# facebookresearch/D3GA

Measured on AMD Instinct MI355X. Metric: fwd+bwd frames/sec @500k Gaussians 1920x1080, higher is better.
Workload: dtype f32

## Files before the change

### d3ga_amd/_lib.py

```python
import ctypes
import os

_HERE = os.path.dirname(os.path.abspath(__file__))
_PATH = os.environ.get("D3GA_LIB_PATH") or os.path.join(_HERE, "libd3ga_hip.so")
_lib = None
ACC_STRIDE = 16
replay_epoch = [0]
ABI_VERSION = 111
KNOBS = ("composite_variant", "merge_slots", "tile_assign", "bwd_split", "sort_merge", "ssim_impl", "wgrad_ws", "chain_abl", "chain_grid")
CAMERA_SLOT_WINDOWED = -1.0
LOSS_PARTIALS = 2048
BLUR_PARTIALS = 6144
OPTIM_CHUNK = 8192
OPTIM_ALIGNED16 = 1


class D3GAError(RuntimeError):
    pass


def library_path():
    return _PATH


class RasterParams(ctypes.Structure):
    _fields_ = [("P", ctypes.c_int32), ("M", ctypes.c_int32), ("sh_degree", ctypes.c_int32),
                ("W", ctypes.c_int32), ("H", ctypes.c_int32),
                ("tanfovx", ctypes.c_float), ("tanfovy", ctypes.c_float), ("scale_modifier", ctypes.c_float),
                ("antialiasing", ctypes.c_int32), ("prefiltered", ctypes.c_int32), ("debug", ctypes.c_int32),
                ("opacity_activation", ctypes.c_int32), ("forward_only", ctypes.c_int32),
                ("acc_self_clearing", ctypes.c_int32), ("n_views", ctypes.c_int32), ("per_view_geometry", ctypes.c_int32),
                ("factor_rows", ctypes.c_int32), ("per_view_appearance", ctypes.c_int32), ("per_view_background", ctypes.c_int32)]


BODY_MAX_JOINTS = 64
BODY_MAX_SHAPE = 32
BODY_LD_ALIGN = 2048


def body_saved_floats(J):
    return 27 * J + 16


class BodyModel(ctypes.Structure):
    _fields_ = [("V", ctypes.c_int32), ("J", ctypes.c_int32), ("n_shape", ctypes.c_int32), ("n_expr", ctypes.c_int32),
                ("n_hand_pca", ctypes.c_int32), ("ld", ctypes.c_int32), ("n_levels", ctypes.c_int32), ("reserved", ctypes.c_int32)] + \
               [(n, ctypes.c_void_p) for n in ("v_template", "dirs", "w_ptr", "w_joint", "w_val", "wt_ptr", "wt_vert", "wt_val",
                                               "J0", "Jdirs", "parents", "level_ptr", "level_joint", "child_ptr", "child_joint",
                                               "hand_comps", "hand_mean")]


class LbsPoseGrad(ctypes.Structure):
    _fields_ = [("J", ctypes.c_int32), ("n_chunks", ctypes.c_int32), ("n_entries", ctypes.c_int64)] + \
               [(n, ctypes.c_void_p) for n in ("tmpl", "delta", "chunk_ptr", "chunk_range", "entries", "counter", "scratch", "g_joint_mats",
                                               "g_Rh", "g_Th")]


SKEL_MAX_JOINTS = 512
SKEL_SAVED_FLOATS = 12


class Skeleton(ctypes.Structure):
    _fields_ = [("J", ctypes.c_int32), ("n_params", ctypes.c_int32), ("n_levels", ctypes.c_int32), ("n_children", ctypes.c_int32)] + \
               [(n, ctypes.c_void_p) for n in ("parents", "level_ptr", "level_joint", "child_ptr", "child_joint", "joint_offset",
                                               "joint_rotation", "transform_offsets", "csr_ptr", "csr_col", "csr_val", "csc_ptr",
                                               "csc_row", "csc_val")]


_vp, _i, _i64, _f = ctypes.c_void_p, ctypes.c_int, ctypes.c_int64, ctypes.c_float
_prm = ctypes.POINTER(RasterParams)
_bm = ctypes.POINTER(BodyModel)
_lpg = ctypes.POINTER(LbsPoseGrad)
_sk = ctypes.POINTER(Skeleton)

_SIGNATURES = {
    "d3ga_version": ([], _i),
    "d3ga_status_string": ([_i], ctypes.c_char_p),
    "d3ga_debug_set": ([ctypes.c_int32, ctypes.c_int32], _i),
    "d3ga_debug_defaults": ([ctypes.POINTER(ctypes.c_int32), ctypes.c_int32], _i),
    "d3ga_lbs_cage_fwd": ([_i, _i] + [_vp] * 8 + [_vp], _i),
    "d3ga_lbs_cage_bwd": ([_i, _i] + [_vp] * 6 + [_vp], _i),
    "d3ga_lbs_pose_scratch_bytes": ([_i, ctypes.c_int32, ctypes.c_int32, ctypes.POINTER(_i64)], _i),
    "d3ga_lbs_cage_bwd_pose": ([_i, _i] + [_vp] * 6 + [_lpg, _vp], _i),
    "d3ga_cage_deform_fwd": ([_i] + [_vp] * 9 + [_vp], _i),
    "d3ga_cage_deform_bwd": ([_i, _i] + [_vp] * 16 + [_vp], _i),
    "d3ga_cage_deform_fwd_ex": ([_i] + [_vp] * 8 + [ctypes.c_int32] + [_vp] * 2 + [_vp], _i),
    "d3ga_cage_deform_bwd_ex": ([_i, _i] + [_vp] * 8 + [ctypes.c_int32] + [_vp] * 9 + [_vp], _i),
    "d3ga_cage_deform_bwd_merged": ([_i, _i] + [_vp] * 8 + [ctypes.c_int32] + [_vp] * 9 + [ctypes.c_int32] + [_vp] * 3 + [_vp], _i),
    "d3ga_cage_deform_bwd_merged_lbs": ([_i, _i] + [_vp] * 8 + [ctypes.c_int32] + [_vp] * 9 + [ctypes.c_int32] + [_vp] * 3 + [_i] + [_vp] * 6 + [_vp], _i),
    "d3ga_cage_deform_bwd_merged_lbs_pose": ([_i, _i] + [_vp] * 8 + [ctypes.c_int32] + [_vp] * 9 + [ctypes.c_int32] + [_vp] * 3 + [_i] + [_vp] * 6 + [_lpg, _vp], _i),
    "d3ga_fem_energy_fwd": ([_i] + [_vp] * 4 + [_vp], _i),
    "d3ga_fem_energy_bwd": ([_i, _i] + [_vp] * 5 + [_vp], _i),
    "d3ga_raster_scratch_bytes": ([ctypes.c_int32, ctypes.c_int32, ctypes.c_int32, _i64, ctypes.POINTER(_i64)], _i),
    "d3ga_raster_scratch_bytes_views": ([ctypes.c_int32] * 4 + [_i64, ctypes.c_int32, ctypes.POINTER(_i64)], _i),
    "d3ga_raster_scratch_bytes_window": ([ctypes.c_int32] * 4 + [_i64, ctypes.c_int32, ctypes.POINTER(_i64)], _i),
    "d3ga_raster_binning_layout_window": ([ctypes.c_int32] * 3 + [_i64, ctypes.POINTER(_i64)], _i),
    "d3ga_raster_binning_layout": ([ctypes.c_int32, ctypes.c_int32, _i64, ctypes.POINTER(_i64)], _i),
    "d3ga_raster_img_layout": ([ctypes.c_int32, ctypes.c_int32, ctypes.POINTER(_i64)], _i),
    "d3ga_raster_img_layout_blocks": ([ctypes.c_int32, ctypes.c_int32, ctypes.POINTER(_i64)], _i),
    "d3ga_raster_img_bytes": ([ctypes.c_int32, ctypes.c_int32, _i64, ctypes.c_int32], _i64),
    "d3ga_raster_preprocess": ([_prm] + [_vp] * 12 + [_i64, _vp, _vp], _i),
    "d3ga_raster_bin_sort": ([_prm, _vp, _vp, _i64, _vp], _i),
    "d3ga_raster_composite_fwd": ([_prm, _vp, _vp, _vp, _i64, _vp, _vp, _vp, _vp], _i),
    "d3ga_raster_composite_bwd": ([_prm, _vp, _vp, _vp, _i64, _vp, _vp, _vp, _vp], _i),
    "d3ga_raster_composite_bwd_depth": ([_prm, _vp, _vp, _vp, _i64, _vp, _vp, _vp, _vp, _vp], _i),
    "d3ga_raster_composite_fwd2": ([_prm, _vp, _vp, _vp, _vp, _vp, _i64, _vp, _vp, _vp, _vp, _vp], _i),
    "d3ga_raster_composite_bwd2": ([_prm, _vp, _vp, _vp, _vp, _vp, _i64, _vp, _vp, _vp, _vp, _vp], _i),
    "d3ga_raster_preprocess_bwd": ([_prm] + [_vp] * 18 + [_vp], _i),
    "d3ga_raster_forward": ([_prm] + [_vp] * 14 + [_i64, _vp, _vp, _vp, _vp], _i),
    "d3ga_raster_backward": ([_prm] + [_vp] * 11 + [_i64] + [_vp] * 11 + [_vp], _i),
    "d3ga_raster_composite_fwd_l1": ([_prm, _vp, _vp, _vp, _i64] + [_vp] * 7 + [_vp], _i),
    "d3ga_raster_composite_bwd_l1": ([_prm, _vp, _vp, _vp, _i64] + [_vp] * 7 + [_vp], _i),
    "d3ga_raster_backward_l1": ([_prm] + [_vp] * 11 + [_i64] + [_vp] * 15 + [_vp], _i),
    "d3ga_raster_recolor": ([_prm] + [_vp] * 6 + [_vp], _i),
    "d3ga_raster_mark_visible": ([ctypes.c_int32, _vp, _vp, _vp, _vp], _i),
    "d3ga_sh_grad_from_views": ([ctypes.c_int32] * 4 + [_vp, _vp, _i64, _vp, _i64, ctypes.c_float, _vp, _vp], _i),
    "d3ga_compute_bary": ([_i, _i] + [_vp] * 5 + [_vp], _i),
    "d3ga_selftest_row_scan": ([_i, _vp, _vp, _vp], _i),
    "d3ga_selftest_alpha": ([ctypes.c_int32, _vp, _i, _vp, _vp, _vp, _vp, _vp, _vp], _i),
    "d3ga_knn3_mean_dist2": ([_i, _vp, _vp, _vp], _i),
    "d3ga_compute_bary_grid": ([_i] + [_vp] * 9 + [_vp], _i),
    "d3ga_knn3_mean_dist2_grid": ([_i] + [_vp] * 6 + [_vp], _i),
    "d3ga_l1_mean_fwd": ([_i64, _vp, _vp, _vp, _vp], _i),
    "d3ga_l1_mean_fwd_ws": ([_i64, _vp, _vp, _vp, _vp, _vp], _i),
    "d3ga_l1_mean_bwd": ([_i64, _vp, _vp, _vp, _vp, _vp], _i),
    "d3ga_l1_mean_fwd_ws_cell": ([_i64, _vp, _vp, _vp, _vp, _vp], _i),
    "d3ga_l1_mean_bwd_cell": ([_i64, _vp, _vp, _vp, _vp, _vp], _i),
    "d3ga_mlp_panel_bytes": ([ctypes.c_int32, ctypes.c_int32], _i64),
    "d3ga_mlp_pack_weights": ([ctypes.c_int32, ctypes.c_int32, _vp, _i64, _i64, _vp, _vp], _i),
    "d3ga_mlp_linear": ([ctypes.c_int32] * 3 + [_vp, _vp, _vp, ctypes.c_float, _vp, _vp, ctypes.c_float, _vp, _vp], _i),
    "d3ga_mlp_chain_panel_bytes": ([ctypes.c_int32, ctypes.c_int32], _i64),
    "d3ga_mlp_pack_chain": ([ctypes.c_int32, ctypes.c_int32, _vp, _i64, _i64, _vp, _vp], _i),
    "d3ga_mlp_chain_fwd": ([ctypes.c_int32, ctypes.c_int32, _vp, ctypes.c_int32] + [_vp] * 9 + [_vp], _i),
    "d3ga_mlp_wgrad": ([ctypes.c_int32] * 3 + [_vp] * 4 + [_vp], _i),
    "d3ga_mlp_wgrad_acc": ([ctypes.c_int32] * 3 + [_vp] * 4 + [_vp], _i),
    "d3ga_field_heads_fwd": ([ctypes.c_int32] * 3 + [_vp, _vp, _vp, _vp, _vp, _vp], _i),
    "d3ga_field_heads_bwd": ([ctypes.c_int32] * 3 + [_vp, _vp, _vp] + [_vp] * 6 + [_vp], _i),
    "d3ga_view_dirs_fwd": ([ctypes.c_int32, _vp, _vp, _vp, _vp], _i),
    "d3ga_view_dirs_bwd": ([ctypes.c_int32, _vp, _vp, _vp, _vp, _vp], _i),
    "d3ga_sh4_encoding_fwd": ([ctypes.c_int32, _vp, _vp, _vp], _i),
    "d3ga_sh4_encoding_bwd": ([ctypes.c_int32, _vp, _vp, _vp, _vp], _i),
    "d3ga_color_rows_fwd": ([ctypes.c_int32, ctypes.c_int32, _vp, _vp, _vp, _vp], _i),
    "d3ga_color_rows_bwd": ([ctypes.c_int32, ctypes.c_int32, _vp, _vp, _vp, _vp, _vp], _i),
    "d3ga_ssim_fwd": ([ctypes.c_int32] * 3 + [_vp] * 6 + [_vp], _i),
    "d3ga_ssim_bwd": ([ctypes.c_int32] * 3 + [_vp] * 7 + [_vp], _i),
    "d3ga_ssim_l1_fwd": ([ctypes.c_int32] * 3 + [_vp] * 7 + [_vp], _i),
    "d3ga_ssim_l1_bwd": ([ctypes.c_int32] * 3 + [_vp] * 8 + [_vp], _i),
    "d3ga_blur_mix_fwd": ([ctypes.c_int32] * 4 + [_vp] * 4 + [_vp], _i),
    "d3ga_blur_mix_bwd": ([ctypes.c_int32] * 4 + [_vp] * 7 + [_vp], _i),
    "d3ga_compose_target": ([ctypes.c_int32] * 3 + [_vp] * 4 + [ctypes.c_int32] + [_vp] * 3 + [_vp], _i),
    "d3ga_optim_scratch_bytes": ([ctypes.c_int32] * 3 + [ctypes.POINTER(_i64)], _i),
    "d3ga_optim_clip_adam_step": ([_vp, ctypes.c_int32, _vp, ctypes.c_int32, _vp, ctypes.c_int32, ctypes.c_float, _vp, _vp, _vp], _i),
    "d3ga_body_model_scratch_bytes": ([_bm, ctypes.c_int32, ctypes.POINTER(_i64), ctypes.POINTER(_i64)], _i),
    "d3ga_body_model_fwd": ([_bm, ctypes.c_int32, ctypes.c_int32] + [_vp] * 10 + [_vp, _i64, _vp], _i),
    "d3ga_body_model_bwd": ([_bm, ctypes.c_int32, ctypes.c_int32] + [_vp] * 12 + [_vp, _i64, _vp], _i),
    "d3ga_skeleton_check": ([_sk] + [ctypes.c_int32] * 3, _i),
    "d3ga_skeleton_fwd": ([_sk] + [ctypes.c_int32] * 3 + [_vp, _vp, ctypes.c_int32, _vp, _vp, _f, ctypes.c_int32] + [_vp] * 4 + [_vp], _i),
    "d3ga_skeleton_bwd": ([_sk] + [ctypes.c_int32] * 4 + [_vp, _f, ctypes.c_int32] + [_vp] * 8 + [_vp], _i),
    "d3ga_skeleton_mats_fwd": ([ctypes.c_int32, ctypes.c_int32, _vp, _vp, _vp, _vp], _i),
    "d3ga_skeleton_mats_bwd": ([ctypes.c_int32, ctypes.c_int32, _vp, _vp, _vp, _vp, _vp], _i),
}
EXPORTS = tuple(_SIGNATURES)


def lib():
    global _lib
    if _lib is None:
        if not os.path.exists(_PATH):
            raise D3GAError(
                f"{_PATH} is missing: the HIP extension has not been built. Run "
                "`python -c 'import __graft_entry__ as g; g.build()'` (or python d3ga_amd/csrc/build.py). "
                "There is no CPU fallback for this path.")
        import torch
        L = ctypes.CDLL(_PATH)
        for name, (args, res) in _SIGNATURES.items():
            fn = getattr(L, name)
            fn.argtypes = args
            fn.restype = res
        if L.d3ga_version() != ABI_VERSION:
            raise D3GAError(f"libd3ga_hip.so version {L.d3ga_version()} does not match the Python layer ({ABI_VERSION})")
        info = (ctypes.c_int32 * (2 + 2 * len(KNOBS)))()
        L.d3ga_debug_defaults(info, len(info))
        if info[0] != 0 and os.environ.get("D3GA_ALLOW_ABLATION") != "1":
            raise D3GAError(f"{_PATH} is a timing-ablation build (D3GA_SCAN_ABL={info[0]}): its results are wrong by design. "
                            "Set D3GA_ALLOW_ABLATION=1 to load it for a timing run.")
        spec = os.environ.get("D3GA_KNOBS", "")
        for item in filter(None, (x.strip() for x in spec.split(","))):
            name, _, val = item.partition("=")
            if name not in KNOBS:
                raise D3GAError(f"D3GA_KNOBS: unknown knob {name!r} (known: {', '.join(KNOBS)})")
            st = L.d3ga_debug_set(KNOBS.index(name), int(val))
            if st != 0:
                raise D3GAError(f"d3ga_debug_set({name}, {val}) failed with status {st}")
        _lib = L
    return _lib


def debug_defaults():
    info = (ctypes.c_int32 * (2 + 2 * len(KNOBS)))()
    check(lib().d3ga_debug_defaults(info, len(info)), "d3ga_debug_defaults")
    out = {"scan_abl": info[0], "diag": info[1]}
    for k, name in enumerate(KNOBS):
        out[name] = (info[2 + 2 * k], info[3 + 2 * k])
    return out


def debug_set(name, value=None):
    check(lib().d3ga_debug_set(KNOBS.index(name), -2**31 if value is None else int(value)), "d3ga_debug_set")


def check(status, what):
    if status != 0:
        msg = lib().d3ga_status_string(status)
        raise D3GAError(f"{what} failed with status {status}: {msg.decode() if msg else '?'}")


def stream_handle():
    import torch
    raw = getattr(torch._C, "_cuda_getCurrentRawStream", None)
    if raw is not None:
        return ctypes.c_void_p(raw(torch.cuda.current_device()))
    return ctypes.c_void_p(torch.cuda.current_stream().cuda_stream)


def dptr(t):
    return None if t is None else ctypes.c_void_p(t.data_ptr())


def f32c16(t):
    if t is None:
        return None
    t = t.float().contiguous()
    if t.data_ptr() % 16:
        t = t.clone(memory_format=__import__("torch").contiguous_format)
    return t


def require_cuda(*tensors):
    import torch
    cur = None
    for t in tensors:
        if t is None:
            continue
        if not t.is_cuda:
            raise D3GAError("d3ga_amd ops run on the GPU only (tensor on %s); there is no CPU fallback" % t.device)
        if cur is None:
            cur = torch.cuda.current_device()
        if t.device.index != cur:
            raise D3GAError(f"tensor on {t.device} but the current device is cuda:{cur}: wrap the call in "
                            f"`with torch.cuda.device({t.device.index}):` (launches go to the current device's stream)")
```

### d3ga_amd/csrc/build.py

```python
import os
import subprocess
import sys

HERE = os.path.dirname(os.path.abspath(__file__))
SOURCES = ["deform.hip", "raster_pre.hip", "raster_bin.hip", "raster_composite.hip", "raster_composite_scan.hip", "raster_api.hip", "bary.hip", "loss.hip", "image_tail.hip", "optim.hip", "mlp.hip", "encoding.hip", "body_model.hip", "skeleton.hip"]
LINK_MAP = os.path.join(HERE, "d3ga.map")
HEADERS = ["d3ga_math.h", "d3ga_internal.h", "raster_pre_body.h", "composite_common.h", "body_model_math.h", "skeleton_math.h", os.path.join("..", "..", "include", "d3ga.h")]
ABL = os.environ.get("D3GA_SCAN_ABL")
VARIANT = os.environ.get("D3GA_VARIANT")
DIAG = os.environ.get("D3GA_DIAG") or (("abl" + ABL) if ABL else None) or (("var" + VARIANT.split(":")[0]) if VARIANT else None)
DIAG_DIR = os.path.abspath(os.path.join(HERE, "..", "..", "tools", "_build"))
_DIAG_TAG = (VARIANT.split(":")[0] if (VARIANT and not os.environ.get("D3GA_DIAG") and not ABL) else
             "diag" if os.environ.get("D3GA_DIAG") in (None, "counters") else os.environ["D3GA_DIAG"])
if VARIANT:
    FLAGS_VARIANT = [f for f in VARIANT.split(":", 1)[1].split(",") if f]
else:
    FLAGS_VARIANT = []
OUT = (os.path.join(DIAG_DIR, f"libd3ga_hip_abl{ABL}.so" if ABL else f"libd3ga_hip_{_DIAG_TAG}.so") if DIAG
       else os.path.join(HERE, "..", "libd3ga_hip.so"))
FLAGS = ["--offload-arch=gfx950", "-O3", "-std=c++17", "-fPIC", "-fvisibility=hidden", "-munsafe-fp-atomics", "-fno-gpu-rdc",
         "-Wall", "-Wno-unused-function"] + FLAGS_VARIANT
EXTRA = {"raster_composite_scan.hip": ["-fno-slp-vectorize"],
         "raster_composite.hip": ["-fno-slp-vectorize"]}
if os.environ.get("D3GA_CHAIN_WAVES"):
    FLAGS.append("-DD3GA_CHAIN_WAVES=" + os.environ["D3GA_CHAIN_WAVES"])
if os.environ.get("D3GA_CHAIN_CS"):
    FLAGS.append("-DD3GA_CHAIN_CS=" + os.environ["D3GA_CHAIN_CS"])
if os.environ.get("D3GA_ALL_NOSLP"):
    FLAGS.append("-fno-slp-vectorize")
if ABL:
    FLAGS.append("-DD3GA_SCAN_ABL=" + ABL.split("w")[0].split("p")[0].split("f")[0])
    if "w" in ABL:
        FLAGS.append("-DD3GA_TILE_WAVES=" + ABL.split("w")[1])
    if "f" in ABL:
        FLAGS.append("-DD3GA_FWD_WAVES=" + ABL.split("f")[1])
    if "p" in ABL:
        FLAGS.append("-DD3GA_TILE_PRIO=1")
if os.environ.get("D3GA_DIAG"):
    FLAGS += ["-DD3GA_DIAG", "-DD3GA_DIAG_TIMELINE"]
    if os.environ.get("D3GA_DIAG") == "counters":
        FLAGS.append("-DD3GA_DIAG_COUNTERS")


def _newer(target, deps):
    if not os.path.exists(target):
        return True
    t = os.path.getmtime(target)
    return any(os.path.getmtime(d) > t for d in deps)


def build(force=False, verbose=False):
    hipcc = os.environ.get("HIPCC", "/opt/rocm/bin/hipcc")
    objdir = os.path.join(DIAG_DIR, f"obj_abl{ABL}" if ABL else f"obj_{_DIAG_TAG}") if DIAG else os.path.join(HERE, "build")
    os.makedirs(objdir, exist_ok=True)
    hdrs = [os.path.join(HERE, h) for h in HEADERS]
    objs = []
    for src in SOURCES:
        s = os.path.join(HERE, src)
        o = os.path.join(objdir, src.replace(".hip", ".o"))
        if force or _newer(o, [s] + hdrs):
            cmd = [hipcc] + FLAGS + EXTRA.get(src, []) + ["-c", s, "-o", o]
            if verbose:
                print(" ".join(cmd))
            subprocess.check_call(cmd)
        objs.append(o)
    if force or _newer(OUT, objs + [LINK_MAP]):
        import torch
        tlib = os.path.join(os.path.dirname(torch.__file__), "lib")
        cmd = ["g++", "-shared", "-fPIC"] + objs + ["-L" + tlib, "-lamdhip64", "-Wl,-rpath," + tlib,
                                                    "-Wl,-rpath,/opt/rocm/lib", "-Wl,--version-script=" + LINK_MAP, "-o", OUT]
        if verbose:
            print(" ".join(cmd))
        subprocess.check_call(cmd)
    return os.path.abspath(OUT)


if __name__ == "__main__":
    print(build(force="--force" in sys.argv, verbose=True))
```

### d3ga_amd/csrc/d3ga_internal.h

```cpp
#pragma once
#include <hip/hip_runtime.h>
#include <stdint.h>

#include "../../include/d3ga.h"
#include "d3ga_math.h"

namespace d3ga {

constexpr int kBlock = 256;

int debug_knob(int key);

static inline int64_t align256(int64_t x) { return (x + 255) & ~int64_t(255); }

struct GeomBuf {
    float *depth;
    float4 *conic_o;
    float4 *rgb_invd;
    uint2 *rect;
    uint8_t *clamped;
    float *cov3D;
    float4 *xyh;
    float *dcol;
    int64_t dcol_stride;
};
static inline int64_t geom_bytes(int64_t P) {
    return align256(4 * P) + align256(16 * P) + align256(16 * P) + align256(8 * P) + align256(P) +
           align256(24 * P) + align256(16 * P) + align256(36 * P);
}
static inline GeomBuf carve_geom(void *base, int64_t P) {
    char *p = (char *)base;
    GeomBuf g;
    g.depth = (float *)p;     p += align256(4 * P);
    g.conic_o = (float4 *)p;  p += align256(16 * P);
    g.rgb_invd = (float4 *)p; p += align256(16 * P);
    g.rect = (uint2 *)p;      p += align256(8 * P);
    g.clamped = (uint8_t *)p; p += align256(P);
    g.cov3D = (float *)p;     p += align256(24 * P);
    g.xyh = (float4 *)p;      p += align256(16 * P);
    g.dcol = (float *)p;
    g.dcol_stride = P;
    return g;
}
__host__ __device__ static inline GeomBuf geom_view(const GeomBuf &g, int64_t P, int64_t v) {
    GeomBuf o = g;
    const int64_t d = v * P;
    o.depth += d; o.conic_o += d; o.rgb_invd += d; o.rect += d; o.clamped += d; o.cov3D += 6 * d; o.xyh += d; o.dcol += d;
    return o;
}

struct BinBuf {
    uint32_t *counters;
    uint32_t *tile_count;
    uint32_t *tile_start;
    uint32_t *tile_cursor;
    uint64_t *keys;
    uint32_t *point_list;
    uint32_t *big_tiles;
    uint32_t *huge_tiles;
    uint32_t *mid_tiles;
    uint32_t *tile_order;
};
static inline int64_t bin_bytes(int64_t tiles, int64_t dcap) {
    return 256 + align256(4 * tiles) + align256(4 * (tiles + 1)) + align256(4 * tiles) + align256(8 * dcap) +
           align256(4 * dcap) + 4 * align256(4 * tiles);
}
static inline BinBuf carve_bin(void *base, int64_t tiles, int64_t dcap) {
    char *p = (char *)base;
    BinBuf b;
    b.counters = (uint32_t *)p;    p += 256;
    b.tile_count = (uint32_t *)p;  p += align256(4 * tiles);
    b.tile_start = (uint32_t *)p;  p += align256(4 * (tiles + 1));
    b.tile_cursor = (uint32_t *)p; p += align256(4 * tiles);
    b.keys = (uint64_t *)p;        p += align256(8 * dcap);
    b.point_list = (uint32_t *)p;  p += align256(4 * dcap);
    b.big_tiles = (uint32_t *)p;   p += align256(4 * tiles);
    b.huge_tiles = (uint32_t *)p;  p += align256(4 * tiles);
    b.mid_tiles = (uint32_t *)p;   p += align256(4 * tiles);
    b.tile_order = (uint32_t *)p;
    return b;
}

struct ImgBuf {
    float *final_T;
    uint32_t *n_contrib;
    uint32_t *blk_count;
    uint2 *blk_list;
};
static inline int64_t img_bytes(int64_t W, int64_t H, int64_t tiles, int64_t dcap, int64_t views = 1) {
    return 2 * align256(4 * W * H * views) + align256(64 * tiles) + align256(128 * dcap);
}
static inline ImgBuf carve_img(void *base, int64_t W, int64_t H, int64_t tiles, int64_t views = 1) {
    ImgBuf i;
    char *p = (char *)base;
    i.final_T = (float *)p;        p += align256(4 * W * H * views);
    i.n_contrib = (uint32_t *)p;   p += align256(4 * W * H * views);
    i.blk_count = (uint32_t *)p;   p += align256(64 * tiles);
    i.blk_list = (uint2 *)p;
    return i;
}

constexpr int kWinTiles = 4096;

struct TileWindow {
    int x0, y0, w, h;
    __device__ __forceinline__ int area() const { return w * h; }
    __device__ __forceinline__ bool fits() const { return w * h <= kWinTiles; }
    __device__ __forceinline__ int tile_of(int k, int gx, float inv_w) const {
        const int r = (int)(((float)k + 0.5f) * inv_w);
        return (y0 + r) * gx + x0 + (k - r * w);
    }
};

#ifdef __HIPCC__
__device__ __forceinline__ TileWindow block_tile_window(int *s_box, bool visible, int rx0, int ry0, int rx1, int ry1) {
    if (threadIdx.x == 0) { s_box[0] = 0x7fffffff; s_box[1] = 0x7fffffff; s_box[2] = 0; s_box[3] = 0; }
    __syncthreads();
    int bx0 = visible ? rx0 : 0x7fffffff, by0 = visible ? ry0 : 0x7fffffff, bx1 = visible ? rx1 : 0, by1 = visible ? ry1 : 0;
#pragma unroll
    for (int off = 1; off < 64; off <<= 1) {
        bx0 = min(bx0, __shfl_xor(bx0, off)); by0 = min(by0, __shfl_xor(by0, off));
        bx1 = max(bx1, __shfl_xor(bx1, off)); by1 = max(by1, __shfl_xor(by1, off));
    }
    if ((threadIdx.x & 63) == 0 && bx1 > 0) {
        atomicMin(&s_box[0], bx0); atomicMin(&s_box[1], by0);
        atomicMax(&s_box[2], bx1); atomicMax(&s_box[3], by1);
    }
    __syncthreads();
    TileWindow win;
    win.x0 = s_box[0]; win.y0 = s_box[1];
    win.w = s_box[2] > s_box[0] ? s_box[2] - s_box[0] : 0;
    win.h = s_box[3] > s_box[1] ? s_box[3] - s_box[1] : 0;
    if (win.w == 0 || win.h == 0) { win.w = 0; win.h = 0; }
    return win;
}
#endif

static inline int tiles_x(int W) { return (W + kTile - 1) / kTile; }
static inline int tiles_y(int H) { return (H + kTile - 1) / kTile; }
static inline int n_views_of(const d3ga_raster_params *prm) { return prm->n_views > 1 ? prm->n_views : 1; }
static inline bool is_windowed(const d3ga_raster_params *prm) { return prm->tanfovx == D3GA_CAMERA_SLOT_WINDOWED; }
static inline int grid_x(const d3ga_raster_params *prm) { return tiles_x(prm->W) + (is_windowed(prm) ? 1 : 0); }
static inline int grid_y(const d3ga_raster_params *prm) { return tiles_y(prm->H) + (is_windowed(prm) ? 1 : 0); }
static inline int4 *win_table(void *binning, int64_t tiles, int64_t dcap) { return (int4 *)((char *)binning + bin_bytes(tiles, dcap)); }
static inline int64_t win_table_bytes(int64_t views) { return align256(16 * views); }

static inline int check_launch(hipStream_t s, int debug) {
    hipError_t e = hipGetLastError();
    if (e != hipSuccess) return (int)e;
    if (debug) {
        e = hipStreamSynchronize(s);
        if (e != hipSuccess) return (int)e;
    }
    return 0;
}

#define D3GA_TRY(expr)            \
    do {                          \
        int _st = (expr);         \
        if (_st != 0) return _st; \
    } while (0)
#define D3GA_HIP(expr)                          \
    do {                                        \
        hipError_t _e = (expr);                 \
        if (_e != hipSuccess) return (int)_e;   \
    } while (0)

#ifdef __HIPCC__
static __global__ void zero_words_kernel(uint32_t *__restrict__ p, size_t n) {
    for (size_t i = (size_t)blockIdx.x * blockDim.x + threadIdx.x; i < n; i += (size_t)gridDim.x * blockDim.x) p[i] = 0u;
}
static __global__ void zero_bytes_kernel(unsigned char *__restrict__ p, size_t n) {
    for (size_t i = (size_t)blockIdx.x * blockDim.x + threadIdx.x; i < n; i += (size_t)gridDim.x * blockDim.x) p[i] = 0;
}
static inline hipError_t zero_async(void *ptr, size_t bytes, hipStream_t s) {
    if (bytes == 0) return hipSuccess;
    if ((((uintptr_t)ptr | bytes) & 3) == 0) {
        const size_t n = bytes / 4;
        const size_t blocks = (n + 4 * kBlock - 1) / (4 * kBlock);
        hipLaunchKernelGGL(zero_words_kernel, dim3((unsigned)(blocks < 1 ? 1 : (blocks > 4096 ? 4096 : blocks))), dim3(kBlock), 0, s,
                           reinterpret_cast<uint32_t *>(ptr), n);
    } else {
        const size_t blocks = (bytes + kBlock - 1) / kBlock;
        hipLaunchKernelGGL(zero_bytes_kernel, dim3((unsigned)(blocks > 4096 ? 4096 : blocks)), dim3(kBlock), 0, s,
                           reinterpret_cast<unsigned char *>(ptr), bytes);
    }
    return hipGetLastError();
}
#endif

}
```

### d3ga_amd/csrc/raster_api.hip

```cpp
#include "d3ga_internal.h"

#include <atomic>

namespace d3ga {
static const int kKnobDefault[D3GA_KNOB_COUNT] = {
     32 | 128,  512,  2,  -1,  -1,
     1,  1,  0,  0};
static std::atomic<int> g_knob[D3GA_KNOB_COUNT] = {{32 | 128}, {512}, {2}, {-1}, {-1}, {1}, {1}, {0}, {0}};
int debug_knob(int key) { return (key >= 0 && key < D3GA_KNOB_COUNT) ? g_knob[key].load(std::memory_order_relaxed) : 0; }
}

using namespace d3ga;

extern "C" int d3ga_debug_set(int32_t key, int32_t value) {
    if (key < 0 || key >= D3GA_KNOB_COUNT) return D3GA_E_SIZE;
    g_knob[key].store(value == D3GA_KNOB_DEFAULT ? kKnobDefault[key] : value, std::memory_order_relaxed);
    return D3GA_OK;
}

extern "C" int d3ga_debug_defaults(int32_t *out, int32_t n) {
    if (!out) return D3GA_E_NULL;
    if (n < 2 + 2 * D3GA_KNOB_COUNT) return D3GA_E_SIZE;
#ifdef D3GA_SCAN_ABL
    out[0] = D3GA_SCAN_ABL;
#else
    out[0] = 0;
#endif
#ifdef D3GA_DIAG
    out[1] = 1;
#else
    out[1] = 0;
#endif
    for (int k = 0; k < D3GA_KNOB_COUNT; ++k) { out[2 + 2 * k] = kKnobDefault[k]; out[3 + 2 * k] = debug_knob(k); }
    return D3GA_OK;
}

extern "C" int d3ga_version(void) { return D3GA_VERSION; }

extern "C" const char *d3ga_status_string(int status) {
    switch (status) {
        case D3GA_OK: return "ok";
        case D3GA_E_NULL: return "required pointer is NULL";
        case D3GA_E_SIZE: return "negative or inconsistent size";
        case D3GA_E_CONFIG: return "unsupported argument combination";
        case D3GA_E_CAPACITY: return "scratch buffer too small";
        default: break;
    }
    if (status > 0) return hipGetErrorString((hipError_t)status);
    return "unknown status";
}

extern "C" int d3ga_raster_scratch_bytes_views(int32_t P, int32_t W, int32_t H, int32_t n_views, int64_t d_capacity,
                                               int32_t forward_only, int64_t sizes[3]) {
    if (!sizes) return D3GA_E_NULL;
    if (P < 0 || W <= 0 || H <= 0 || d_capacity < 0 || n_views < 0) return D3GA_E_SIZE;
    const int64_t k = n_views > 1 ? n_views : 1;
    if ((int64_t)tiles_y(H) * k > 65535 || (int64_t)P * k >= (1ll << 31)) return D3GA_E_SIZE;
    const int64_t tiles = (int64_t)tiles_x(W) * tiles_y(H) * k, cap = d_capacity > 0 ? d_capacity : 1;
    sizes[0] = geom_bytes(P > 0 ? P * k : 1);
    sizes[1] = bin_bytes(tiles, cap);
    sizes[2] = forward_only ? 2 * align256(4 * (int64_t)W * H * k) : img_bytes(W, H, tiles, cap, k);
    return D3GA_OK;
}

extern "C" int d3ga_raster_scratch_bytes_window(int32_t P, int32_t W, int32_t H, int32_t n_views, int64_t d_capacity,
                                                int32_t forward_only, int64_t sizes[3]) {
    if (!sizes) return D3GA_E_NULL;
    if (P < 0 || W <= 0 || H <= 0 || d_capacity < 0 || n_views < 0) return D3GA_E_SIZE;
    const int64_t k = n_views > 1 ? n_views : 1;
    const int64_t gx = tiles_x(W) + 1, gy = tiles_y(H) + 1;
    if (gy * k > 65535 || gx > 65535 || (int64_t)P * k >= (1ll << 31)) return D3GA_E_SIZE;
    const int64_t tiles = gx * gy * k, cap = d_capacity > 0 ? d_capacity : 1;
    sizes[0] = geom_bytes(P > 0 ? P * k : 1);
    sizes[1] = bin_bytes(tiles, cap) + win_table_bytes(k);
    sizes[2] = forward_only ? 2 * align256(4 * (int64_t)W * H * k) : img_bytes(W, H, tiles, cap, k);
    return D3GA_OK;
}

extern "C" int d3ga_raster_binning_layout_window(int32_t W, int32_t H, int32_t n_views, int64_t d_capacity, int64_t offsets[7]) {
    if (!offsets) return D3GA_E_NULL;
    if (W <= 0 || H <= 0 || d_capacity < 0 || n_views < 0) return D3GA_E_SIZE;
    const int64_t k = n_views > 1 ? n_views : 1, cap = d_capacity > 0 ? d_capacity : 1;
    const int64_t tiles = (int64_t)(tiles_x(W) + 1) * (tiles_y(H) + 1) * k;
    char *base = (char *)nullptr + 256;
    const BinBuf b = carve_bin(base, tiles, cap);
    offsets[0] = (char *)b.counters - base;
    offsets[1] = (char *)b.tile_count - base;
    offsets[2] = (char *)b.tile_start - base;
    offsets[3] = (char *)b.tile_cursor - base;
    offsets[4] = (char *)b.keys - base;
    offsets[5] = (char *)b.point_list - base;
    offsets[6] = (char *)win_table(base, tiles, cap) - base;
    return D3GA_OK;
}

extern "C" int d3ga_raster_scratch_bytes(int32_t P, int32_t W, int32_t H, int64_t d_capacity, int64_t sizes[3]) {
    return d3ga_raster_scratch_bytes_views(P, W, H, 1, d_capacity, 0, sizes);
}

extern "C" int64_t d3ga_raster_img_bytes(int32_t W, int32_t H, int64_t d_capacity, int32_t forward_only) {
    if (W <= 0 || H <= 0 || d_capacity < 0) return D3GA_E_SIZE;
    const int64_t tiles = (int64_t)tiles_x(W) * tiles_y(H);
    return forward_only ? 2 * align256(4 * (int64_t)W * H) : img_bytes(W, H, tiles, d_capacity > 0 ? d_capacity : 1);
}

extern "C" int d3ga_raster_binning_layout(int32_t W, int32_t H, int64_t d_capacity, int64_t offsets[6]) {
    if (!offsets) return D3GA_E_NULL;
    if (W <= 0 || H <= 0 || d_capacity < 0) return D3GA_E_SIZE;
    char *base = (char *)nullptr + 256;
    const BinBuf b = carve_bin(base, (int64_t)tiles_x(W) * tiles_y(H), d_capacity > 0 ? d_capacity : 1);
    offsets[0] = (char *)b.counters - base;
    offsets[1] = (char *)b.tile_count - base;
    offsets[2] = (char *)b.tile_start - base;
    offsets[3] = (char *)b.tile_cursor - base;
    offsets[4] = (char *)b.keys - base;
    offsets[5] = (char *)b.point_list - base;
    return D3GA_OK;
}

extern "C" int d3ga_raster_img_layout(int32_t W, int32_t H, int64_t offsets[2]) {
    if (!offsets) return D3GA_E_NULL;
    if (W <= 0 || H <= 0) return D3GA_E_SIZE;
    offsets[0] = 0;
    offsets[1] = align256(4 * (int64_t)W * H);
    return D3GA_OK;
}

extern "C" int d3ga_raster_img_layout_blocks(int32_t W, int32_t H, int64_t offsets[2]) {
    if (!offsets) return D3GA_E_NULL;
    if (W <= 0 || H <= 0) return D3GA_E_SIZE;
    const int64_t tiles = (int64_t)tiles_x(W) * tiles_y(H);
    char *base = (char *)nullptr + 256;
    const ImgBuf im = carve_img(base, W, H, tiles);
    offsets[0] = (char *)im.blk_count - base;
    offsets[1] = (char *)im.blk_list - base;
    return D3GA_OK;
}

extern "C" int d3ga_raster_forward(const d3ga_raster_params *prm, const float *means3D, const float *shs,
                                   const float *colors_precomp, const float *opacities, const float *scales,
                                   const float *rotations, const float *cov3D_precomp, const float *viewmatrix,
                                   const float *projmatrix, const float *campos, const float *bg, void *geom,
                                   void *binning, void *img, int64_t d_capacity, float *out_color, int32_t *radii,
                                   float *out_invdepth, d3ga_stream_t stream) {
    D3GA_TRY(d3ga_raster_preprocess(prm, means3D, shs, colors_precomp, opacities, scales, rotations, cov3D_precomp,
                                    viewmatrix, projmatrix, campos, geom, binning, d_capacity, radii, stream));
    D3GA_TRY(d3ga_raster_bin_sort(prm, geom, binning, d_capacity, stream));
    return d3ga_raster_composite_fwd(prm, bg, geom, binning, d_capacity, img, out_color, out_invdepth, stream);
}

extern "C" int d3ga_raster_backward(const d3ga_raster_params *prm, const float *means3D, const float *shs,
                                    const float *scales, const float *rotations, const float *cov3D_precomp,
                                    const float *viewmatrix, const float *projmatrix, const float *campos,
                                    const float *bg, const void *geom, const void *binning, int64_t d_capacity,
                                    const void *img, const float *dL_dpix, float *acc, float *dL_dmeans3D,
                                    float *dL_dmeans2D, float *dL_dopacity, float *dL_dsh, float *dL_dcolors,
                                    float *dL_dcov3D, float *dL_dscales, float *dL_drots, d3ga_stream_t stream) {
    if (prm && prm->P > 0 && acc && !prm->acc_self_clearing)
        D3GA_HIP(zero_async(acc, sizeof(float) * D3GA_ACC_STRIDE * (size_t)prm->P * (size_t)n_views_of(prm), (hipStream_t)stream));
    D3GA_TRY(d3ga_raster_composite_bwd(prm, bg, geom, binning, d_capacity, img, dL_dpix, acc, stream));
    return d3ga_raster_preprocess_bwd(prm, means3D, shs, scales, rotations, cov3D_precomp, viewmatrix, projmatrix,
                                      campos, geom, acc, dL_dmeans3D, dL_dmeans2D, dL_dopacity, dL_dsh, dL_dcolors,
                                      dL_dcov3D, dL_dscales, dL_drots, stream);
}

extern "C" int d3ga_raster_backward_l1(const d3ga_raster_params *prm, const float *means3D, const float *shs,
                                       const float *scales, const float *rotations, const float *cov3D_precomp,
                                       const float *viewmatrix, const float *projmatrix, const float *campos,
                                       const float *bg, const void *geom, const void *binning, int64_t d_capacity,
                                       const void *img, const float *image, const float *target, const void *target_cell,
                                       const float *g_loss, const float *dL_dpix, float *acc, float *dL_dmeans3D,
                                       float *dL_dmeans2D, float *dL_dopacity, float *dL_dsh, float *dL_dcolors,
                                       float *dL_dcov3D, float *dL_dscales, float *dL_drots, d3ga_stream_t stream) {
    if (prm && prm->P > 0 && acc && !prm->acc_self_clearing)
        D3GA_HIP(zero_async(acc, sizeof(float) * D3GA_ACC_STRIDE * (size_t)prm->P * (size_t)n_views_of(prm), (hipStream_t)stream));
    D3GA_TRY(d3ga_raster_composite_bwd_l1(prm, bg, geom, binning, d_capacity, img, image, target, target_cell, g_loss, dL_dpix,
                                          acc, stream));
    return d3ga_raster_preprocess_bwd(prm, means3D, shs, scales, rotations, cov3D_precomp, viewmatrix, projmatrix,
                                      campos, geom, acc, dL_dmeans3D, dL_dmeans2D, dL_dopacity, dL_dsh, dL_dcolors,
                                      dL_dcov3D, dL_dscales, dL_drots, stream);
}
```

### d3ga_amd/csrc/raster_bin.hip

```cpp
#include <atomic>

#include "composite_common.h"

namespace d3ga {

constexpr int kScanBlock = 1024;

__device__ __forceinline__ void tile_scan_body(int tiles, const uint32_t *__restrict__ count,
                                               uint32_t *__restrict__ start, uint32_t *__restrict__ cursor,
                                               uint32_t *__restrict__ counters, uint64_t dcap,
                                               uint32_t *__restrict__ big_tiles, uint32_t *__restrict__ huge_tiles,
                                               uint32_t *__restrict__ mid_tiles, uint32_t n_small, uint32_t n_mid,
                                               uint32_t n_large) {
    constexpr int kPer = 8, kChunk = kPer * kScanBlock;
    __shared__ uint32_t s_wave[2][kScanBlock / 64];
    __shared__ uint32_t s_max;
    const int tid = threadIdx.x, lane = tid & 63, wave = tid >> 6;
    if (tid == 0) s_max = 0;
    uint32_t carry = 0, mx = 0;
    int par = 0;
    for (int c0 = 0; c0 < tiles; c0 += kChunk, par ^= 1) {
        const int t0 = c0 + kPer * tid;
        uint32_t c[kPer];
        if (t0 + kPer <= tiles) {
            const uint4 lo = reinterpret_cast<const uint4 *>(count + t0)[0], hi = reinterpret_cast<const uint4 *>(count + t0)[1];
            c[0] = lo.x; c[1] = lo.y; c[2] = lo.z; c[3] = lo.w; c[4] = hi.x; c[5] = hi.y; c[6] = hi.z; c[7] = hi.w;
        } else {
#pragma unroll
            for (int k = 0; k < kPer; ++k) c[k] = t0 + k < tiles ? count[t0 + k] : 0u;
        }
        uint32_t sum = 0;
#pragma unroll
        for (int k = 0; k < kPer; ++k) { sum += c[k]; mx = max(mx, c[k]); }
        uint32_t incl = sum;
#pragma unroll
        for (int off = 1; off < 64; off <<= 1) {
            const uint32_t v = __shfl_up(incl, off);
            if (lane >= off) incl += v;
        }
        if (lane == 63) s_wave[par][wave] = incl;
        __syncthreads();
        uint32_t wbase = 0, total = 0;
#pragma unroll
        for (int w = 0; w < kScanBlock / 64; ++w) {
            const uint32_t v = s_wave[par][w];
            wbase += w < wave ? v : 0u;
            total += v;
        }
        uint32_t run = carry + wbase + incl - sum;
        uint32_t e[kPer];
        int cls[kPer];
#pragma unroll
        for (int k = 0; k < kPer; ++k) {
            e[k] = run;
            run += c[k];
            cls[k] = c[k] > n_large ? 2 : (c[k] > n_mid ? 1 : (c[k] > n_small ? 0 : -1));
        }
#pragma unroll
        for (int q = 0; q < 3; ++q) {
            uint32_t nq = 0;
#pragma unroll
            for (int k = 0; k < kPer; ++k) nq += cls[k] == q ? 1u : 0u;
            if (__ballot(nq != 0u) == 0ull) continue;
            uint32_t inq = nq;
#pragma unroll
            for (int off = 1; off < 64; off <<= 1) {
                const uint32_t v = __shfl_up(inq, off);
                if (lane >= off) inq += v;
            }
            const uint32_t tot = (uint32_t)__shfl((int)inq, 63);
            uint32_t base = 0;
            if (lane == 0) base = atomicAdd(&counters[q == 0 ? D3GA_CNT_MID : (q == 1 ? D3GA_CNT_BIG : D3GA_CNT_HUGE)], tot);
            uint32_t pos = (uint32_t)__shfl((int)base, 0) + inq - nq;
            uint32_t *list = q == 0 ? mid_tiles : (q == 1 ? big_tiles : huge_tiles);
#pragma unroll
            for (int k = 0; k < kPer; ++k)
                if (cls[k] == q) list[pos++] = (uint32_t)(t0 + k);
        }
        if (t0 + kPer <= tiles) {
            const uint4 lo = make_uint4(e[0], e[1], e[2], e[3]), hi = make_uint4(e[4], e[5], e[6], e[7]);
            reinterpret_cast<uint4 *>(start + t0)[0] = lo; reinterpret_cast<uint4 *>(start + t0)[1] = hi;
            reinterpret_cast<uint4 *>(cursor + t0)[0] = lo; reinterpret_cast<uint4 *>(cursor + t0)[1] = hi;
        } else {
#pragma unroll
            for (int k = 0; k < kPer; ++k)
                if (t0 + k < tiles) { start[t0 + k] = e[k]; cursor[t0 + k] = e[k]; }
        }
        carry += total;
    }
#pragma unroll
    for (int off = 1; off < 64; off <<= 1) mx = max(mx, (uint32_t)__shfl_xor((int)mx, off));
    if (lane == 0) atomicMax(&s_max, mx);
    __syncthreads();
    if (tid == 0) {
        start[tiles] = carry;
        counters[D3GA_CNT_D] = carry;
        counters[D3GA_CNT_OVERFLOW] = (uint64_t)carry > dcap ? 1u : 0u;
        counters[D3GA_CNT_MAXTILE] = s_max;
    }
}

__device__ __forceinline__ void tile_order_body(int tiles, const uint32_t *__restrict__ count,
                                                uint32_t *__restrict__ order, uint32_t *__restrict__ counters) {
    __shared__ uint32_t s_hist[256];
    __shared__ uint32_t s_zero;
    const int tid = threadIdx.x, lane = tid & 63;
    constexpr int kPer = 8;
    if (tid < 256) s_hist[tid] = 0;
    if (tid == 0) s_zero = 0;
    __syncthreads();
    auto bucket = [](uint32_t c) { return 254u - min(c >> 4, 254u); };
    for (int c0 = 0; c0 < tiles; c0 += kPer * kScanBlock) {
        uint32_t c[kPer];
#pragma unroll
        for (int k = 0; k < kPer; ++k) {
            const int t = c0 + k * kScanBlock + tid;
            c[k] = t < tiles ? count[t] : 0xffffffffu;
        }
#pragma unroll
        for (int k = 0; k < kPer; ++k) {
            const bool zero = c[k] == 0u;
            const unsigned long long zm = __ballot(zero);
            if (lane == 0 && zm) atomicAdd(&s_zero, (uint32_t)__popcll(zm));
            if (c[k] != 0u && c[k] != 0xffffffffu) atomicAdd(&s_hist[bucket(c[k])], 1u);
        }
        if (c0 + kPer * kScanBlock < tiles) continue;
        __syncthreads();
        if (tid < 64) {
            uint32_t v[4], sum = 0;
#pragma unroll
            for (int k = 0; k < 4; ++k) { v[k] = (4 * tid + k < 255) ? s_hist[4 * tid + k] : 0u; sum += v[k]; }
            uint32_t incl = sum;
#pragma unroll
            for (int off = 1; off < 64; off <<= 1) {
                const uint32_t u = __shfl_up(incl, off);
                if (tid >= off) incl += u;
            }
            uint32_t run = incl - sum;
#pragma unroll
            for (int k = 0; k < 4; ++k) { s_hist[4 * tid + k] = run; run += v[k]; }
        }
        __syncthreads();
        if (tid == 0) {
            s_zero = s_hist[255];
            counters[D3GA_CNT_HEAVY] = s_hist[255] <= 4096u ? (s_hist[255] + 9u) / 10u : 0u;
        }
        __syncthreads();
        for (int c1 = 0; c1 < tiles; c1 += kPer * kScanBlock) {
            if (c0 != 0) {
#pragma unroll
                for (int k = 0; k < kPer; ++k) {
                    const int t = c1 + k * kScanBlock + tid;
                    c[k] = t < tiles ? count[t] : 0xffffffffu;
                }
            }
#pragma unroll
            for (int k = 0; k < kPer; ++k) {
                const int t = c1 + k * kScanBlock + tid;
                const bool zero = c[k] == 0u;
                const unsigned long long zm = __ballot(zero);
                uint32_t zbase = 0;
                if (lane == 0 && zm) zbase = atomicAdd(&s_zero, (uint32_t)__popcll(zm));
                zbase = (uint32_t)__shfl((int)zbase, 0);
                if (zero) order[zbase + (uint32_t)__popcll(zm & ((1ull << lane) - 1ull))] = (uint32_t)t;
                if (c[k] != 0u && c[k] != 0xffffffffu) order[atomicAdd(&s_hist[bucket(c[k])], 1u)] = (uint32_t)t;
            }
        }
    }
}

__global__ __launch_bounds__(kScanBlock) void tile_scan_order_kernel(int tiles, const uint32_t *__restrict__ count,
                                                                     uint32_t *__restrict__ start,
                                                                     uint32_t *__restrict__ cursor,
                                                                     uint32_t *__restrict__ counters, uint64_t dcap,
                                                                     uint32_t *__restrict__ big_tiles,
                                                                     uint32_t *__restrict__ huge_tiles,
                                                                     uint32_t *__restrict__ mid_tiles, uint32_t n_small,
                                                                     uint32_t n_mid, uint32_t n_large,
                                                                     uint32_t *__restrict__ order) {
    if (blockIdx.x == 0) tile_scan_body(tiles, count, start, cursor, counters, dcap, big_tiles, huge_tiles, mid_tiles, n_small, n_mid, n_large);
    else tile_order_body(tiles, count, order, counters);
}

__global__ __launch_bounds__(kBlock) void tile_scatter_kernel(int P, int gx, const uint2 *__restrict__ rect,
                                                              const float *__restrict__ depth,
                                                              uint32_t *__restrict__ cursor, uint64_t *__restrict__ keys,
                                                              uint64_t dcap) {
    __shared__ int s_box[4];
    __shared__ uint32_t s_cnt[kWinTiles];
    const int tid = threadIdx.x;
    const int i = blockIdx.x * kBlock + tid;
    int x0 = 0, y0 = 0, x1 = 0, y1 = 0;
    uint64_t key = 0;
    if (i < P) {
        const uint2 rc = rect[i];
        x0 = rc.x & 0xffffu; y0 = rc.x >> 16; x1 = rc.y & 0xffffu; y1 = rc.y >> 16;
        key = ((uint64_t)__float_as_uint(depth[i]) << 32) | (uint32_t)i;
    }
    const bool visible = x1 > x0 && y1 > y0;
    const TileWindow win = block_tile_window(s_box, visible, x0, y0, x1, y1);
    const int area = win.area();
    if (area == 0) return;
    if (win.fits()) {
        for (int k = tid; k < area; k += kBlock) s_cnt[k] = 0;
        __syncthreads();
        if (visible)
            for (int ty = y0; ty < y1; ++ty)
                for (int tx = x0; tx < x1; ++tx) atomicAdd(&s_cnt[(ty - win.y0) * win.w + (tx - win.x0)], 1u);
        __syncthreads();
        const float inv_w = 1.0f / (float)win.w;
        for (int k = tid; k < area; k += kBlock) {
            const uint32_t c = s_cnt[k];
            if (c) s_cnt[k] = atomicAdd(&cursor[win.tile_of(k, gx, inv_w)], c);
        }
        __syncthreads();
        if (visible)
            for (int ty = y0; ty < y1; ++ty)
                for (int tx = x0; tx < x1; ++tx) {
                    const int l = (ty - win.y0) * win.w + (tx - win.x0);
                    const uint32_t pos = atomicAdd(&s_cnt[l], 1u);
                    if (pos < dcap) keys[pos] = key;
                }
    } else if (visible) {
        for (int ty = y0; ty < y1; ++ty)
            for (int tx = x0; tx < x1; ++tx) {
                const uint32_t pos = atomicAdd(&cursor[ty * gx + tx], 1u);
                if (pos < dcap) keys[pos] = key;
            }
    }
}

template <typename KeyPtr>
__device__ __forceinline__ void bitonic_sort(KeyPtr k, int n, int tid, int nthreads) {
    int n2 = 1;
    while (n2 < n) n2 <<= 1;
    const int half = n2 >> 1;
    for (int size = 2, lsz = 1; size <= n2; size <<= 1, ++lsz) {
        const int hs = size >> 1;
        for (int i = tid; i < half; i += nthreads) {
            const int blk = i >> (lsz - 1), off = i & (hs - 1);
            const int lo = (blk << lsz) + off, hi = (blk << lsz) + size - 1 - off;
            if (hi < n) {
                const uint64_t a = k[lo], b = k[hi];
                if (b < a) { k[lo] = b; k[hi] = a; }
            }
        }
        __syncthreads();
        for (int j = hs >> 1, lj = lsz - 2; j >= 1; j >>= 1, --lj) {
            for (int i = tid; i < half; i += nthreads) {
                const int blk = i >> lj, off = i & (j - 1);
                const int lo = (blk << (lj + 1)) + off, hi = lo + j;
                if (hi < n) {
                    const uint64_t a = k[lo], b = k[hi];
                    if (b < a) { k[lo] = b; k[hi] = a; }
                }
            }
            __syncthreads();
        }
    }
}

template <int BLOCK, int CAP>
__device__ __forceinline__ void sort_one_tile_bucket(uint64_t *s_key, uint32_t *s_bin, uint32_t *s_red, int tile,
                                                     const uint32_t *__restrict__ start, const uint64_t *__restrict__ keys,
                                                     uint32_t *__restrict__ point_list, uint64_t dcap) {
    static_assert(CAP == 8 * BLOCK, "eight keys / eight counters per thread");
    constexpr int NW = BLOCK / 64;
    const uint64_t b64 = min((uint64_t)start[tile], dcap), e64 = min((uint64_t)start[tile + 1], dcap);
    const int n = min((int)(e64 - b64), CAP);
    const int tid = threadIdx.x, lane = tid & 63, wave = tid >> 6;
    uint64_t r[8];
    uint32_t lo = 0xffffffffu, hi = 0u;
#pragma unroll
    for (int k = 0; k < 8; ++k) {
        const int i = tid + k * BLOCK;
        r[k] = i < n ? keys[b64 + i] : ~0ull;
    }
#pragma unroll
    for (int k = 0; k < 8; ++k) {
        const int i = tid + k * BLOCK;
        if (i < n) { const uint32_t d = (uint32_t)(r[k] >> 32); lo = min(lo, d); hi = max(hi, d); }
    }
#pragma unroll
    for (int off = 1; off < 64; off <<= 1) {
        lo = min(lo, (uint32_t)__shfl_xor((int)lo, off));
        hi = max(hi, (uint32_t)__shfl_xor((int)hi, off));
    }
    if (lane == 0) { s_red[wave] = lo; s_red[NW + wave] = hi; }
#pragma unroll
    for (int k = 0; k < 8; ++k) s_bin[tid + k * BLOCK] = 0u;
    __syncthreads();
#pragma unroll
    for (int w = 0; w < NW; ++w) { lo = min(lo, s_red[w]); hi = max(hi, s_red[NW + w]); }
    const uint32_t range = hi - lo;
    int sh = 32 - __clz((int)(range | 1u)) - (31 - __clz(CAP));
    if (range & 0x80000000u) sh = 32 - (31 - __clz(CAP));
    sh = max(sh, 0);
    uint32_t bucket[8], slot[8];
#pragma unroll
    for (int k = 0; k < 8; ++k) {
        const int i = tid + k * BLOCK;
        bucket[k] = ((uint32_t)(r[k] >> 32) - lo) >> sh;
        slot[k] = 0u;
        if (i < n) slot[k] = atomicAdd(&s_bin[bucket[k]], 1u);
    }
    __syncthreads();
    {
        uint32_t c[8], sum = 0;
#pragma unroll
        for (int k = 0; k < 8; ++k) { c[k] = s_bin[8 * tid + k]; sum += c[k]; }
        uint32_t incl = sum;
#pragma unroll
        for (int off = 1; off < 64; off <<= 1) {
            const uint32_t u = (uint32_t)__shfl_up((int)incl, off);
            if (lane >= off) incl += u;
        }
        if (lane == 63) s_red[wave] = incl;
        __syncthreads();
        uint32_t run = incl - sum;
#pragma unroll
        for (int w = 0; w < NW; ++w) if (w < wave) run += s_red[w];
#pragma unroll
        for (int k = 0; k < 8; ++k) { s_bin[8 * tid + k] = run; run += c[k]; }
        if (tid == BLOCK - 1) s_bin[CAP] = run;
    }
    __syncthreads();
#pragma unroll
    for (int k = 0; k < 8; ++k) {
        const int i = tid + k * BLOCK;
        if (i < n) s_key[s_bin[bucket[k]] + slot[k]] = r[k];
    }
    __syncthreads();
#pragma unroll
    for (int k = 0; k < 8; ++k) {
        const int i = tid + k * BLOCK;
        if (i < n) {
            const uint32_t b0 = s_bin[bucket[k]], b1 = s_bin[bucket[k] + 1];
            uint32_t less = 0;
            for (uint32_t p = b0; p < b1; ++p) less += s_key[p] < r[k] ? 1u : 0u;
            point_list[b64 + b0 + less] = (uint32_t)r[k];
        }
    }
}

template <int BLOCK, int CAP>
__device__ __forceinline__ bool sort_huge_tile_bucket(uint64_t *s_key, uint32_t *s_bin, uint32_t *s_cur, uint32_t *s_red, int tile,
                                                      const uint32_t *__restrict__ start, const uint64_t *__restrict__ keys,
                                                      uint32_t *__restrict__ point_list, uint64_t dcap) {
    static_assert(CAP == 8 * BLOCK, "eight counters per thread");
    constexpr int NW = BLOCK / 64;
    const uint64_t b64 = min((uint64_t)start[tile], dcap), e64 = min((uint64_t)start[tile + 1], dcap);
    const int n = (int)(e64 - b64);
    const int tid = threadIdx.x, lane = tid & 63, wave = tid >> 6;
    uint32_t lo = 0xffffffffu, hi = 0u;
    for (int i = tid; i < n; i += BLOCK) { const uint32_t d = (uint32_t)(keys[b64 + i] >> 32); lo = min(lo, d); hi = max(hi, d); }
#pragma unroll
    for (int off = 1; off < 64; off <<= 1) {
        lo = min(lo, (uint32_t)__shfl_xor((int)lo, off));
        hi = max(hi, (uint32_t)__shfl_xor((int)hi, off));
    }
    __syncthreads();
    if (lane == 0) { s_red[wave] = lo; s_red[NW + wave] = hi; }
#pragma unroll
    for (int k = 0; k < 8; ++k) s_bin[tid + k * BLOCK] = 0u;
    __syncthreads();
#pragma unroll
    for (int w = 0; w < NW; ++w) { lo = min(lo, s_red[w]); hi = max(hi, s_red[NW + w]); }
    const uint32_t range = hi - lo;
    const int sh = max(32 - __clz((int)(range | 1u)) - (31 - __clz(CAP)), 0);
    for (int i = tid; i < n; i += BLOCK) atomicAdd(&s_bin[((uint32_t)(keys[b64 + i] >> 32) - lo) >> sh], 1u);
    __syncthreads();
    uint32_t cmax = 0;
    {
        uint32_t c[8], sum = 0;
#pragma unroll
        for (int k = 0; k < 8; ++k) { c[k] = s_bin[8 * tid + k]; sum += c[k]; cmax = max(cmax, c[k]); }
        uint32_t incl = sum;
#pragma unroll
        for (int off = 1; off < 64; off <<= 1) {
            const uint32_t u = (uint32_t)__shfl_up((int)incl, off);
            if (lane >= off) incl += u;
            cmax = max(cmax, (uint32_t)__shfl_xor((int)cmax, off));
        }
        __syncthreads();
        if (lane == 63) { s_red[wave] = incl; s_red[NW + wave] = cmax; }
        __syncthreads();
        uint32_t run = incl - sum;
#pragma unroll
        for (int w = 0; w < NW; ++w) { if (w < wave) run += s_red[w]; cmax = max(cmax, s_red[NW + w]); }
#pragma unroll
        for (int k = 0; k < 8; ++k) { s_bin[8 * tid + k] = run; run += c[k]; }
        if (tid == BLOCK - 1) s_bin[CAP] = run;
    }
    __syncthreads();
    if (cmax > (uint32_t)CAP) return false;
    for (int segA = 0; segA < CAP;) {
        if (tid == 0) {
            const uint32_t limit = s_bin[segA] + (uint32_t)CAP;
            int a = segA + 1, b = CAP;
            while (a < b) { const int m = (a + b + 1) >> 1; if (s_bin[m] <= limit) a = m; else b = m - 1; }
            s_red[0] = (uint32_t)a;
        }
#pragma unroll
        for (int k = 0; k < 8; ++k) s_cur[tid + k * BLOCK] = 0u;
        __syncthreads();
        const int segB = (int)s_red[0];
        const uint32_t baseA = s_bin[segA], m = s_bin[segB] - baseA;
        if (m) {
            for (int i = tid; i < n; i += BLOCK) {
                const uint64_t key = keys[b64 + i];
                const uint32_t b = ((uint32_t)(key >> 32) - lo) >> sh;
                if (b >= (uint32_t)segA && b < (uint32_t)segB) s_key[s_bin[b] - baseA + atomicAdd(&s_cur[b], 1u)] = key;
            }
            __syncthreads();
            for (uint32_t i = tid; i < m; i += BLOCK) {
                const uint64_t key = s_key[i];
                const uint32_t b = ((uint32_t)(key >> 32) - lo) >> sh;
                const uint32_t b0 = s_bin[b] - baseA, b1 = s_bin[b + 1] - baseA;
                uint32_t less = 0;
                for (uint32_t p = b0; p < b1; ++p) less += s_key[p] < key ? 1u : 0u;
                point_list[b64 + baseA + b0 + less] = (uint32_t)key;
            }
        }
        __syncthreads();
        segA = segB;
    }
    return true;
}

template <int BLOCK, int CAP>
__global__ __launch_bounds__(BLOCK) void tile_sort_lds_kernel(const uint32_t *__restrict__ start,
                                                              const uint64_t *__restrict__ keys,
                                                              uint32_t *__restrict__ point_list, uint64_t dcap,
                                                              const uint32_t *__restrict__ order, int tiles) {
    __shared__ uint64_t s_key[CAP];
    __shared__ __attribute__((aligned(8))) uint32_t s_bin[CAP + 1];
    __shared__ uint32_t s_red[2 * (BLOCK / 64)];
    for (int rank = blockIdx.x; rank < tiles; rank += gridDim.x) {
        const int tile = (int)order[rank];
        const uint32_t n = start[tile + 1] - start[tile];
        if (n == 0) return;
        if (n <= (uint32_t)CAP) sort_one_tile_bucket<BLOCK, CAP>(s_key, s_bin, s_red, tile, start, keys, point_list, dcap);
        __syncthreads();
    }
}

template <int BLOCK, int CAP>
__global__ __launch_bounds__(BLOCK) void tile_sort_lds_list_kernel(const uint32_t *__restrict__ start,
                                                                   const uint64_t *__restrict__ keys,
                                                                   uint32_t *__restrict__ point_list, uint64_t dcap,
                                                                   const uint32_t *__restrict__ list,
                                                                   const uint32_t *__restrict__ list_count,
                                                                   uint64_t *__restrict__ keys_rw,
                                                                   const uint32_t *__restrict__ huge_list,
                                                                   const uint32_t *__restrict__ huge_count,
                                                                   const uint32_t *__restrict__ list2,
                                                                   const uint32_t *__restrict__ list2_count) {
    extern __shared__ __attribute__((aligned(16))) uint64_t s_key_dyn[];
    uint32_t *s_bin = reinterpret_cast<uint32_t *>(s_key_dyn + CAP);
    uint32_t *s_red = s_bin + CAP + 1;
    uint32_t *s_cur = s_red + 2 * (BLOCK / 64) + 2;
    const uint32_t count = *list_count;
    for (uint32_t v = blockIdx.x; v < count; v += gridDim.x) {
        __syncthreads();
        sort_one_tile_bucket<BLOCK, CAP>(s_key_dyn, s_bin, s_red, (int)list[v], start, keys, point_list, dcap);
    }
    if (list2) {
        const uint32_t count2 = *list2_count;
        for (uint32_t v = gridDim.x - 1u - blockIdx.x; v < count2; v += gridDim.x) {
            __syncthreads();
            sort_one_tile_bucket<BLOCK, CAP>(s_key_dyn, s_bin, s_red, (int)list2[v], start, keys, point_list, dcap);
        }
    }
    if (huge_list) {
        const uint32_t hcount = *huge_count;
        const int tid = threadIdx.x;
        for (uint32_t k = blockIdx.x; k < hcount; k += gridDim.x) {
            const int tile = (int)huge_list[k];
            const uint64_t b64 = min((uint64_t)start[tile], dcap), e64 = min((uint64_t)start[tile + 1], dcap);
            const int n = (int)(e64 - b64);
            __syncthreads();
            if (!sort_huge_tile_bucket<BLOCK, CAP>(s_key_dyn, s_bin, s_cur, s_red, tile, start, keys, point_list, dcap)) {
                bitonic_sort(keys_rw + b64, n, tid, BLOCK);
                for (int i = tid; i < n; i += BLOCK) point_list[b64 + i] = (uint32_t)keys_rw[b64 + i];
            }
        }
    }
}

}

using namespace d3ga;

constexpr int kSortSmall = 2048;
constexpr int kSortMid = 4096;
constexpr int kSortLarge = 8192;
static inline size_t sort_lds_bytes(int cap, int block, bool huge = false) {
    return (size_t)cap * 8 + ((size_t)cap + 1 + 2 * (block / 64) + 2 + (huge ? cap : 0)) * 4 + 16;
}


extern "C" int d3ga_raster_bin_sort(const d3ga_raster_params *prm, void *geom, void *binning, int64_t d_capacity,
                                    d3ga_stream_t stream) {
    if (!prm || !geom || !binning) return D3GA_E_NULL;
    if (prm->P < 0 || prm->W <= 0 || prm->H <= 0 || d_capacity < 0) return D3GA_E_SIZE;
    hipStream_t s = (hipStream_t)stream;
    const int views = n_views_of(prm);
    const int gx = grid_x(prm);
    const int tiles = gx * grid_y(prm) * views;
    const int64_t P = (int64_t)prm->P * views;
    BinBuf bin = carve_bin(binning, tiles, d_capacity);
    GeomBuf g = carve_geom(geom, P);
    hipLaunchKernelGGL(tile_scan_order_kernel, dim3(2), dim3(kScanBlock), 0, s, tiles, bin.tile_count, bin.tile_start,
                       bin.tile_cursor, bin.counters, (uint64_t)d_capacity, bin.big_tiles, bin.huge_tiles, bin.mid_tiles,
                       (uint32_t)kSortSmall, (uint32_t)kSortMid, (uint32_t)kSortLarge, bin.tile_order);
    D3GA_TRY(check_launch(s, prm->debug));
    if (P == 0 || d_capacity == 0) return D3GA_OK;
    hipLaunchKernelGGL(tile_scatter_kernel, dim3((unsigned)((P + kBlock - 1) / kBlock)), dim3(kBlock), 0, s, (int)P, gx, g.rect,
                       g.depth, bin.tile_cursor, bin.keys, (uint64_t)d_capacity);
    D3GA_TRY(check_launch(s, prm->debug));
    {
        static std::atomic<int> resident[64] = {};
        int dev = 0;
        D3GA_HIP(hipGetDevice(&dev));
        int want = (dev >= 0 && dev < 64) ? resident[dev].load(std::memory_order_relaxed) : 0;
        if (want == 0) {
            int per_cu = 0, cus = 0;
            if (hipOccupancyMaxActiveBlocksPerMultiprocessor(&per_cu, (const void *)tile_sort_lds_kernel<256, kSortSmall>, 256, 0) != hipSuccess || per_cu < 1) per_cu = 4;
            if (hipDeviceGetAttribute(&cus, hipDeviceAttributeMultiprocessorCount, dev) != hipSuccess || cus < 1) cus = 256;
            want = per_cu * cus;
            if (dev >= 0 && dev < 64) resident[dev].store(want, std::memory_order_relaxed);
        }
        hipLaunchKernelGGL((tile_sort_lds_kernel<256, kSortSmall>), dim3(tiles < want ? tiles : want), dim3(256), 0, s, bin.tile_start,
                           bin.keys, bin.point_list, (uint64_t)d_capacity, (const uint32_t *)bin.tile_order, tiles);
    }
    D3GA_TRY(check_launch(s, prm->debug));
    {
        static std::atomic<bool> attr_set[64] = {};
        int dev = 0;
        D3GA_HIP(hipGetDevice(&dev));
        if (dev >= 0 && dev < 64 && !attr_set[dev].load(std::memory_order_relaxed)) {
            D3GA_HIP(hipFuncSetAttribute((const void *)tile_sort_lds_list_kernel<1024, kSortLarge>,
                                         hipFuncAttributeMaxDynamicSharedMemorySize, (int)sort_lds_bytes(kSortLarge, 1024, true)));
            attr_set[dev].store(true, std::memory_order_relaxed);
        }
    }
    const int lgrid = tiles < 256 ? tiles : 256, mgrid = tiles < 768 ? tiles : 768;
    const int merge_knob = debug_knob(D3GA_KNOB_SORT_MERGE);
    const bool merged = merge_knob >= 0 ? merge_knob != 0 : d_capacity / (tiles > 0 ? tiles : 1) < 320;
#define D3GA_LAUNCH_LIST_SORT(BLOCKV, CAPV, GRID, HUGE, LIST, CNT, KEYS_RW, HLIST, HCNT, LIST2, CNT2)                              \
    hipLaunchKernelGGL((tile_sort_lds_list_kernel<BLOCKV, CAPV>), dim3(GRID), dim3(BLOCKV), sort_lds_bytes(CAPV, BLOCKV, HUGE), s, \
                       bin.tile_start, bin.keys, bin.point_list, (uint64_t)d_capacity, LIST, CNT, KEYS_RW, HLIST, HCNT, LIST2, CNT2)
    const uint32_t *const nil = nullptr;
    if (!merged) {
        D3GA_LAUNCH_LIST_SORT(512, kSortMid, mgrid, false, bin.mid_tiles, bin.counters + D3GA_CNT_MID, (uint64_t *)nullptr, nil, nil, nil, nil);
        D3GA_TRY(check_launch(s, prm->debug));
    }
    const uint32_t *l2 = merged ? (const uint32_t *)bin.mid_tiles : nil, *c2 = merged ? (const uint32_t *)(bin.counters + D3GA_CNT_MID) : nil;
    D3GA_LAUNCH_LIST_SORT(1024, kSortLarge, lgrid, true, bin.big_tiles, bin.counters + D3GA_CNT_BIG, bin.keys,
                          (const uint32_t *)bin.huge_tiles, (const uint32_t *)(bin.counters + D3GA_CNT_HUGE), l2, c2);
#undef D3GA_LAUNCH_LIST_SORT
    return check_launch(s, prm->debug);
}
```

### d3ga_amd/csrc/raster_pre.hip

```cpp
#include "composite_common.h"
#include "raster_pre_body.h"

namespace d3ga {

constexpr int kShRow = 52;
constexpr int kShSlab = 64 * kShRow;
constexpr size_t kShLdsBytes = (size_t)(kBlock / 64) * kShSlab * sizeof(float);

__host__ __device__ __forceinline__ bool sh_staged(int M) { return M > 0 && (3 * M) % 4 == 0 && 3 * M <= 48; }

__device__ __forceinline__ void sh_slab_load(float *slab, const float *__restrict__ src, int rows, int M3, int lane) {
    const int nvec = rows * M3 / 4;
    for (int v = lane; v < nvec; v += 64) {
        const float4 x = reinterpret_cast<const float4 *>(src)[v];
        const int e = 4 * v, r = e / M3, c = e - r * M3;
        *reinterpret_cast<float4 *>(slab + r * kShRow + c) = x;
    }
}
__device__ __forceinline__ void sh_slab_store(const float *slab, float *__restrict__ dst, int rows, int M3, int lane) {
    const int nvec = rows * M3 / 4;
    for (int v = lane; v < nvec; v += 64) {
        const int e = 4 * v, r = e / M3, c = e - r * M3;
        reinterpret_cast<float4 *>(dst)[v] = *reinterpret_cast<const float4 *>(slab + r * kShRow + c);
    }
}

template <int ROWS>
struct ShRegs { float4 v[ROWS * 12 / 64]; };
template <int ROWS>
__device__ __forceinline__ ShRegs<ROWS> sh_rows48_load(const float *__restrict__ src, int lane) {
    ShRegs<ROWS> r;
#pragma unroll
    for (int k = 0; k < ROWS * 12 / 64; ++k) r.v[k] = reinterpret_cast<const float4 *>(src)[lane + 64 * k];
    return r;
}
template <int ROWS>
__device__ __forceinline__ void sh_rows48_to_slab(float *slab, const ShRegs<ROWS> &r, int lane) {
#pragma unroll
    for (int k = 0; k < ROWS * 12 / 64; ++k) {
        const int e = 4 * (lane + 64 * k), row = e / 48, c = e - row * 48;
        *reinterpret_cast<float4 *>(slab + row * kShRow + c) = r.v[k];
    }
}
template <int ROWS>
__device__ __forceinline__ void sh_rows48_store(const float *slab, float *__restrict__ dst, int lane) {
#pragma unroll
    for (int k = 0; k < ROWS * 12 / 64; ++k) {
        const int e = 4 * (lane + 64 * k), row = e / 48, c = e - row * 48;
        reinterpret_cast<float4 *>(dst)[lane + 64 * k] = *reinterpret_cast<const float4 *>(slab + row * kShRow + c);
    }
}

constexpr int kShPassRows = 32;
constexpr int kShHalfSlab = kShPassRows * kShRow;
constexpr size_t kShHalfLdsBytes = (size_t)(kBlock / 64) * kShHalfSlab * sizeof(float);

template <bool WANT_J>
__device__ __forceinline__ void staged_sh_colour(const d3ga_raster_params &prm, const float *__restrict__ means3D,
                                                 const float *__restrict__ shs, const float *__restrict__ campos,
                                                 float *s_sh, float acc[3], ShColJ &cj) {
    const int tid = threadIdx.x, lane = tid & 63, wave = tid >> 6;
    const int i = blockIdx.x * kBlock + tid;
    const int M3 = 3 * prm.M;
    float *slab = s_sh + wave * kShHalfSlab;
    const int row0 = blockIdx.x * kBlock + wave * 64;
    const int rows = min(64, prm.P - row0);
    const int nb = (prm.sh_degree + 1) * (prm.sh_degree + 1);
    float B[16];
    float dx = 0.f, dy = 0.f, dz = 1.f;
    if (WANT_J && i < prm.P) sh_view_dir(means3D, i, campos, dx, dy, dz);
    auto eval = [&](const float *row) __attribute__((always_inline)) {
        if (WANT_J) cj = sh_accumulate_jacobian(B, dx, dy, dz, row, nb, cj);
        else sh_accumulate(B, row, 0, 16, nb, acc);
    };
    if (M3 == 48 && rows == 64) {
        const float *src = shs + (size_t)48 * row0;
        const ShRegs<kShPassRows> h0 = sh_rows48_load<kShPassRows>(src, lane);
        const ShRegs<kShPassRows> h1 = sh_rows48_load<kShPassRows>(src + 48 * kShPassRows, lane);
        sh_view_basis(prm, means3D, i, campos, B);
        __builtin_amdgcn_wave_barrier();
        sh_rows48_to_slab<kShPassRows>(slab, h0, lane);
        __builtin_amdgcn_wave_barrier();
        if (lane / kShPassRows == 0) eval(slab + (lane % kShPassRows) * kShRow);
        __builtin_amdgcn_wave_barrier();
        sh_rows48_to_slab<kShPassRows>(slab, h1, lane);
        __builtin_amdgcn_wave_barrier();
        if (lane / kShPassRows == 1) eval(slab + (lane % kShPassRows) * kShRow);
        return;
    }
    if (i < prm.P) sh_view_basis(prm, means3D, i, campos, B);
    for (int h = 0; h < 2; ++h) {
        const int r = min(kShPassRows, rows - kShPassRows * h);
        __builtin_amdgcn_wave_barrier();
        if (r > 0) sh_slab_load(slab, shs + (size_t)M3 * (row0 + kShPassRows * h), r, M3, lane);
        __builtin_amdgcn_wave_barrier();
        if (i < prm.P && lane / kShPassRows == h) eval(slab + (lane % kShPassRows) * kShRow);
    }
}

struct TileRect { bool visible; int r0, r1, r2, r3; };
__device__ __forceinline__ TileRect write_geom_records(const GeomBuf &geom, int i, const PreOut &o, bool keep_cov, int tile_row0,
                                                       int32_t *__restrict__ radii, bool want_j, const ShColJ &cj) {
    const Splat &sp = o.sp;
    if (keep_cov) {
#pragma unroll
        for (int k = 0; k < 6; ++k) geom.cov3D[6 * (size_t)i + k] = o.c6[k];
    }
    radii[i] = sp.radius;
    geom.depth[i] = sp.depth;
    geom.rect[i] = sp.visible ? make_uint2((uint32_t)sp.rect[0] | ((uint32_t)(sp.rect[1] + tile_row0) << 16),
                                           (uint32_t)sp.rect[2] | ((uint32_t)(sp.rect[3] + tile_row0) << 16))
                              : make_uint2(0u, 0u);
    geom.conic_o[i] = make_float4(sp.conic[0], sp.conic[1], sp.conic[2], o.opacity);
    {
        const SplatCull sc = splat_cull(sp.conic[0], sp.conic[1], sp.conic[2], o.opacity);
        geom.xyh[i] = make_float4(sp.px, sp.py, sp.visible ? sc.hx : -1.0f, sc.hy);
    }
    geom.rgb_invd[i] = make_float4(o.rgb[0], o.rgb[1], o.rgb[2], sp.visible ? 1.0f / sp.depth : 0.f);
    geom.clamped[i] = o.clampmask;
    if (want_j) dcol_store(geom.dcol, geom.dcol_stride, i, cj);
    return TileRect{sp.visible, sp.rect[0], sp.rect[1] + tile_row0, sp.rect[2], sp.rect[3] + tile_row0};
}

__device__ __forceinline__ PreOut window_clip(PreOut o, int x0, int y0, int gx, int gy) {
    Splat &sp = o.sp;
    const int r0 = max(sp.rect[0], x0) - x0, r1 = max(sp.rect[1], y0) - y0;
    const int r2 = min(sp.rect[2], x0 + gx) - x0, r3 = min(sp.rect[3], y0 + gy) - y0;
    if (sp.visible && r2 > r0 && r3 > r1) { sp.rect[0] = r0; sp.rect[1] = r1; sp.rect[2] = r2; sp.rect[3] = r3; }
    else { sp.visible = false; sp.rect[0] = sp.rect[1] = sp.rect[2] = sp.rect[3] = 0; }
    return o;
}
__global__ void window_table_kernel(d3ga_raster_params prm, const float *__restrict__ campos, int views, int4 *__restrict__ table) {
    const int v = blockIdx.x * blockDim.x + threadIdx.x;
    if (v >= views) return;
    const ViewCam c = view_cam(prm, nullptr, nullptr, campos + (size_t)D3GA_CAMERA_SLOT_WINDOWED_FLOATS * v, true);
    table[v] = make_int4(c.ox, c.oy, c.W, c.H);
}

__device__ __forceinline__ void tile_histogram(int *s_box, uint32_t *s_cnt, const TileRect &t, int gx, uint32_t *__restrict__ tile_count,
                                               uint32_t *__restrict__ counters) {
    const int tid = threadIdx.x;
    const TileWindow win = block_tile_window(s_box, t.visible, t.r0, t.r1, t.r2, t.r3);
    const int nvis = __syncthreads_count(t.visible);
    if (tid == 0 && nvis) atomicAdd(&counters[D3GA_CNT_VISIBLE], (uint32_t)nvis);
    const int area = win.area();
    if (area == 0) return;
    if (win.fits()) {
        for (int k = tid; k < area; k += kBlock) s_cnt[k] = 0;
        __syncthreads();
        if (t.visible)
            for (int ty = t.r1; ty < t.r3; ++ty)
                for (int tx = t.r0; tx < t.r2; ++tx) atomicAdd(&s_cnt[(ty - win.y0) * win.w + (tx - win.x0)], 1u);
        __syncthreads();
        const float inv_w = 1.0f / (float)win.w;
        for (int k = tid; k < area; k += kBlock) {
            const uint32_t c = s_cnt[k];
            if (c) atomicAdd(&tile_count[win.tile_of(k, gx, inv_w)], c);
        }
    } else if (t.visible) {
        for (int ty = t.r1; ty < t.r3; ++ty)
            for (int tx = t.r0; tx < t.r2; ++tx) atomicAdd(&tile_count[ty * gx + tx], 1u);
    }
}

template <bool WIN>
__device__ __forceinline__ TileRect preprocess_view(const d3ga_raster_params &prm, const ViewCam &cam, int i, const float *means3D,
                                                    const float *sh_row, bool staged, const ShColJ &cj, bool pre, const float (&pc6)[6],
                                                    float pop, const float *colors_precomp, const float *opacities, const float *scales,
                                                    const float *rotations, const float *cov3D_precomp, const GeomBuf &geom,
                                                    int tile_row0, int32_t *radii, bool want_j, int gx, int gy) {
    PreLoaded pl;
    pl.has_sh = staged; pl.has_c6 = pre;
    pl.sh[0] = cj.a0; pl.sh[1] = cj.a1; pl.sh[2] = cj.a2;
#pragma unroll
    for (int k = 0; k < 6; ++k) pl.c6[k] = pc6[k];
    pl.op = pop;
    PreOut o = preprocess_one(prm, cam, i, means3D, sh_row, colors_precomp, opacities, scales, rotations, cov3D_precomp, pl);
    if constexpr (WIN) o = window_clip(o, cam.ox / kTile, cam.oy / kTile, gx, gy);
    return write_geom_records(geom, i, o, !cov3D_precomp, tile_row0, radii, want_j, cj);
}

template <bool WANT_J, bool WIN>
__global__ __launch_bounds__(kBlock) void preprocess_kernel(
    d3ga_raster_params prm, const float *__restrict__ means3D, const float *__restrict__ shs,
    const float *__restrict__ colors_precomp, const float *__restrict__ opacities, const float *__restrict__ scales,
    const float *__restrict__ rotations, const float *__restrict__ cov3D_precomp, const float *__restrict__ viewmatrix,
    const float *__restrict__ projmatrix, const float *__restrict__ campos, GeomBuf geom,
    uint32_t *__restrict__ tile_count, uint32_t *__restrict__ counters, int32_t *__restrict__ radii,
    int tile_row0 ) {
    const ViewCam cam = view_cam(prm, viewmatrix, projmatrix, campos, WIN);
    const int gx = (prm.W + kTile - 1) / kTile + (WIN ? 1 : 0), gy = (prm.H + kTile - 1) / kTile + 1;
    extern __shared__ __attribute__((aligned(16))) char smem[];
    __shared__ int s_box[4];
    float *s_sh = reinterpret_cast<float *>(smem);
    uint32_t *s_cnt = reinterpret_cast<uint32_t *>(smem);
    const int tid = threadIdx.x;
    const int i = blockIdx.x * kBlock + tid;
    const int M3 = 3 * prm.M;
    const bool staged = shs != nullptr && sh_staged(prm.M);
    float pc6[6] = {0.f, 0.f, 0.f, 0.f, 0.f, 0.f}, pop = 0.f;
    const bool pre = staged && cov3D_precomp != nullptr;
    if (pre && i < prm.P) {
#pragma unroll
        for (int k = 0; k < 6; ++k) pc6[k] = cov3D_precomp[6 * (size_t)i + k];
        pop = opacities[i];
    }
    ShColJ cj = {0.f, 0.f, 0.f, 0.f, 0.f, 0.f, 0.f, 0.f, 0.f, 0.f, 0.f, 0.f};
    float acc[3] = {0.f, 0.f, 0.f};
    if (staged) {
        staged_sh_colour<WANT_J>(prm, means3D, shs, campos, s_sh, acc, cj);
        if (!WANT_J) { cj.a0 = acc[0]; cj.a1 = acc[1]; cj.a2 = acc[2]; }
        __syncthreads();
    }
    TileRect tr = {false, 0, 0, 0, 0};
    if (i < prm.P) {
        tr = staged ? preprocess_view<WIN>(prm, cam, i, means3D, nullptr, true, cj, pre, pc6, pop, colors_precomp, opacities, scales,
                                           rotations, cov3D_precomp, geom, tile_row0, radii, WANT_J, gx, gy)
                    : preprocess_view<WIN>(prm, cam, i, means3D, shs ? shs + (size_t)M3 * i : nullptr, false, cj, false, pc6, pop,
                                           colors_precomp, opacities, scales, rotations, cov3D_precomp, geom, tile_row0, radii,
                                           WANT_J, gx, gy);
    }
    tile_histogram(s_box, s_cnt, tr, gx, tile_count, counters);
}

template <bool WANT_J, int KV>
__device__ __forceinline__ void staged_sh_colour_views(const d3ga_raster_params &prm, const float *__restrict__ means3D, size_t pv,
                                                       const float *__restrict__ shs, const ViewCams<KV> &cams, float *s_sh,
                                                       ShColJ (&cj)[KV]) {
    const int tid = threadIdx.x, lane = tid & 63, wave = tid >> 6;
    const int i = blockIdx.x * kBlock + tid;
    const int M3 = 3 * prm.M;
    float *slab = s_sh + wave * kShHalfSlab;
    const int row0 = blockIdx.x * kBlock + wave * 64;
    const int rows = min(64, prm.P - row0);
    const int nb = (prm.sh_degree + 1) * (prm.sh_degree + 1);
    auto eval = [&](const float *row) __attribute__((always_inline)) {
#pragma unroll
        for (int v = 0; v < KV; ++v) {
            float B[16];
            const float *mv = means3D + 3 * pv * v;
            if (WANT_J) {
                float dx, dy, dz;
                sh_view_dir(mv, i, cams.cp[v], dx, dy, dz);
                sh_basis(prm.sh_degree, dx, dy, dz, B);
                cj[v] = sh_accumulate_jacobian(B, dx, dy, dz, row, nb, cj[v]);
            } else {
                sh_view_basis(prm, mv, i, cams.cp[v], B);
                float acc[3] = {cj[v].a0, cj[v].a1, cj[v].a2};
                sh_accumulate(B, row, 0, 16, nb, acc);
                cj[v].a0 = acc[0]; cj[v].a1 = acc[1]; cj[v].a2 = acc[2];
            }
        }
    };
    if (M3 == 48 && rows == 64) {
        const float *src = shs + (size_t)48 * row0;
        const ShRegs<kShPassRows> h0 = sh_rows48_load<kShPassRows>(src, lane);
        const ShRegs<kShPassRows> h1 = sh_rows48_load<kShPassRows>(src + 48 * kShPassRows, lane);
        __builtin_amdgcn_wave_barrier();
        sh_rows48_to_slab<kShPassRows>(slab, h0, lane);
        __builtin_amdgcn_wave_barrier();
        if (lane / kShPassRows == 0) eval(slab + (lane % kShPassRows) * kShRow);
        __builtin_amdgcn_wave_barrier();
        sh_rows48_to_slab<kShPassRows>(slab, h1, lane);
        __builtin_amdgcn_wave_barrier();
        if (lane / kShPassRows == 1) eval(slab + (lane % kShPassRows) * kShRow);
        return;
    }
    for (int h = 0; h < 2; ++h) {
        const int r = min(kShPassRows, rows - kShPassRows * h);
        __builtin_amdgcn_wave_barrier();
        if (r > 0) sh_slab_load(slab, shs + (size_t)M3 * (row0 + kShPassRows * h), r, M3, lane);
        __builtin_amdgcn_wave_barrier();
        if (i < prm.P && lane / kShPassRows == h) eval(slab + (lane % kShPassRows) * kShRow);
    }
}

template <bool WANT_J, int KV>
__global__ __launch_bounds__(kBlock) void preprocess_views_kernel(
    d3ga_raster_params prm, const float *__restrict__ means3D, const float *__restrict__ shs,
    const float *__restrict__ colors_precomp, const float *__restrict__ opacities, const float *__restrict__ scales,
    const float *__restrict__ rotations, const float *__restrict__ cov3D_precomp, ViewCams<KV> cams, GeomBuf geom ,
    uint32_t *__restrict__ tile_count, uint32_t *__restrict__ counters, int32_t *__restrict__ radii ,
    int tile_row0, int gyv, size_t pv ) {
    extern __shared__ __attribute__((aligned(16))) char smem[];
    __shared__ int s_box[4];
    float *s_sh = reinterpret_cast<float *>(smem);
    uint32_t *s_cnt = reinterpret_cast<uint32_t *>(smem);
    const int tid = threadIdx.x;
    const int i = blockIdx.x * kBlock + tid;
    float pc6[6] = {0.f, 0.f, 0.f, 0.f, 0.f, 0.f}, pop = 0.f;
    const bool pre = cov3D_precomp != nullptr && pv == 0;
    if (pre && i < prm.P) {
#pragma unroll
        for (int k = 0; k < 6; ++k) pc6[k] = cov3D_precomp[6 * (size_t)i + k];
        pop = opacities[i];
    }
    ShColJ cj[KV];
#pragma unroll
    for (int v = 0; v < KV; ++v) cj[v] = ShColJ{0.f, 0.f, 0.f, 0.f, 0.f, 0.f, 0.f, 0.f, 0.f, 0.f, 0.f, 0.f};
    staged_sh_colour_views<WANT_J, KV>(prm, means3D, pv, shs, cams, s_sh, cj);
    const int gx = (prm.W + kTile - 1) / kTile;
#pragma unroll
    for (int v = 0; v < KV; ++v) {
        __syncthreads();
        TileRect tr = {false, 0, 0, 0, 0};
        if (i < prm.P) {
            const size_t og = pv * v;
            tr = preprocess_view<false>(prm, view_cam(prm, cams.vm[v], cams.pm[v], cams.cp[v], false), i, means3D + 3 * og, nullptr, true,
                                        cj[v], pre, pc6, pop, colors_precomp, opacities, scales ? scales + 3 * og : nullptr,
                                        rotations ? rotations + 4 * og : nullptr, cov3D_precomp ? cov3D_precomp + 6 * og : nullptr,
                                        geom_view(geom, prm.P, v), tile_row0 + v * gyv, radii + (size_t)prm.P * v, WANT_J, gx, 0);
        }
        tile_histogram(s_box, s_cnt, tr, gx, tile_count, counters);
    }
}

template <bool WANT_J>
__global__ __launch_bounds__(kBlock) void recolor_kernel(d3ga_raster_params prm, const float *__restrict__ means3D,
                                                         const float *__restrict__ shs,
                                                         const float *__restrict__ colors_precomp,
                                                         const float *__restrict__ campos, GeomBuf src, GeomBuf dst) {
    extern __shared__ __attribute__((aligned(16))) char smem[];
    float *s_sh = reinterpret_cast<float *>(smem);
    const int i = blockIdx.x * kBlock + threadIdx.x;
    const int M3 = 3 * prm.M;
    const bool staged = shs != nullptr && sh_staged(prm.M);
    ShColJ cj = {0.f, 0.f, 0.f, 0.f, 0.f, 0.f, 0.f, 0.f, 0.f, 0.f, 0.f, 0.f};
    float acc[3] = {0.f, 0.f, 0.f};
    if (staged) staged_sh_colour<WANT_J>(prm, means3D, shs, campos, s_sh, acc, cj);
    if (i >= prm.P) return;
    if (WANT_J) {
        acc[0] = cj.a0; acc[1] = cj.a1; acc[2] = cj.a2;
        dcol_store(dst.dcol, dst.dcol_stride, i, cj);
    }
    const uint2 rc = src.rect[i];
    const bool visible = rect_visible(rc.x, rc.y);
    const float depth = src.depth[i];
    dst.depth[i] = depth;
    dst.conic_o[i] = src.conic_o[i];
    dst.xyh[i] = src.xyh[i];
    dst.rect[i] = rc;
#pragma unroll
    for (int k = 0; k < 6; ++k) dst.cov3D[6 * (size_t)i + k] = src.cov3D[6 * (size_t)i + k];
    float rgb[3] = {0.f, 0.f, 0.f};
    uint8_t mask = 0;
    if (visible) {
        if (colors_precomp) {
            rgb[0] = colors_precomp[3 * (size_t)i]; rgb[1] = colors_precomp[3 * (size_t)i + 1];
            rgb[2] = colors_precomp[3 * (size_t)i + 2];
        } else {
            if (!staged) {
                float B[16];
                sh_view_basis(prm, means3D, i, campos, B);
                sh_accumulate(B, shs + (size_t)M3 * i, 0, 16, (prm.sh_degree + 1) * (prm.sh_degree + 1), acc);
            }
#pragma unroll
            for (int c = 0; c < 3; ++c) {
                const float v = acc[c] + 0.5f;
                if (v < 0.f) mask |= (uint8_t)(1u << c);
                rgb[c] = fmaxf(v, 0.f);
            }
        }
    }
    dst.rgb_invd[i] = make_float4(rgb[0], rgb[1], rgb[2], visible ? 1.0f / depth : 0.f);
    dst.clamped[i] = mask;
}

__device__ __forceinline__ ViewRecs view_recs(const GeomBuf &g, const float *acc) {
    return ViewRecs{reinterpret_cast<const uint32_t *>(g.rect), acc, g.clamped, reinterpret_cast<const float *>(g.conic_o), g.dcol,
                    g.dcol_stride};
}

template <bool WIN>
__global__ __launch_bounds__(kBlock) void preprocess_bwd_kernel(
    d3ga_raster_params prm, const float *__restrict__ means3D, const float *__restrict__ shs,
    const float *__restrict__ scales, const float *__restrict__ rotations, const float *__restrict__ viewmatrix,
    const float *__restrict__ projmatrix, const float *__restrict__ campos, GeomBuf geom,
    const float *__restrict__ acc, float *__restrict__ dL_dmeans3D, float *__restrict__ dL_dmeans2D,
    float *__restrict__ dL_dopacity, float *__restrict__ dL_dsh, float *__restrict__ dL_dcolors,
    float *__restrict__ dL_dcov3D, float *__restrict__ dL_dscales, float *__restrict__ dL_drots,
    const float *__restrict__ cov3D_precomp, int accum ) {
    const ViewCam cam = view_cam(prm, viewmatrix, projmatrix, campos, WIN);
    extern __shared__ __attribute__((aligned(16))) char smem[];
    float *s_sh = reinterpret_cast<float *>(smem);
    const int tid = threadIdx.x, lane = tid & 63, wave = tid >> 6;
    const int i = blockIdx.x * kBlock + tid;
    const int M3 = 3 * prm.M;
    const bool staged = shs != nullptr && sh_staged(prm.M);
    const int row0 = blockIdx.x * kBlock + wave * 64;
    const int rows = min(64, prm.P - row0);
    float *slab = s_sh + wave * kShSlab;
    const bool full48 = M3 == 48 && rows == 64;
    uint2 rc = make_uint2(0u, 0u);
    AccRec ar;
    float c6[6] = {0.f, 0.f, 0.f, 0.f, 0.f, 0.f};
    uint8_t clampmask = 0;
    float act_opacity = 0.f;
    if (i < prm.P) {
        rc = geom.rect[i];
        ar = acc_load(acc, i, prm.acc_self_clearing);
#pragma unroll
        for (int k = 0; k < 6; ++k) c6[k] = (cov3D_precomp ? cov3D_precomp : geom.cov3D)[6 * (size_t)i + k];
        clampmask = geom.clamped[i];
        act_opacity = geom.conic_o[i].w;
    }
    const bool have_j = staged && !prm.forward_only;
    ShColJ jd = {0.f, 0.f, 0.f, 0.f, 0.f, 0.f, 0.f, 0.f, 0.f, 0.f, 0.f, 0.f};
    if (have_j && i < prm.P) jd = dcol_load(geom.dcol, geom.dcol_stride, i);
    if (staged && !have_j) {
        if (full48) sh_rows48_to_slab<64>(slab, sh_rows48_load<64>(shs + (size_t)48 * row0, lane), lane);
        else if (rows > 0) sh_slab_load(slab, shs + (size_t)M3 * row0, rows, M3, lane);
        __builtin_amdgcn_wave_barrier();
    }
    if (i < prm.P) {
        const bool visible = rect_visible(rc.x, rc.y);
        if (!visible) {
#pragma unroll
            for (int k = 0; k < 12; ++k) ar.a[k] = 0.f;
#pragma unroll
            for (int k = 0; k < 6; ++k) c6[k] = 0.f;
            act_opacity = 0.f;
        }
        if (staged)
            preprocess_bwd_one(prm, cam, i, visible, means3D, slab + lane * kShRow, scales, rotations, c6, clampmask, ar.a, dL_dmeans3D,
                               dL_dmeans2D, dL_dopacity, dL_dsh ? slab + lane * kShRow : nullptr, dL_dcolors, dL_dcov3D, dL_dscales,
                               dL_drots, act_opacity, have_j, jd, accum);
        else
            preprocess_bwd_one(prm, cam, i, visible, means3D, shs ? shs + (size_t)M3 * i : nullptr, scales, rotations, c6, clampmask,
                               ar.a, dL_dmeans3D, dL_dmeans2D, dL_dopacity, dL_dsh ? dL_dsh + (size_t)M3 * i : nullptr, dL_dcolors,
                               dL_dcov3D, dL_dscales, dL_drots, act_opacity, false, ShColJ(), accum);
    }
    if (staged && dL_dsh) {
        __builtin_amdgcn_wave_barrier();
        if (full48) sh_rows48_store<64>(slab, dL_dsh + (size_t)48 * row0, lane);
        else if (rows > 0) sh_slab_store(slab, dL_dsh + (size_t)M3 * row0, rows, M3, lane);
    }
}

constexpr int kMaxGroup = 8;
template <bool WIN>
__global__ __launch_bounds__(kBlock) void preprocess_bwd_views_kernel(
    d3ga_raster_params prm, int kv, const float *__restrict__ means3D, bool sh_path, const float *__restrict__ scales,
    const float *__restrict__ rotations, const float *__restrict__ cov3D_precomp, ViewCams<kMaxGroup> cams, GeomBuf geom ,
    const float *__restrict__ acc , float *__restrict__ dL_dmeans3D, float *__restrict__ dL_dmeans2D ,
    float *__restrict__ dL_dopacity, float *__restrict__ dL_dsh, float *__restrict__ dL_dcolors, float *__restrict__ dL_dcov3D,
    float *__restrict__ dL_dscales, float *__restrict__ dL_drots, bool accum,
    size_t pv ,
    bool pva ) {
    extern __shared__ __attribute__((aligned(16))) char smem[];
    float *s_sh = reinterpret_cast<float *>(smem);
    const int tid = threadIdx.x, lane = tid & 63, wave = tid >> 6;
    const int i = blockIdx.x * kBlock + tid;
    const int M3 = 3 * prm.M;
    const int row0 = blockIdx.x * kBlock + wave * 64;
    const int rows = min(64, prm.P - row0);
    float *slab = s_sh + wave * kShSlab;
    if (i < prm.P)
        preprocess_bwd_views_one(prm, i, kv, WIN, cams, view_recs(geom, acc), means3D, cov3D_precomp ? cov3D_precomp : geom.cov3D,
                                 scales, rotations, sh_path, pv, pva, accum, dL_dmeans3D, dL_dmeans2D, dL_dopacity, dL_dcolors,
                                 dL_dcov3D, dL_dscales, dL_drots, sh_path && dL_dsh ? slab + lane * kShRow : nullptr);
    if (sh_path && dL_dsh) {
        __builtin_amdgcn_wave_barrier();
        if (accum) {
            const int nvec = rows > 0 ? rows * M3 / 4 : 0;
            float4 *dst = reinterpret_cast<float4 *>(dL_dsh + (size_t)M3 * row0);
            for (int v = lane; v < nvec; v += 64) {
                const int e = 4 * v, r = e / M3, c = e - r * M3;
                const float4 x = *reinterpret_cast<const float4 *>(slab + r * kShRow + c);
                float4 y = dst[v];
                y.x += x.x; y.y += x.y; y.z += x.z; y.w += x.w;
                dst[v] = y;
            }
        } else if (M3 == 48 && rows == 64) sh_rows48_store<64>(slab, dL_dsh + (size_t)48 * row0, lane);
        else if (rows > 0) sh_slab_store(slab, dL_dsh + (size_t)M3 * row0, rows, M3, lane);
    }
}

__global__ __launch_bounds__(kBlock) void sh_grad_from_views_kernel(
    int P, int M, int sh_degree, int n_views, const float *__restrict__ means3D, int64_t means_stride ,
    const float *__restrict__ g_views, int64_t g_stride, const float *__restrict__ campos_views, int64_t campos_stride, float scale,
    float *__restrict__ dL_dsh) {
    extern __shared__ __attribute__((aligned(16))) char smem[];
    float *s_sh = reinterpret_cast<float *>(smem);
    const int tid = threadIdx.x, lane = tid & 63, wave = tid >> 6;
    const int i = blockIdx.x * kBlock + tid;
    const int M3 = 3 * M;
    const bool staged = sh_staged(M);
    const int row0 = blockIdx.x * kBlock + wave * 64;
    const int rows = min(64, P - row0);
    float *slab = s_sh + wave * kShSlab;
    if (i < P) {
        float out[48];
#pragma unroll
        for (int k = 0; k < 48; ++k) out[k] = 0.f;
        const int nb = (sh_degree + 1) * (sh_degree + 1);
        for (int v = 0; v < n_views; ++v) {
            const float *g = g_views + v * g_stride + 3 * (size_t)i;
            const float g0 = g[0], g1 = g[1], g2 = g[2];
            if (g0 == 0.f && g1 == 0.f && g2 == 0.f) continue;
            const V3 mean = ld3(means3D + v * means_stride, i);
            const float *cp = campos_views + v * campos_stride;
            const V3 d0 = mean - v3(cp[0], cp[1], cp[2]);
            const float inv = 1.0f / sqrtf(dot(d0, d0));
            float B[16];
            sh_basis(sh_degree, d0.x * inv, d0.y * inv, d0.z * inv, B);
#pragma unroll
            for (int k = 0; k < 16; ++k)
                if (k < nb) {
                    out[3 * k] += B[k] * g0; out[3 * k + 1] += B[k] * g1; out[3 * k + 2] += B[k] * g2;
                }
        }
        float *row = staged ? slab + lane * kShRow : nullptr;
#pragma unroll
        for (int k = 0; k < 48; ++k)
            if (k < M3) {
                if (staged) row[k] = out[k] * scale;
                else dL_dsh[(size_t)M3 * i + k] = out[k] * scale;
            }
    }
    if (staged) {
        __syncthreads();
        if (rows > 0) sh_slab_store(slab, dL_dsh + (size_t)M3 * row0, rows, M3, lane);
    }
}

__global__ __launch_bounds__(kBlock) void mark_visible_kernel(int P, const float *__restrict__ means3D,
                                                              const float *__restrict__ viewmatrix,
                                                              uint8_t *__restrict__ visible) {
    const int i = blockIdx.x * kBlock + threadIdx.x;
    if (i >= P) return;
    visible[i] = xform_point(viewmatrix, ld3(means3D, i)).z > kNear ? 1 : 0;
}

}

using namespace d3ga;

static int validate(const d3ga_raster_params *prm) {
    if (!prm) return D3GA_E_NULL;
    if (prm->P < 0 || prm->W <= 0 || prm->H <= 0 || prm->M < 0 || prm->M > 16) return D3GA_E_SIZE;
    if (prm->sh_degree < 0 || prm->sh_degree > 3) return D3GA_E_CONFIG;
    if (prm->n_views < 0) return D3GA_E_SIZE;
    if (grid_x(prm) > 65535 || (int64_t)grid_y(prm) * n_views_of(prm) > 65535) return D3GA_E_SIZE;
    if ((int64_t)prm->P * n_views_of(prm) >= (1ll << 31)) return D3GA_E_SIZE;
    return D3GA_OK;
}

static bool staged(const d3ga_raster_params *prm, const float *shs) { return shs != nullptr && sh_staged(prm->M); }
static bool leaves_dcol(const d3ga_raster_params *prm, const float *shs) { return staged(prm, shs) && !prm->forward_only; }
static size_t lds_bytes(bool staged, size_t slabs, size_t floor = 0) { return staged && slabs > floor ? slabs : floor; }
static int cam_stride(const d3ga_raster_params *prm) {
    return prm->tanfovx > 0.f ? 3 : (is_windowed(prm) ? D3GA_CAMERA_SLOT_WINDOWED_FLOATS : 5);
}
template <int K>
static ViewCams<K> view_cams(const float *vm, const float *pm, const float *cp, int stride, int v0, int kv) {
    ViewCams<K> c;
    for (int q = 0; q < K; ++q) {
        const int v = v0 + (q < kv ? q : 0);
        c.vm[q] = vm + 16 * (size_t)v; c.pm[q] = pm + 16 * (size_t)v; c.cp[q] = cp + (size_t)stride * v;
    }
    return c;
}
template <class T>
static T *at(T *p, size_t n, size_t r) { return p ? p + n * r : nullptr; }

extern "C" int d3ga_raster_preprocess(const d3ga_raster_params *prm, const float *means3D, const float *shs,
                                      const float *colors_precomp, const float *opacities, const float *scales,
                                      const float *rotations, const float *cov3D_precomp, const float *viewmatrix,
                                      const float *projmatrix, const float *campos, void *geom, void *binning,
                                      int64_t d_capacity, int32_t *radii, d3ga_stream_t stream) {
    D3GA_TRY(validate(prm));
    if (!geom || !binning || !viewmatrix || !projmatrix || !campos) return D3GA_E_NULL;
    if (d_capacity < 0) return D3GA_E_SIZE;
    hipStream_t s = (hipStream_t)stream;
    const int views = n_views_of(prm), gyv = grid_y(prm);
    const int64_t tiles = (int64_t)grid_x(prm) * gyv * views;
    const bool wnd = is_windowed(prm);
    BinBuf bin = carve_bin(binning, tiles, d_capacity);
    D3GA_HIP(zero_async(bin.counters, 256 + align256(4 * tiles), s));
    if (wnd) hipLaunchKernelGGL(window_table_kernel, dim3((views + 63) / 64), dim3(64), 0, s, *prm, campos, views, win_table(binning, tiles, d_capacity));
    if (prm->P == 0) return D3GA_OK;
    if ((shs != nullptr) == (colors_precomp != nullptr)) return D3GA_E_CONFIG;
    const bool pva = views > 1 && prm->per_view_appearance;
    if (pva && shs) return D3GA_E_CONFIG;
    const bool sr = scales != nullptr && rotations != nullptr;
    if (sr == (cov3D_precomp != nullptr)) return D3GA_E_CONFIG;
    if (shs && (prm->sh_degree + 1) * (prm->sh_degree + 1) > prm->M) return D3GA_E_CONFIG;
    if (!means3D || !opacities || !radii) return D3GA_E_NULL;
    const GeomBuf g = carve_geom(geom, (int64_t)prm->P * views);
    const size_t lds = lds_bytes(staged(prm, shs), kShHalfLdsBytes, (size_t)kWinTiles * 4);
    const bool want_j = leaves_dcol(prm, shs);
    const int cs = cam_stride(prm);
    const size_t pv = (views > 1 && prm->per_view_geometry) ? (size_t)prm->P : 0;
    const size_t pa = pva ? (size_t)prm->P : 0;
    const dim3 grid((prm->P + kBlock - 1) / kBlock), block(kBlock);
    int v0 = 0;
    const bool grouped = views > 1 && !pva && !wnd && staged(prm, shs);
    auto launch_group = [&](auto kv) {
        constexpr int KV = decltype(kv)::value;
        const size_t og = pv * v0;
        hipLaunchKernelGGL((want_j ? preprocess_views_kernel<true, KV> : preprocess_views_kernel<false, KV>), grid, block, lds, s, *prm,
                           at(means3D, 3, og), shs, colors_precomp, opacities, at(scales, 3, og), at(rotations, 4, og),
                           at(cov3D_precomp, 6, og), view_cams<KV>(viewmatrix, projmatrix, campos, cs, v0, KV), geom_view(g, prm->P, v0),
                           bin.tile_count, bin.counters, radii + (size_t)prm->P * v0, v0 * gyv, gyv, pv);
        v0 += KV;
    };
    while (grouped && views - v0 >= 2) {
        const int left = views - v0;
        if (left >= 4 && left != 5) launch_group(std::integral_constant<int, 4>());
        else if (left == 3 || left == 5) launch_group(std::integral_constant<int, 3>());
        else launch_group(std::integral_constant<int, 2>());
    }
    const auto kernel = want_j ? (wnd ? preprocess_kernel<true, true> : preprocess_kernel<true, false>)
                               : (wnd ? preprocess_kernel<false, true> : preprocess_kernel<false, false>);
    for (int v = v0; v < views; ++v) {
        const ViewCams<1> c = view_cams<1>(viewmatrix, projmatrix, campos, cs, v, 1);
        const size_t og = pv * v, oa = pa * v;
        hipLaunchKernelGGL(kernel, grid, block, lds, s, *prm, at(means3D, 3, og), shs, at(colors_precomp, 3, oa), opacities + oa,
                           at(scales, 3, og), at(rotations, 4, og), at(cov3D_precomp, 6, og), c.vm[0], c.pm[0], c.cp[0],
                           geom_view(g, prm->P, v), bin.tile_count, bin.counters, radii + (size_t)prm->P * v, v * gyv);
    }
    return check_launch(s, prm->debug & 0xff);
}

extern "C" int d3ga_raster_recolor(const d3ga_raster_params *prm, const float *means3D, const float *shs,
                                   const float *colors_precomp, const float *campos, const void *geom_src,
                                   void *geom_dst, d3ga_stream_t stream) {
    D3GA_TRY(validate(prm));
    if (n_views_of(prm) > 1 || is_windowed(prm)) return D3GA_E_CONFIG;
    if (prm->P == 0) return D3GA_OK;
    if (!geom_src || !geom_dst || geom_src == geom_dst) return D3GA_E_NULL;
    if ((shs != nullptr) == (colors_precomp != nullptr)) return D3GA_E_CONFIG;
    if (shs && (!means3D || !campos)) return D3GA_E_NULL;
    if (shs && (prm->sh_degree + 1) * (prm->sh_degree + 1) > prm->M) return D3GA_E_CONFIG;
    hipStream_t s = (hipStream_t)stream;
    const GeomBuf src = carve_geom(const_cast<void *>(geom_src), prm->P), dst = carve_geom(geom_dst, prm->P);
    hipLaunchKernelGGL(leaves_dcol(prm, shs) ? recolor_kernel<true> : recolor_kernel<false>, dim3((prm->P + kBlock - 1) / kBlock),
                       dim3(kBlock), lds_bytes(staged(prm, shs), kShHalfLdsBytes), s, *prm, means3D, shs, colors_precomp, campos, src, dst);
    return check_launch(s, prm->debug & 0xff);
}

extern "C" int d3ga_raster_preprocess_bwd(const d3ga_raster_params *prm, const float *means3D, const float *shs,
                                          const float *scales, const float *rotations, const float *cov3D_precomp,
                                          const float *viewmatrix, const float *projmatrix, const float *campos,
                                          const void *geom, const float *acc, float *dL_dmeans3D, float *dL_dmeans2D,
                                          float *dL_dopacity, float *dL_dsh, float *dL_dcolors, float *dL_dcov3D,
                                          float *dL_dscales, float *dL_drots, d3ga_stream_t stream) {
    D3GA_TRY(validate(prm));
    if (prm->P == 0) return D3GA_OK;
    if (!means3D || !viewmatrix || !projmatrix || !campos || !geom || !acc || !dL_dmeans3D) return D3GA_E_NULL;
    if (dL_dsh && !shs) return D3GA_E_NULL;
    if (shs && !dL_dsh && !dL_dcolors) return D3GA_E_NULL;
    if ((dL_dscales != nullptr) != (dL_drots != nullptr)) return D3GA_E_CONFIG;
    if (dL_dscales && (!scales || !rotations)) return D3GA_E_NULL;
    if (!cov3D_precomp && !(scales && rotations)) return D3GA_E_NULL;
    hipStream_t s = (hipStream_t)stream;
    const int views = n_views_of(prm);
    const bool pva = views > 1 && prm->per_view_appearance;
    if (pva && shs) return D3GA_E_CONFIG;
    const GeomBuf g = carve_geom(const_cast<void *>(geom), (int64_t)prm->P * views);
    const size_t lds = lds_bytes(staged(prm, shs), kShLdsBytes);
    const bool win = is_windowed(prm);
    const int cs = cam_stride(prm);
    const dim3 grid((prm->P + kBlock - 1) / kBlock), block(kBlock);
    const size_t pv = prm->per_view_geometry ? (size_t)prm->P : 0;
    auto launch_view = [&](int v, float *dsh, float *dcol, int accum) {
        const ViewCams<1> c = view_cams<1>(viewmatrix, projmatrix, campos, cs, v, 1);
        const size_t o = (size_t)prm->P * v, og = pv * v;
        hipLaunchKernelGGL(win ? preprocess_bwd_kernel<true> : preprocess_bwd_kernel<false>, grid, block, lds, s, *prm, at(means3D, 3, og),
                           shs, at(scales, 3, og), at(rotations, 4, og), c.vm[0], c.pm[0], c.cp[0], geom_view(g, prm->P, v),
                           acc + D3GA_ACC_STRIDE * o, dL_dmeans3D + 3 * og, at(dL_dmeans2D, 3, o), dL_dopacity, dsh, dcol,
                           at(dL_dcov3D, 6, og), at(dL_dscales, 3, og), at(dL_drots, 4, og), at(cov3D_precomp, 6, og), accum);
    };
    if (views == 1) {
        launch_view(0, dL_dsh, dL_dcolors, 0);
        return check_launch(s, prm->debug);
    }
    if (shs ? (dL_dsh != nullptr && leaves_dcol(prm, shs)) : true) {
        for (int v0 = 0; v0 < views; v0 += kMaxGroup) {
            const int kv = views - v0 < kMaxGroup ? views - v0 : kMaxGroup;
            const size_t o = (size_t)prm->P * v0, og = pv * v0, oa = pva ? o : 0;
            hipLaunchKernelGGL(win ? preprocess_bwd_views_kernel<true> : preprocess_bwd_views_kernel<false>, grid, block, lds, s, *prm, kv,
                               at(means3D, 3, og), shs != nullptr, at(scales, 3, og), at(rotations, 4, og), at(cov3D_precomp, 6, og),
                               view_cams<kMaxGroup>(viewmatrix, projmatrix, campos, cs, v0, kv), geom_view(g, prm->P, v0),
                               acc + D3GA_ACC_STRIDE * o, dL_dmeans3D + 3 * og, at(dL_dmeans2D, 3, o), at(dL_dopacity, 1, oa), dL_dsh,
                               at(dL_dcolors, 3, oa), at(dL_dcov3D, 6, og), at(dL_dscales, 3, og), at(dL_drots, 4, og), v0 > 0, pv, pva);
        }
        return check_launch(s, prm->debug);
    }
    if (pva) return D3GA_E_CONFIG;
    if (shs && !dL_dcolors) return D3GA_E_NULL;
    if (prm->factor_rows != 0 && prm->factor_rows < prm->P) return D3GA_E_SIZE;
    const size_t fr = prm->factor_rows > 0 ? (size_t)prm->factor_rows : (size_t)prm->P;
    for (int v = 0; v < views; ++v) launch_view(v, nullptr, shs ? dL_dcolors + 3 * fr * v : dL_dcolors, v > 0 ? (pv ? 1 : 3) : 0);
    D3GA_TRY(check_launch(s, prm->debug));
    if (shs && dL_dsh) {
        hipLaunchKernelGGL(sh_grad_from_views_kernel, grid, block, lds_bytes(sh_staged(prm->M), kShLdsBytes), s, prm->P, prm->M,
                           prm->sh_degree, views, means3D, (int64_t)(3 * pv), dL_dcolors, (int64_t)(3 * fr), campos, (int64_t)cs, 1.0f, dL_dsh);
        return check_launch(s, prm->debug);
    }
    return D3GA_OK;
}

extern "C" int d3ga_sh_grad_from_views(int32_t P, int32_t M, int32_t sh_degree, int32_t n_views, const float *means3D,
                                       const float *g_views, int64_t g_stride, const float *campos_views,
                                       int64_t campos_stride, float scale, float *dL_dsh, d3ga_stream_t stream) {
    if (P < 0 || M < 1 || M > 16 || n_views < 0) return D3GA_E_SIZE;
    if (sh_degree < 0 || sh_degree > 3 || (sh_degree + 1) * (sh_degree + 1) > M) return D3GA_E_CONFIG;
    if (P == 0) return D3GA_OK;
    if (!means3D || !dL_dsh || (n_views > 0 && (!g_views || !campos_views))) return D3GA_E_NULL;
    hipStream_t s = (hipStream_t)stream;
    hipLaunchKernelGGL(sh_grad_from_views_kernel, dim3((P + kBlock - 1) / kBlock), dim3(kBlock), lds_bytes(sh_staged(M), kShLdsBytes), s, P, M, sh_degree,
                       n_views, means3D, (int64_t)0, g_views, g_stride, campos_views, campos_stride, scale, dL_dsh);
    return check_launch(s, 0);
}

extern "C" int d3ga_raster_mark_visible(int32_t P, const float *means3D, const float *viewmatrix, uint8_t *visible,
                                        d3ga_stream_t stream) {
    if (P < 0) return D3GA_E_SIZE;
    if (P == 0) return D3GA_OK;
    if (!means3D || !viewmatrix || !visible) return D3GA_E_NULL;
    hipLaunchKernelGGL(mark_visible_kernel, dim3((P + kBlock - 1) / kBlock), dim3(kBlock), 0, (hipStream_t)stream, P,
                       means3D, viewmatrix, visible);
    return check_launch((hipStream_t)stream, 0);
}
```

### d3ga_amd/rasterizer.py

```python
import ctypes
import os
from typing import NamedTuple, Optional

import torch
from torch import nn

from . import _lib
from ._lib import RasterParams, check, dptr, require_cuda, stream_handle


class GaussianRasterizationSettings(NamedTuple):
    image_height: int
    image_width: int
    tanfovx: float
    tanfovy: float
    bg: torch.Tensor
    scale_modifier: float
    viewmatrix: torch.Tensor
    projmatrix: torch.Tensor
    sh_degree: int
    campos: torch.Tensor
    prefiltered: bool
    debug: bool
    antialiasing: bool = False


_policy = {"mode": "auto", "static": 0}
_hwm = {}
_last = {}
_last_img = {}
_capture_log = None


def set_capacity_policy(mode, capacity=0):
    if mode not in ("auto", "static"):
        raise ValueError(mode)
    _policy["mode"] = mode
    _policy["static"] = int(capacity)


def _record_forward(dev, binning, cap):
    _last[dev.index] = (binning, cap)
    if _capture_log is not None:
        _capture_log.append((binning, cap))


def _forward_with_capacity(P, k, dev, launch):
    static = _policy["mode"] == "static"
    cap = _policy["static"] if static else k * max(_hwm.get(dev.index, 0), 4 * P + 1024)
    while True:
        geom, binning, img = launch(cap)
        _record_forward(dev, binning, cap)
        if static:
            break
        cnt = binning[:32].view(torch.int32)[:2].cpu().tolist()
        D = cnt[0] & 0xFFFFFFFF
        _hwm[dev.index] = max(_hwm.get(dev.index, 0), int(D * 1.25 / k) + 1024)
        if not cnt[1]:
            break
        cap = k * _hwm[dev.index]
    return cap, geom, binning, img


_acc_policy = {"persistent": False}
_acc_cache = {}


def set_accumulator_policy(mode):
    if mode not in ("fresh", "persistent"):
        raise ValueError(mode)
    _acc_policy["persistent"] = mode == "persistent"
    if mode == "fresh":
        _acc_cache.clear()


_l1_policy = {"fused_value": os.environ.get("D3GA_L1_VALUE", "fused") != "separate"}


def l1_mean_forward(image, target, cell, out, dev):
    L = _lib.lib()
    ws = torch.empty(_lib.LOSS_PARTIALS, dtype=torch.float32, device=dev)
    if cell is None:
        check(L.d3ga_l1_mean_fwd_ws(image.numel(), dptr(image), dptr(target), dptr(out), dptr(ws), stream_handle()), "d3ga_l1_mean_fwd_ws")
    else:
        check(L.d3ga_l1_mean_fwd_ws_cell(image.numel(), dptr(image), dptr(cell), dptr(out), dptr(ws), stream_handle()),
              "d3ga_l1_mean_fwd_ws_cell")


def _accumulator(P, dev):
    if not _acc_policy["persistent"] or P == 0:
        return torch.empty((P, _lib.ACC_STRIDE), dtype=torch.float32, device=dev), False
    key = (dev.index, P)
    buf = _acc_cache.get(key)
    if buf is None:
        if len(_acc_cache) > 8:
            _acc_cache.clear()
        buf = _acc_cache[key] = torch.zeros((P, _lib.ACC_STRIDE), dtype=torch.float32, device=dev)
    return buf, True


def last_counters(device=None):
    dev = torch.cuda.current_device() if device is None else torch.device(device).index
    c = _last[dev][0][:32].view(torch.int32)[:4].cpu().tolist()
    return {"D": c[0] & 0xFFFFFFFF, "overflow": bool(c[1]), "max_tile": c[2] & 0xFFFFFFFF, "visible": c[3]}


class StageTimer:

    def __init__(self):
        self.enabled = False
        self.records = []
        self.burst = {}

    def reset(self):
        self.records = []

    def stage(self, name, fn):
        if not self.enabled:
            return fn()
        reps = int(self.burst.get(name, 1))
        a, b = torch.cuda.Event(enable_timing=True), torch.cuda.Event(enable_timing=True)
        a.record()
        r = fn()
        for _ in range(reps - 1):
            fn()
        b.record()
        self.records.append((name, a, b, reps))
        return r

    def summary(self):
        per = {}
        for name, a, b, reps in self.records:
            per.setdefault(name, []).append((a.elapsed_time(b) / reps, reps))
        out = {}
        for name, ts in per.items():
            med = sorted(t for t, _ in ts)[len(ts) // 2]
            kept = [(t, r) for t, r in ts if t <= 5.0 * med] or ts
            out[name] = (sum(r for _, r in kept), sum(t for t, _ in kept) / len(kept))
        return out


stage_timer = StageTimer()


_scratch_sizes = {}
_prm_cache = {}


def _scratch(P, W, H, k, cap, device, forward_only, windowed, binning=True):
    key = (P, W, H, k, cap, bool(forward_only), bool(windowed))
    sz = _scratch_sizes.get(key)
    if sz is None:
        sizes = (ctypes.c_int64 * 3)()
        name = "d3ga_raster_scratch_bytes_window" if windowed else "d3ga_raster_scratch_bytes_views"
        check(getattr(_lib.lib(), name)(P, W, H, k, cap, int(bool(forward_only)), sizes), name)
        if len(_scratch_sizes) > 64:
            _scratch_sizes.clear()
        sz = _scratch_sizes[key] = tuple(int(n) for n in sizes)
    new = lambda n: torch.empty(n, dtype=torch.uint8, device=device)
    return [new(sz[0]), new(sz[1]) if binning else None, new(sz[2])]


def _params(P, M, sh_degree, W, H, tanfovx, tanfovy, scale_modifier, antialiasing, prefiltered, debug, opacity_activation,
            forward_only, n_views=0, per_view_geometry=False, per_view_appearance=False, per_view_background=False):
    key = (P, M, sh_degree, W, H, tanfovx, tanfovy, scale_modifier, antialiasing, prefiltered, debug, opacity_activation,
           forward_only, n_views, per_view_geometry, per_view_appearance, per_view_background)
    prm = _prm_cache.get(key)
    if prm is None:
        if len(_prm_cache) > 64:
            _prm_cache.clear()
        prm = _prm_cache[key] = RasterParams(
            P=P, M=M, sh_degree=sh_degree, W=W, H=H, tanfovx=tanfovx, tanfovy=tanfovy, scale_modifier=scale_modifier,
            antialiasing=int(antialiasing), prefiltered=int(prefiltered), debug=int(debug),
            opacity_activation=_ACTIVATIONS[opacity_activation], forward_only=int(forward_only), n_views=n_views,
            per_view_geometry=int(per_view_geometry), per_view_appearance=int(per_view_appearance),
            per_view_background=int(per_view_background))
        prm.cache_key = key
    return prm


def _prm_variant(prm, **fields):
    key = (prm.cache_key, tuple(fields.items()))
    p2 = _prm_cache.get(key)
    if p2 is None:
        if len(_prm_cache) > 64:
            _prm_cache.clear()
        p2 = _prm_cache[key] = RasterParams(**{f: getattr(prm, f) for f, _ in RasterParams._fields_})
        for f, value in fields.items():
            setattr(p2, f, value)
        p2.cache_key = key
    return p2


def _f32(t, device):
    if t is None:
        return None
    if t.dtype != torch.float32 or t.device != device:
        t = t.to(device=device, dtype=torch.float32)
    return t if t.is_contiguous() else t.contiguous()


def _views_of(prm):
    return max(prm.n_views, 1)


def _composite_forward(prm, cap, windowed, bg, geom, binning, img, color, invdepth, pair, l1):
    L, st, pp = _lib.lib(), stream_handle(), ctypes.byref(prm)
    if pair is not None:
        colors2, bg2, color2 = pair
        stage_timer.stage("composite_fwd", lambda: check(L.d3ga_raster_composite_fwd2(
            pp, dptr(bg), dptr(bg2), dptr(geom), dptr(colors2), dptr(binning), cap, dptr(img), dptr(color), dptr(color2),
            dptr(invdepth), st), "d3ga_raster_composite_fwd2"))
    elif l1 is not None:
        target, cell, loss = l1
        ws = torch.empty(4 * _views_of(prm) * ((prm.W + 15) // 16 + windowed) * ((prm.H + 15) // 16 + windowed),
                         dtype=torch.float32, device=color.device)
        stage_timer.stage("composite_fwd", lambda: check(L.d3ga_raster_composite_fwd_l1(
            pp, dptr(bg), dptr(geom), dptr(binning), cap, dptr(img), dptr(color), dptr(invdepth),
            dptr(None if cell is not None else target), dptr(cell), dptr(loss), dptr(ws), st), "d3ga_raster_composite_fwd_l1"))
    else:
        stage_timer.stage("composite_fwd", lambda: check(L.d3ga_raster_composite_fwd(
            pp, dptr(bg), dptr(geom), dptr(binning), cap, dptr(img), dptr(color), dptr(invdepth), st), "d3ga_raster_composite_fwd"))


def _launch_forward(prm, cap, windowed, gauss, cam, bg, color, radii, invdepth, pair=None, l1=None):
    means3D, sh, colors_precomp, opacities, scales, rotations, cov3Ds_precomp = gauss
    view, proj, campos = cam
    k = _views_of(prm)
    geom, binning, img = _scratch(prm.P, prm.W, prm.H, k, cap, color.device, prm.forward_only, windowed)
    L = _lib.lib()
    if stage_timer.enabled or k > 1 or pair is not None or l1 is not None:
        st, pp = stream_handle(), ctypes.byref(prm)
        stage_timer.stage("preprocess", lambda: check(L.d3ga_raster_preprocess(
            pp, dptr(means3D), dptr(sh), dptr(colors_precomp), dptr(opacities), dptr(scales), dptr(rotations),
            dptr(cov3Ds_precomp), dptr(view), dptr(proj), dptr(campos), dptr(geom), dptr(binning), cap,
            dptr(radii), st), "d3ga_raster_preprocess"))
        stage_timer.stage("bin_sort", lambda: check(L.d3ga_raster_bin_sort(
            pp, dptr(geom), dptr(binning), cap, st), "d3ga_raster_bin_sort"))
        _composite_forward(prm, cap, windowed, bg, geom, binning, img, color, invdepth, pair, l1)
    else:
        check(L.d3ga_raster_forward(ctypes.byref(prm), dptr(means3D), dptr(sh), dptr(colors_precomp),
                                    dptr(opacities), dptr(scales), dptr(rotations), dptr(cov3Ds_precomp),
                                    dptr(view), dptr(proj), dptr(campos), dptr(bg), dptr(geom), dptr(binning),
                                    dptr(img), cap, dptr(color), dptr(radii), dptr(invdepth), stream_handle()),
              "d3ga_raster_forward")
    return geom, binning, img


def _grad_buffers(prm, has_sh, from_sr, dev, exchanged, geo, opac, col, lead):
    new = lambda *shape: torch.empty(shape, dtype=torch.float32, device=dev)
    P, cut = prm.P, None
    if not exchanged:
        g_means3D, g_opac = new(*geo, 3), new(*opac)
        g_sh = new(P, prm.M, 3) if has_sh else None
        g_col = None if col is None else new(*col)
        g_cov = None if from_sr else new(*geo, 6)
        g_scales = new(*geo, 3) if from_sr else None
        g_rots = new(*geo, 4) if from_sr else None
    else:
        widths = [3, 1] + ([3, 4] if from_sr else [6]) + ([] if has_sh else [3])
        flat = new(P * sum(widths))
        parts, off = [], 0
        for w in widths:
            parts.append(flat[off:off + P * w].view(P, w))
            off += P * w
        g_means3D, g_opac = parts[0], parts[1]
        g_scales, g_rots = (parts[2], parts[3]) if from_sr else (None, None)
        g_cov = None if from_sr else parts[2]
        g_sh = factor = None
        by_name = {"means3D": g_means3D, "opacities": g_opac}
        by_name.update({"scales": g_scales, "rotations": g_rots} if from_sr else {"cov3D_precomp": g_cov})
        if not has_sh:
            g_col = by_name["colors_precomp"] = parts[-1]
        else:
            g_col = factor = new(*lead, P + 1, 3)
            if _views_of(prm) > 1:
                prm = _prm_variant(prm, factor_rows=P + 1)
        cut = (flat, factor, by_name)
    return g_means3D, g_opac, g_sh, g_col, g_cov, g_scales, g_rots, cut, prm


def _launch_backward(prm, cap, gauss, cam, bg, geom, binning, img, grad_color, grads, pair=None, g_invd=None, l1=None):
    means3D, sh, scales, rotations, cov3Ds_precomp = gauss
    view, proj, campos = cam
    g_means3D, g_means2D, g_opac, g_sh, g_col, g_cov, g_scales, g_rots = grads
    k = _views_of(prm)
    acc, self_clearing = _accumulator(k * prm.P, means3D.device)
    if self_clearing != bool(prm.acc_self_clearing):
        prm = _prm_variant(prm, acc_self_clearing=int(self_clearing))
    L = _lib.lib()
    if stage_timer.enabled or k > 1 or pair is not None or g_invd is not None:
        st, pp = stream_handle(), ctypes.byref(prm)
        if not self_clearing:
            acc.zero_()
        if pair is not None:
            colors2, bg2, grad_color2 = pair
            stage_timer.stage("composite_bwd", lambda: check(L.d3ga_raster_composite_bwd2(
                pp, dptr(bg), dptr(bg2), dptr(geom), dptr(colors2), dptr(binning), cap, dptr(img), dptr(grad_color),
                dptr(grad_color2), dptr(acc), st), "d3ga_raster_composite_bwd2"))
        elif g_invd is not None:
            stage_timer.stage("composite_bwd", lambda: check(L.d3ga_raster_composite_bwd_depth(
                pp, dptr(bg), dptr(geom), dptr(binning), cap, dptr(img), dptr(grad_color), dptr(g_invd), dptr(acc), st),
                "d3ga_raster_composite_bwd_depth"))
        elif l1 is not None:
            image, target, cell, g_loss = l1
            stage_timer.stage("composite_bwd", lambda: check(L.d3ga_raster_composite_bwd_l1(
                pp, dptr(bg), dptr(geom), dptr(binning), cap, dptr(img), dptr(image), dptr(target), dptr(cell),
                dptr(g_loss), dptr(grad_color), dptr(acc), st), "d3ga_raster_composite_bwd_l1"))
        else:
            stage_timer.stage("composite_bwd", lambda: check(L.d3ga_raster_composite_bwd(
                pp, dptr(bg), dptr(geom), dptr(binning), cap, dptr(img), dptr(grad_color), dptr(acc), st),
                "d3ga_raster_composite_bwd"))
        stage_timer.stage("preprocess_bwd", lambda: check(L.d3ga_raster_preprocess_bwd(
            pp, dptr(means3D), dptr(sh), dptr(scales), dptr(rotations), dptr(cov3Ds_precomp), dptr(view), dptr(proj),
            dptr(campos), dptr(geom), dptr(acc), dptr(g_means3D), dptr(g_means2D), dptr(g_opac), dptr(g_sh),
            dptr(g_col), dptr(g_cov), dptr(g_scales), dptr(g_rots), st), "d3ga_raster_preprocess_bwd"))
    elif l1 is not None:
        image, target, cell, g_loss = l1
        check(L.d3ga_raster_backward_l1(
            ctypes.byref(prm), dptr(means3D), dptr(sh), dptr(scales), dptr(rotations), dptr(cov3Ds_precomp),
            dptr(view), dptr(proj), dptr(campos), dptr(bg), dptr(geom), dptr(binning), cap, dptr(img),
            dptr(image), dptr(target), dptr(cell), dptr(g_loss), dptr(grad_color), dptr(acc), dptr(g_means3D),
            dptr(g_means2D), dptr(g_opac), dptr(g_sh), dptr(g_col), dptr(g_cov), dptr(g_scales), dptr(g_rots),
            stream_handle()), "d3ga_raster_backward_l1")
    else:
        check(L.d3ga_raster_backward(
            ctypes.byref(prm), dptr(means3D), dptr(sh), dptr(scales), dptr(rotations), dptr(cov3Ds_precomp),
            dptr(view), dptr(proj), dptr(campos), dptr(bg), dptr(geom), dptr(binning), cap, dptr(img),
            dptr(grad_color), dptr(acc), dptr(g_means3D), dptr(g_means2D), dptr(g_opac), dptr(g_sh), dptr(g_col),
            dptr(g_cov), dptr(g_scales), dptr(g_rots), stream_handle()), "d3ga_raster_backward")


def _sh_grad_from_factors(gathered, P, M, sh_degree, means3D, scale):
    g_sh = torch.empty((P, M, 3), dtype=torch.float32, device=means3D.device)
    g = gathered.view(-1, P + 1, 3)
    check(_lib.lib().d3ga_sh_grad_from_views(P, M, sh_degree, g.shape[0], dptr(means3D), dptr(g), 3 * (P + 1), dptr(g[0, P]),
                                             3 * (P + 1), scale, dptr(g_sh), stream_handle()), "d3ga_sh_grad_from_views")
    return g_sh


def _exchange_gradients(sync, prm, cut, campos, means3D):
    P = prm.P
    flat, factor, by_name = cut
    if factor is not None:
        factor.view(-1, P + 1, 3)[:, P].copy_(campos.reshape(_views_of(prm), -1)[:, :3])
    if getattr(sync, "deferred", False):
        sync.park(flat, factor, by_name,
                  None if factor is None else {"P": P, "M": prm.M, "sh_degree": prm.sh_degree, "means3D": means3D})
        return True, None
    gathered = sync.exchange(flat, factor)
    return False, None if factor is None else _sh_grad_from_factors(gathered, P, prm.M, prm.sh_degree, means3D, sync.scale)


_reuse = {"enabled": False}
_geom_cache = {}


def set_geometry_reuse(enabled):
    _reuse["enabled"] = bool(enabled)
    if not enabled:
        _geom_cache.clear()


def clear_geometry_cache():
    _geom_cache.clear()


class geometry_reuse:

    def __enter__(self):
        self._was = _reuse["enabled"]
        _reuse["enabled"] = True
        return self

    def __exit__(self, *exc):
        _reuse["enabled"] = self._was
        _geom_cache.clear()
        return False


def _tkey(t):
    return None if t is None else (t.data_ptr(), t._version, tuple(t.shape))


def _geometry_key(prm, cap_mode, tensors):
    return (prm.P, prm.W, prm.H, prm.tanfovx, prm.tanfovy, prm.scale_modifier, prm.prefiltered, prm.opacity_activation, prm.antialiasing, cap_mode) + tuple(
        _tkey(t) for t in tensors)


def _empty_to_none(t):
    return None if (t is None or t.numel() == 0) else t


def _check_exactly_one(shs, colors_precomp, scales, rotations, cov3D_precomp):
    if (shs is None) == (colors_precomp is None):
        raise Exception("Please provide excatly one of either SHs or precomputed colors!")
    if ((scales is None or rotations is None) and cov3D_precomp is None) or (
            (scales is not None or rotations is not None) and cov3D_precomp is not None):
        raise Exception("Please provide exactly one of either scale/rotation pair or precomputed 3D covariance!")


def _admit_grad_sync(grad_sync, P):
    if grad_sync is None or P == 0 or not (grad_sync.world > 1 or getattr(grad_sync, "always", False)):
        return None
    return grad_sync


def _verify_sync_inputs(sync, means3D, opacities, colors_precomp, sh, cov3Ds_precomp, scales, rotations):
    if sync is not None and hasattr(sync, "verify_inputs"):
        sync.verify_inputs({"means3D": means3D, "opacities": opacities, "colors_precomp": colors_precomp,
                            "shs": sh, "cov3D_precomp": cov3Ds_precomp, "scales": scales, "rotations": rotations})


class _RasterizeGaussians(torch.autograd.Function):
    @staticmethod
    def forward(ctx, means3D, means2D, sh, colors_precomp, opacities, scales, rotations, cov3Ds_precomp,
                raster_settings, grad_sync=None, colors2=None, bg2=None, opacity_activation=None, l1_target=None,
                want_invdepth=True):
        s = raster_settings
        require_cuda(means3D)
        dev = means3D.device
        if means3D.shape[0] > 0:
            sh, colors_precomp, scales, rotations, cov3Ds_precomp = map(
                _empty_to_none, (sh, colors_precomp, scales, rotations, cov3Ds_precomp))
        means3D, sh, colors_precomp, opacities, scales, rotations, cov3Ds_precomp = (
            _f32(t, dev) for t in (means3D, sh, colors_precomp, opacities, scales, rotations, cov3Ds_precomp))
        view, proj, campos, bg = (_f32(t, dev) for t in (s.viewmatrix, s.projmatrix, s.campos, s.bg))
        P = means3D.shape[0]
        dual = colors2 is not None and P > 0
        empty_pair = colors2 is not None and P == 0
        if colors2 is not None:
            colors2, bg2 = _f32(colors2.detach(), dev), _f32(bg2, dev)
        H, W = int(s.image_height), int(s.image_width)
        M = sh.shape[1] if sh is not None else 0
        tfx, tfy = float(s.tanfovx), float(s.tanfovy)
        windowed = tfx == _lib.CAMERA_SLOT_WINDOWED and tfy == _lib.CAMERA_SLOT_WINDOWED and campos.numel() >= 9
        if not (tfx > 0.0 and tfy > 0.0) and not windowed:
            if not (tfx == 0.0 and tfy == 0.0 and campos.numel() >= 5):
                raise ValueError(f"GaussianRasterizationSettings: tanfovx / tanfovy must be positive (got {tfx}, {tfy}); only a "
                                 "camera slot (tanfovx = tanfovy = 0 with a 5-float campos: cameras.CameraSlot) reads them from the device")
        fwd_only = not any(ctx.needs_input_grad[:8])
        prm = _params(P, M, int(s.sh_degree), W, H, tfx, tfy, float(s.scale_modifier), bool(s.antialiasing), bool(s.prefiltered),
                      bool(s.debug), opacity_activation, fwd_only)
        color = torch.empty((3, H, W), dtype=torch.float32, device=dev)
        l1_t = l1_cell = loss = None
        if l1_target is not None:
            from .graph import TensorSlot
            l1_t = l1_target.current if isinstance(l1_target, TensorSlot) else _f32(l1_target, dev)
            l1_cell = l1_target.cell if isinstance(l1_target, TensorSlot) else None
            if tuple(l1_t.shape) != (3, H, W):
                raise ValueError(f"rasterize_gaussians_l1: the target must be (3, {H}, {W}), got {tuple(l1_t.shape)}")
            loss = torch.empty((), dtype=torch.float32, device=dev)
        l1 = (l1_t, l1_cell, loss) if (l1_target is not None and P > 0 and colors2 is None and _l1_policy["fused_value"]) else None
        invdepth = torch.empty((1, H, W), dtype=torch.float32, device=dev) if want_invdepth else None
        radii = torch.empty((P,), dtype=torch.int32, device=dev)
        gauss = (means3D, sh, colors_precomp, opacities, scales, rotations, cov3Ds_precomp)
        cam = (view, proj, campos)
        geo_inputs = (means3D, opacities, scales, rotations, cov3Ds_precomp, view, proj)
        color2 = torch.empty((3, H, W), dtype=torch.float32, device=dev) if dual else None
        pair = (colors2, bg2, color2) if dual else None
        use_cache = _reuse["enabled"] and P > 0 and not dual and not windowed and not torch.cuda.is_current_stream_capturing()
        key = hit = None
        if use_cache:
            key = _geometry_key(prm, ("static", _policy["static"]) if _policy["mode"] == "static" else "auto", geo_inputs)
            hit = _geom_cache.get(dev.index)
        if hit is not None and hit["key"] == key:
            cap, binning, radii = hit["cap"], hit["binning"], hit["radii"]
            geom, _unused, img = _scratch(P, W, H, 1, cap, dev, fwd_only, False, binning=False)
            L, st, pp = _lib.lib(), stream_handle(), ctypes.byref(prm)
            stage_timer.stage("recolor", lambda: check(L.d3ga_raster_recolor(
                pp, dptr(means3D), dptr(sh), dptr(colors_precomp), dptr(campos), dptr(hit["geom"]), dptr(geom), st),
                "d3ga_raster_recolor"))
            _composite_forward(prm, cap, windowed, bg, geom, binning, img, color, invdepth, None, l1)
            _record_forward(dev, binning, cap)
        else:
            cap, geom, binning, img = _forward_with_capacity(P, 1, dev, lambda cap: _launch_forward(
                prm, cap, windowed, gauss, cam, bg, color, radii, invdepth, pair, l1))
            if use_cache:
                _geom_cache[dev.index] = {"key": key, "geom": geom, "binning": binning, "cap": cap, "radii": radii,
                                          "pins": tuple(None if t is None else t.detach() for t in geo_inputs)}
        ctx.prm = prm
        ctx.cap = cap
        ctx.has_means2D = means2D is not None
        ctx.grad_sync = _admit_grad_sync(grad_sync, P)
        _verify_sync_inputs(ctx.grad_sync, means3D, opacities, colors_precomp, sh, cov3Ds_precomp, scales, rotations)
        ctx.dual = dual
        ctx.l1 = l1_target is not None and P > 0 and not dual
        if l1_target is not None and l1 is None:
            l1_mean_forward(color, l1_t, l1_cell, loss, dev)
        _last_img[dev.index] = (img, W, H, geom, P)
        ctx.save_for_backward(means3D, sh, scales, rotations, cov3Ds_precomp, view, proj, campos, bg, geom, binning, img,
                              colors2, bg2, color if ctx.l1 else None, l1_t if ctx.l1 else None, l1_cell if ctx.l1 else None)
        ctx.mark_non_differentiable(radii)
        ctx.set_materialize_grads(False)
        if l1_target is not None:
            return color, radii, invdepth, loss
        if dual:
            return color, radii, invdepth, color2
        if empty_pair:
            return color, radii, invdepth, bg2.reshape(3, 1, 1).expand(3, H, W).contiguous()
        return color, radii, invdepth

    @staticmethod
    def backward(ctx, grad_color, _grad_radii, _grad_invdepth, grad_color2=None):
        (means3D, sh, scales, rotations, cov3Ds_precomp, view, proj, campos, bg, geom, binning, img, colors2,
         bg2, image, l1_t, l1_cell) = ctx.saved_tensors
        prm, dev, P = ctx.prm, means3D.device, means3D.shape[0]
        dual = ctx.dual
        g_loss = None
        if ctx.l1:
            g_loss, grad_color2 = grad_color2, None
            if g_loss is not None:
                g_loss = _f32(g_loss, dev).reshape(1)
        g_invd = None
        if _grad_invdepth is not None:
            if dual or ctx.l1:
                raise NotImplementedError("a gradient of the inverse-depth image is implemented for the single-image rasterizer call only "
                                          "(not for rasterize_gaussians_pair / rasterize_gaussians_l1)")
            g_invd = _f32(_grad_invdepth, dev).reshape(prm.H, prm.W)
        if grad_color is None and g_loss is None and g_invd is None:
            grad_color = torch.zeros((3, prm.H, prm.W), dtype=torch.float32, device=dev)
        grad_color = _f32(grad_color, dev)
        if dual:
            grad_color2 = (torch.zeros_like(grad_color) if grad_color2 is None else _f32(grad_color2, dev))
        has_sh, from_sr, sync = sh is not None, cov3Ds_precomp is None, ctx.grad_sync
        g_means3D, g_opac, g_sh, g_col, g_cov, g_scales, g_rots, cut, prm = _grad_buffers(
            prm, has_sh, from_sr, dev, exchanged=sync is not None, geo=(P,), opac=(P, 1), col=None if has_sh else (P, 3), lead=())
        g_means2D = torch.empty((P, 3), dtype=torch.float32, device=dev)
        _launch_backward(prm, ctx.cap, (means3D, sh, scales, rotations, cov3Ds_precomp), (view, proj, campos), bg, geom, binning, img,
                         grad_color, (g_means3D, g_means2D, g_opac, g_sh, g_col, g_cov, g_scales, g_rots),
                         (colors2, bg2, grad_color2) if dual else None, g_invd,
                         (image, l1_t, l1_cell, g_loss) if g_loss is not None else None)
        if sync is not None:
            parked, g_sh = _exchange_gradients(sync, prm, cut, campos, means3D)
            if parked:
                return (None, g_means2D if ctx.has_means2D else None) + (None,) * 13
            if has_sh:
                g_col = None
        return (g_means3D, g_means2D if ctx.has_means2D else None, g_sh, g_col, g_opac, g_scales, g_rots, g_cov, None,
                None, None, None, None, None, None)

# ... 101 lines not shown
```

### include/d3ga.h

```cpp
#ifndef D3GA_H
#define D3GA_H

#include <stdint.h>

#ifdef __cplusplus
extern "C" {
#endif

#if defined(__GNUC__)
#pragma GCC visibility push(default)
#endif

#define D3GA_VERSION 111

#define D3GA_OK 0
#define D3GA_E_NULL (-1)
#define D3GA_E_SIZE (-2)
#define D3GA_E_CONFIG (-3)
#define D3GA_E_CAPACITY (-4)

typedef void *d3ga_stream_t;

int d3ga_version(void);
const char *d3ga_status_string(int status);
#define D3GA_KNOB_COMPOSITE_VARIANT 0
#define D3GA_KNOB_MERGE_SLOTS 1
#define D3GA_KNOB_TILE_ASSIGN 2
#define D3GA_KNOB_BWD_SPLIT 3
#define D3GA_KNOB_SORT_MERGE 4
#define D3GA_KNOB_SSIM_IMPL 5
#define D3GA_KNOB_WGRAD_WS 6
#define D3GA_KNOB_CHAIN_ABL 7
#define D3GA_KNOB_CHAIN_GRID 8
#define D3GA_KNOB_COUNT 9
#define D3GA_KNOB_DEFAULT (-2147483647 - 1)
int d3ga_debug_set(int32_t key, int32_t value);
int d3ga_debug_defaults(int32_t *out, int32_t n);

int d3ga_lbs_cage_fwd(int V, int K, const float *tmpl, const float *delta, const float *joint_mats,
                      const int32_t *skin_idx, const float *skin_w, const float *Rh, const float *Th, float *out,
                      d3ga_stream_t stream);
int d3ga_lbs_cage_bwd(int V, int K, const float *joint_mats, const int32_t *skin_idx, const float *skin_w,
                      const float *Rh, const float *grad_out, float *grad_delta, d3ga_stream_t stream);
typedef struct d3ga_lbs_pose_grad {
    int32_t J;
    int32_t n_chunks;
    int64_t n_entries;
    const float *tmpl;
    const float *delta;
    const int32_t *chunk_ptr;
    const int32_t *chunk_range;
    const int32_t *entries;
    uint32_t *counter;
    void *scratch;
    float *g_joint_mats;
    float *g_Rh;
    float *g_Th;
} d3ga_lbs_pose_grad;
int d3ga_lbs_pose_scratch_bytes(int V, int32_t n_chunks, int32_t fused, int64_t *bytes);
int d3ga_lbs_cage_bwd_pose(int V, int K, const float *joint_mats, const int32_t *skin_idx, const float *skin_w,
                           const float *Rh, const float *grad_out, float *grad_delta, const d3ga_lbs_pose_grad *pose,
                           d3ga_stream_t stream);

#define D3GA_DEFORM_LOG_SCALES 1
#define D3GA_DEFORM_GRAD_PER_TET 2
int d3ga_cage_deform_fwd(int P, const float *tetpoints, const int32_t *tetras, const int32_t *tetra_id,
                         const float *barys, const float *canon_grad, const float *scales, const float *rots,
                         float *means3D, float *cov6, d3ga_stream_t stream);
int d3ga_cage_deform_bwd(int P, int V, const float *tetpoints, const int32_t *tetras, const int32_t *tetra_id,
                         const float *barys, const float *canon_grad, const float *scales, const float *rots,
                         const float *g_means, const float *g_cov6, float *g_tetpoints, float *g_barys,
                         float *g_scales, float *g_rots, const int32_t *vert_start, const int32_t *vert_items,
                         float *corner_grads, d3ga_stream_t stream);
int d3ga_cage_deform_fwd_ex(int P, const float *tetpoints, const int32_t *tetras, const int32_t *tetra_id,
                            const float *barys, const float *canon_grad, const float *scales, const float *rots,
                            const float *delta_barys, int32_t flags, float *means3D, float *cov6, d3ga_stream_t stream);
int d3ga_cage_deform_bwd_ex(int P, int V, const float *tetpoints, const int32_t *tetras, const int32_t *tetra_id,
                            const float *barys, const float *canon_grad, const float *scales, const float *rots,
                            const float *delta_barys, int32_t flags, const float *g_means, const float *g_cov6,
                            float *g_tetpoints, float *g_barys, float *g_scales, float *g_rots,
                            const int32_t *vert_start, const int32_t *vert_items, float *corner_grads,
                            d3ga_stream_t stream);

int d3ga_cage_deform_bwd_merged(int P, int V, const float *tetpoints, const int32_t *tetras, const int32_t *tetra_id,
                                const float *barys, const float *canon_grad, const float *scales, const float *rots,
                                const float *delta_barys, int32_t flags, const float *g_means, const float *g_cov6,
                                float *g_tetpoints, float *g_barys, float *g_scales, float *g_rots,
                                const uint16_t *item_pos, const int32_t *seg_ptr, const uint16_t *seg_begin,
                                int32_t n_segments, const int32_t *vert_start, const int32_t *vert_parts, float *partials,
                                d3ga_stream_t stream);

int d3ga_cage_deform_bwd_merged_lbs(int P, int V, const float *tetpoints, const int32_t *tetras, const int32_t *tetra_id,
                                    const float *barys, const float *canon_grad, const float *scales, const float *rots,
                                    const float *delta_barys, int32_t flags, const float *g_means, const float *g_cov6,
                                    float *g_tetpoints, float *g_barys, float *g_scales, float *g_rots,
                                    const uint16_t *item_pos, const int32_t *seg_ptr, const uint16_t *seg_begin,
                                    int32_t n_segments, const int32_t *vert_start, const int32_t *vert_parts, float *partials,
                                    int K, const float *joint_mats, const int32_t *skin_idx, const float *skin_w, const float *Rh,
                                    const float *g_tetpoints_extra, float *g_delta, d3ga_stream_t stream);
int d3ga_cage_deform_bwd_merged_lbs_pose(int P, int V, const float *tetpoints, const int32_t *tetras, const int32_t *tetra_id,
                                         const float *barys, const float *canon_grad, const float *scales, const float *rots,
                                         const float *delta_barys, int32_t flags, const float *g_means, const float *g_cov6,
                                         float *g_tetpoints, float *g_barys, float *g_scales, float *g_rots,
                                         const uint16_t *item_pos, const int32_t *seg_ptr, const uint16_t *seg_begin,
                                         int32_t n_segments, const int32_t *vert_start, const int32_t *vert_parts, float *partials,
                                         int K, const float *joint_mats, const int32_t *skin_idx, const float *skin_w, const float *Rh,
                                         const float *g_tetpoints_extra, float *g_delta, const d3ga_lbs_pose_grad *pose,
                                         d3ga_stream_t stream);

int d3ga_fem_energy_fwd(int T, const float *tetpoints, const int32_t *tetras, const float *Dn_inv, float *energy,
                        d3ga_stream_t stream);
int d3ga_fem_energy_bwd(int T, int V, const float *tetpoints, const int32_t *tetras, const float *Dn_inv,
                        const float *g_energy, float *g_tetpoints, d3ga_stream_t stream);

#define D3GA_BODY_MAX_JOINTS 64
#define D3GA_BODY_MAX_SHAPE 32
#define D3GA_BODY_LD_ALIGN 2048
#define D3GA_BODY_SAVED_FLOATS(J) (27 * (J) + 16)
typedef struct d3ga_body_model {
    int32_t V, J;
    int32_t n_shape, n_expr;
    int32_t n_hand_pca;
    int32_t ld;
    int32_t n_levels;
    int32_t reserved;
    const float *v_template;
    const float *dirs;
    const int32_t *w_ptr, *w_joint;
    const float *w_val;
    const int32_t *wt_ptr, *wt_vert;
    const float *wt_val;
    const float *J0;
    const float *Jdirs;
    const int32_t *parents, *level_ptr, *level_joint, *child_ptr, *child_joint;
    const float *hand_comps, *hand_mean;
} d3ga_body_model;
int d3ga_body_model_scratch_bytes(const d3ga_body_model *model, int32_t B, int64_t *fwd_bytes, int64_t *bwd_bytes);
int d3ga_body_model_fwd(const d3ga_body_model *model, int32_t B, int32_t pose_width, const float *poses, const float *shapes,
                        const float *expr, const float *Rh, const float *Th, float *verts, float *T, float *A, float *bs,
                        float *saved, void *scratch, int64_t scratch_bytes, d3ga_stream_t stream);
int d3ga_body_model_bwd(const d3ga_body_model *model, int32_t B, int32_t pose_width, const float *saved, const float *T,
                        const float *bs, const float *g_verts, const float *g_T, const float *g_A, const float *g_bs,
                        float *g_poses, float *g_shapes, float *g_expr, float *g_Rh, float *g_Th, void *scratch,
                        int64_t scratch_bytes, d3ga_stream_t stream);

typedef struct d3ga_raster_params {
    int32_t P;
    int32_t M;
    int32_t sh_degree;
    int32_t W, H;
    float tanfovx, tanfovy;
    float scale_modifier;
    int32_t antialiasing;
    int32_t prefiltered;
    int32_t debug;
    int32_t opacity_activation;
    int32_t forward_only;
    int32_t acc_self_clearing;
    int32_t n_views;
    int32_t per_view_geometry;
    int32_t factor_rows;
    int32_t per_view_appearance;
    int32_t per_view_background;
} d3ga_raster_params;
#define D3GA_OPACITY_SIGMOID 1

#define D3GA_CAMERA_SLOT_WINDOWED (-1.0f)
#define D3GA_CAMERA_SLOT_WINDOWED_FLOATS 9

int d3ga_raster_scratch_bytes(int32_t P, int32_t W, int32_t H, int64_t d_capacity, int64_t sizes[3]);
int64_t d3ga_raster_img_bytes(int32_t W, int32_t H, int64_t d_capacity, int32_t forward_only);
int d3ga_raster_scratch_bytes_views(int32_t P, int32_t W, int32_t H, int32_t n_views, int64_t d_capacity, int32_t forward_only,
                                    int64_t sizes[3]);

int d3ga_raster_scratch_bytes_window(int32_t P, int32_t W, int32_t H, int32_t n_views, int64_t d_capacity, int32_t forward_only,
                                     int64_t sizes[3]);
int d3ga_raster_binning_layout_window(int32_t W, int32_t H, int32_t n_views, int64_t d_capacity, int64_t offsets[7]);

int d3ga_raster_binning_layout(int32_t W, int32_t H, int64_t d_capacity, int64_t offsets[6]);
int d3ga_raster_img_layout(int32_t W, int32_t H, int64_t offsets[2]);
int d3ga_raster_img_layout_blocks(int32_t W, int32_t H, int64_t offsets[2]);

#define D3GA_CNT_D 0
#define D3GA_CNT_OVERFLOW 1
#define D3GA_CNT_MAXTILE 2
#define D3GA_CNT_VISIBLE 3
#define D3GA_CNT_BIG 4
#define D3GA_CNT_HUGE 5
#define D3GA_CNT_MID 6
#define D3GA_CNT_HEAVY 7

int d3ga_raster_preprocess(const d3ga_raster_params *prm, const float *means3D, const float *shs,
                           const float *colors_precomp, const float *opacities, const float *scales,
                           const float *rotations, const float *cov3D_precomp, const float *viewmatrix,
                           const float *projmatrix, const float *campos, void *geom, void *binning,
                           int64_t d_capacity, int32_t *radii, d3ga_stream_t stream);
int d3ga_raster_bin_sort(const d3ga_raster_params *prm, void *geom, void *binning, int64_t d_capacity,
                         d3ga_stream_t stream);
int d3ga_raster_composite_fwd(const d3ga_raster_params *prm, const float *bg, const void *geom, const void *binning,
                              int64_t d_capacity, void *img, float *out_color, float *out_invdepth,
                              d3ga_stream_t stream);
#define D3GA_ACC_STRIDE 16
int d3ga_raster_composite_bwd(const d3ga_raster_params *prm, const float *bg, const void *geom, const void *binning,
                              int64_t d_capacity, const void *img, const float *dL_dpix, float *acc,
                              d3ga_stream_t stream);
int d3ga_raster_composite_bwd_depth(const d3ga_raster_params *prm, const float *bg, const void *geom, const void *binning,
                                    int64_t d_capacity, const void *img, const float *dL_dpix, const float *dL_dinvdepth,
                                    float *acc, d3ga_stream_t stream);

int d3ga_raster_composite_fwd2(const d3ga_raster_params *prm, const float *bg, const float *bg2, const void *geom,
                               const float *colors2, const void *binning, int64_t d_capacity, void *img, float *out_color,
                               float *out_color2, float *out_invdepth, d3ga_stream_t stream);
int d3ga_raster_composite_bwd2(const d3ga_raster_params *prm, const float *bg, const float *bg2, const void *geom,
                               const float *colors2, const void *binning, int64_t d_capacity, const void *img,
                               const float *dL_dpix, const float *dL_dpix2, float *acc, d3ga_stream_t stream);

int d3ga_raster_composite_fwd_l1(const d3ga_raster_params *prm, const float *bg, const void *geom, const void *binning,
                                 int64_t d_capacity, void *img, float *out_color, float *out_invdepth, const float *target,
                                 const void *target_cell, float *loss, float *partials, d3ga_stream_t stream);
int d3ga_raster_composite_bwd_l1(const d3ga_raster_params *prm, const float *bg, const void *geom, const void *binning,
                                 int64_t d_capacity, const void *img, const float *image, const float *target,
                                 const void *target_cell, const float *g_loss, const float *dL_dpix, float *acc,
                                 d3ga_stream_t stream);
int d3ga_raster_backward_l1(const d3ga_raster_params *prm, const float *means3D, const float *shs, const float *scales,
                            const float *rotations, const float *cov3D_precomp, const float *viewmatrix,
                            const float *projmatrix, const float *campos, const float *bg, const void *geom,
                            const void *binning, int64_t d_capacity, const void *img, const float *image,
                            const float *target, const void *target_cell, const float *g_loss, const float *dL_dpix,
                            float *acc, float *dL_dmeans3D, float *dL_dmeans2D, float *dL_dopacity, float *dL_dsh,
                            float *dL_dcolors, float *dL_dcov3D, float *dL_dscales, float *dL_drots, d3ga_stream_t stream);
int d3ga_raster_recolor(const d3ga_raster_params *prm, const float *means3D, const float *shs,
                        const float *colors_precomp, const float *campos, const void *geom_src, void *geom_dst,
                        d3ga_stream_t stream);

int d3ga_raster_preprocess_bwd(const d3ga_raster_params *prm, const float *means3D, const float *shs,
                               const float *scales, const float *rotations, const float *cov3D_precomp,
                               const float *viewmatrix, const float *projmatrix, const float *campos,
                               const void *geom, const float *acc, float *dL_dmeans3D, float *dL_dmeans2D,
                               float *dL_dopacity, float *dL_dsh, float *dL_dcolors, float *dL_dcov3D,
                               float *dL_dscales, float *dL_drots, d3ga_stream_t stream);

int d3ga_raster_forward(const d3ga_raster_params *prm, const float *means3D, const float *shs,
                        const float *colors_precomp, const float *opacities, const float *scales,
                        const float *rotations, const float *cov3D_precomp, const float *viewmatrix,
                        const float *projmatrix, const float *campos, const float *bg, void *geom, void *binning,
                        void *img, int64_t d_capacity, float *out_color, int32_t *radii, float *out_invdepth,
                        d3ga_stream_t stream);
int d3ga_raster_backward(const d3ga_raster_params *prm, const float *means3D, const float *shs, const float *scales,
                         const float *rotations, const float *cov3D_precomp, const float *viewmatrix,
                         const float *projmatrix, const float *campos, const float *bg, const void *geom,
                         const void *binning, int64_t d_capacity, const void *img, const float *dL_dpix, float *acc,
                         float *dL_dmeans3D, float *dL_dmeans2D, float *dL_dopacity, float *dL_dsh,
                         float *dL_dcolors, float *dL_dcov3D, float *dL_dscales, float *dL_drots,
                         d3ga_stream_t stream);

int d3ga_sh_grad_from_views(int32_t P, int32_t M, int32_t sh_degree, int32_t n_views, const float *means3D,
                            const float *g_views, int64_t g_stride, const float *campos_views, int64_t campos_stride,
                            float scale, float *dL_dsh, d3ga_stream_t stream);

int d3ga_raster_mark_visible(int32_t P, const float *means3D, const float *viewmatrix, uint8_t *visible,
                             d3ga_stream_t stream);

int d3ga_l1_mean_fwd(int64_t n, const float *a, const float *b, float *out, d3ga_stream_t stream);
#define D3GA_LOSS_PARTIALS 2048
int d3ga_l1_mean_fwd_ws(int64_t n, const float *a, const float *b, float *out, float *partials, d3ga_stream_t stream);
int d3ga_l1_mean_bwd(int64_t n, const float *a, const float *b, const float *g, float *grad_a, d3ga_stream_t stream);
int d3ga_l1_mean_fwd_ws_cell(int64_t n, const float *a, const float *const *b_cell, float *out, float *partials,
                             d3ga_stream_t stream);
int d3ga_l1_mean_bwd_cell(int64_t n, const float *a, const float *const *b_cell, const float *g, float *grad_a,
                          d3ga_stream_t stream);

int d3ga_ssim_fwd(int32_t C, int32_t H, int32_t W, const float *img1, const float *img2, float *out, float *Dm,
                  float *Dq1, float *Dq12, d3ga_stream_t stream);
int d3ga_ssim_bwd(int32_t C, int32_t H, int32_t W, const float *img1, const float *img2, const float *Dm,
                  const float *Dq1, const float *Dq12, const float *g, float *grad_img1, d3ga_stream_t stream);
int d3ga_ssim_l1_fwd(int32_t C, int32_t H, int32_t W, const float *img1, const float *img2, float *out, float *Dm,
                     float *Dq1, float *Dq12, float *out_l1, d3ga_stream_t stream);
int d3ga_ssim_l1_bwd(int32_t C, int32_t H, int32_t W, const float *img1, const float *img2, const float *Dm,
                     const float *Dq1, const float *Dq12, const float *g, const float *g_l1, float *grad_img1,
                     d3ga_stream_t stream);

#define D3GA_BLUR_PARTIALS 6144
int d3ga_blur_mix_fwd(int32_t C, int32_t H, int32_t W, int32_t n_cameras, const float *img, const float *weights_raw,
                      const int32_t *cam_idx, float *out, d3ga_stream_t stream);
int d3ga_blur_mix_bwd(int32_t C, int32_t H, int32_t W, int32_t n_cameras, const float *img, const float *weights_raw,
                      const int32_t *cam_idx, const float *grad_out, float *grad_img, float *grad_weights_raw,
                      float *partials, d3ga_stream_t stream);
int d3ga_compose_target(int32_t C, int32_t H, int32_t W, const float *image, const float *alpha, const float *silhouette,
                        const void *boundary_fg, int32_t boundary_is_float, const float *bg, float *gt_image,
                        float *gt_silhouette, d3ga_stream_t stream);

#define D3GA_OPTIM_CHUNK 8192
#define D3GA_OPTIM_ALIGNED16 1
typedef struct d3ga_optim_chunk {
    float *p;
    const float *g;
    float *m;
    float *v;
    int32_t n;
    int32_t tensor;
    int32_t flags;
    int32_t reserved;
} d3ga_optim_chunk;
typedef struct d3ga_optim_tensor {
    float *step;
    int32_t group;
    int32_t reserved;
} d3ga_optim_tensor;
int d3ga_optim_scratch_bytes(int32_t n_chunks, int32_t n_tensors, int32_t n_groups, int64_t *out);
int d3ga_optim_clip_adam_step(const d3ga_optim_chunk *table, int32_t n_chunks, const d3ga_optim_tensor *tensor_state,
                              int32_t n_tensors, const double *group_hparams, int32_t n_groups, float max_norm,
                              void *scratch, float *grad_norm_out, d3ga_stream_t stream);

int d3ga_selftest_row_scan(int n, const float *in, float *out, d3ga_stream_t stream);
int d3ga_selftest_alpha(int32_t P, const void *geom, int n, const int32_t *gid, const int32_t *px, const int32_t *py,
                        uint8_t *ok, float *alpha, d3ga_stream_t stream);

int d3ga_compute_bary(int P, int T, const float *points, const float *tetra_corners, float *barys,
                      int32_t *tetra_id, uint8_t *active, d3ga_stream_t stream);

int d3ga_compute_bary_grid(int P, const float *points, const float *tetra_corners, const int32_t *cell_start,
                           const int32_t *cell_tets, const float *origin_h, const int32_t *dims, float *barys,
                           int32_t *tetra_id, float *min_weight, d3ga_stream_t stream);

int d3ga_knn3_mean_dist2(int P, const float *points, float *out, d3ga_stream_t stream);
int d3ga_knn3_mean_dist2_grid(int P, const float *points, const int32_t *cell_start, const int32_t *cell_points,
                              const float *origin_h, const int32_t *dims, float *out, d3ga_stream_t stream);

int64_t d3ga_mlp_panel_bytes(int32_t K, int32_t n_out);
int d3ga_mlp_pack_weights(int32_t K, int32_t n_out, const float *W, int64_t ld_k, int64_t ld_n, void *panel,
                          d3ga_stream_t stream);
int d3ga_mlp_linear(int32_t P, int32_t K, int32_t n_out, const float *X, const void *panel, const float *bias,
                    float out_slope, uint32_t *sign_out, const uint32_t *mask_bits, float mask_slope, float *Y,
                    d3ga_stream_t stream);

int64_t d3ga_mlp_chain_panel_bytes(int32_t K, int32_t n_out);
int d3ga_mlp_pack_chain(int32_t K, int32_t n_out, const float *W, int64_t ld_k, int64_t ld_n, void *panel, d3ga_stream_t stream);
int d3ga_mlp_chain_fwd(int32_t P, int32_t K0, const float *X, int32_t L, const int32_t *Ks, const int32_t *Ns,
                       void *const *panels, const float *const *biases, const float *slopes, float *const *outs,
                       uint32_t *const *signs, const uint32_t *const *masks, const float *mask_slopes, d3ga_stream_t stream);
int d3ga_mlp_wgrad(int32_t P, int32_t N, int32_t K, const float *dpre, const float *X, float *dW, float *db,
                   d3ga_stream_t stream);
int d3ga_mlp_wgrad_acc(int32_t P, int32_t N, int32_t K, const float *dpre, const float *X, float *dW, float *db,
                       d3ga_stream_t stream);

int d3ga_field_heads_fwd(int32_t P, int32_t N, int32_t n_heads, const int32_t *width, const int32_t *act, const float *param,
                         const float *pred, float *out, d3ga_stream_t stream);
int d3ga_field_heads_bwd(int32_t P, int32_t N, int32_t n_heads, const int32_t *width, const int32_t *act, const float *param,
                         const float *out, const float *g0, const float *g1, const float *g2, const float *g3, float *d_pred,
                         d3ga_stream_t stream);
int d3ga_view_dirs_fwd(int32_t P, const float *means3D, const float *campos, float *dirs, d3ga_stream_t stream);
int d3ga_view_dirs_bwd(int32_t P, const float *means3D, const float *campos, const float *d_dirs, float *d_means3D,
                       d3ga_stream_t stream);
int d3ga_sh4_encoding_fwd(int32_t P, const float *dirs, float *enc, d3ga_stream_t stream);
int d3ga_sh4_encoding_bwd(int32_t P, const float *dirs, const float *d_enc, float *d_dirs, d3ga_stream_t stream);
int d3ga_color_rows_fwd(int32_t P, int32_t F, const float *dirs, const float *feats, float *x, d3ga_stream_t stream);
int d3ga_color_rows_bwd(int32_t P, int32_t F, const float *dirs, const float *d_x, float *d_dirs, float *d_feats,
                        d3ga_stream_t stream);

#define D3GA_SKEL_MAX_JOINTS 512
#define D3GA_SKEL_SAVED_FLOATS 12
typedef struct d3ga_skeleton {
    int32_t J, n_params;
    int32_t n_levels;
    int32_t n_children;
    const int32_t *parents, *level_ptr, *level_joint, *child_ptr, *child_joint;
    const float *joint_offset;
    const float *joint_rotation;
    const float *transform_offsets;
    const int32_t *csr_ptr, *csr_col;
    const float *csr_val;
    const int32_t *csc_ptr, *csc_row;
    const float *csc_val;
} d3ga_skeleton;
int d3ga_skeleton_check(const d3ga_skeleton *model, int32_t B, int32_t n_sets, int32_t pose_width);
int d3ga_skeleton_fwd(const d3ga_skeleton *model, int32_t B, int32_t n_sets, int32_t pose_width, const float *poses,
                      const float *scales, int32_t scale_rows, const float *direct, const float *bind, float trans_scale,
                      int32_t root_joint, float *states, float *saved, float *mats, float *root, d3ga_stream_t stream);
int d3ga_skeleton_bwd(const d3ga_skeleton *model, int32_t B, int32_t n_sets, int32_t pose_width, int32_t direct_mode,
                      const float *bind, float trans_scale, int32_t root_joint, const float *states, const float *saved,
                      const float *g_states, const float *g_mats, const float *g_root, float *g_poses, float *g_scales,
                      float *g_direct, d3ga_stream_t stream);
int d3ga_skeleton_mats_fwd(int32_t B, int32_t J, const float *bind, const float *states, float *mats, d3ga_stream_t stream);
int d3ga_skeleton_mats_bwd(int32_t B, int32_t J, const float *bind, const float *states, const float *g_mats, float *g_states,
                           d3ga_stream_t stream);

#if defined(__GNUC__)
#pragma GCC visibility pop
#endif
#ifdef __cplusplus
}
#endif
#endif
```

Baseline: 2620.

## Split SH colour evaluation out of preprocess and overlap it with bin sort

Preprocess now computes geometry only when colour splitting applies. The SH colour evaluation is moved into extra workgroups appended to the tile scan and large-tile sort launches, so it fills CUs those small-grid kernels leave idle. A plan function splits the colour units between the two launches based on CU count. This shortens the critical path of preprocess, at the cost of extra LDS setup, template variants and a more complex launch configuration.

```diff
diff --git a/d3ga_amd/_lib.py b/d3ga_amd/_lib.py
--- a/d3ga_amd/_lib.py
+++ b/d3ga_amd/_lib.py
@@ -7,7 +7,8 @@
 ACC_STRIDE = 16
 replay_epoch = [0]
 ABI_VERSION = 111
-KNOBS = ("composite_variant", "merge_slots", "tile_assign", "bwd_split", "sort_merge", "ssim_impl", "wgrad_ws", "chain_abl", "chain_grid")
+KNOBS = ("composite_variant", "merge_slots", "tile_assign", "bwd_split", "sort_merge", "ssim_impl", "wgrad_ws", "chain_abl", "chain_grid",
+         "split_colour", "colour_scan_pct")
 CAMERA_SLOT_WINDOWED = -1.0
 LOSS_PARTIALS = 2048
 BLUR_PARTIALS = 6144
@@ -101,6 +102,9 @@
     "d3ga_raster_img_bytes": ([ctypes.c_int32, ctypes.c_int32, _i64, ctypes.c_int32], _i64),
     "d3ga_raster_preprocess": ([_prm] + [_vp] * 12 + [_i64, _vp, _vp], _i),
     "d3ga_raster_bin_sort": ([_prm, _vp, _vp, _i64, _vp], _i),
+    "d3ga_raster_preprocess_split": ([_prm] + [_vp] * 12 + [_i64, _vp, _vp], _i),
+    "d3ga_raster_bin_sort_colour": ([_prm] + [_vp] * 5 + [_i64, _vp], _i),
+    "d3ga_raster_colour_plan": ([ctypes.c_int32] * 4 + [ctypes.POINTER(ctypes.c_int32)], _i),
     "d3ga_raster_composite_fwd": ([_prm, _vp, _vp, _vp, _i64, _vp, _vp, _vp, _vp], _i),
     "d3ga_raster_composite_bwd": ([_prm, _vp, _vp, _vp, _i64, _vp, _vp, _vp, _vp], _i),
     "d3ga_raster_composite_bwd_depth": ([_prm, _vp, _vp, _vp, _i64, _vp, _vp, _vp, _vp, _vp], _i),
diff --git a/d3ga_amd/csrc/build.py b/d3ga_amd/csrc/build.py
--- a/d3ga_amd/csrc/build.py
+++ b/d3ga_amd/csrc/build.py
@@ -5,7 +5,7 @@
 HERE = os.path.dirname(os.path.abspath(__file__))
 SOURCES = ["deform.hip", "raster_pre.hip", "raster_bin.hip", "raster_composite.hip", "raster_composite_scan.hip", "raster_api.hip", "bary.hip", "loss.hip", "image_tail.hip", "optim.hip", "mlp.hip", "encoding.hip", "body_model.hip", "skeleton.hip"]
 LINK_MAP = os.path.join(HERE, "d3ga.map")
-HEADERS = ["d3ga_math.h", "d3ga_internal.h", "raster_pre_body.h", "composite_common.h", "body_model_math.h", "skeleton_math.h", os.path.join("..", "..", "include", "d3ga.h")]
+HEADERS = ["d3ga_math.h", "d3ga_internal.h", "raster_pre_body.h", "raster_colour.h", "composite_common.h", "body_model_math.h", "skeleton_math.h", os.path.join("..", "..", "include", "d3ga.h")]
 ABL = os.environ.get("D3GA_SCAN_ABL")
 VARIANT = os.environ.get("D3GA_VARIANT")
 DIAG = os.environ.get("D3GA_DIAG") or (("abl" + ABL) if ABL else None) or (("var" + VARIANT.split(":")[0]) if VARIANT else None)
diff --git a/d3ga_amd/csrc/d3ga_internal.h b/d3ga_amd/csrc/d3ga_internal.h
--- a/d3ga_amd/csrc/d3ga_internal.h
+++ b/d3ga_amd/csrc/d3ga_internal.h
@@ -142,6 +142,9 @@
 static inline bool is_windowed(const d3ga_raster_params *prm) { return prm->tanfovx == D3GA_CAMERA_SLOT_WINDOWED; }
 static inline int grid_x(const d3ga_raster_params *prm) { return tiles_x(prm->W) + (is_windowed(prm) ? 1 : 0); }
 static inline int grid_y(const d3ga_raster_params *prm) { return tiles_y(prm->H) + (is_windowed(prm) ? 1 : 0); }
+static inline bool colour_split(const d3ga_raster_params *prm, const float *shs) {
+    return shs != nullptr && prm->P > 0 && n_views_of(prm) == 1 && !is_windowed(prm) && debug_knob(D3GA_KNOB_SPLIT_COLOUR) != 0;
+}
 static inline int4 *win_table(void *binning, int64_t tiles, int64_t dcap) { return (int4 *)((char *)binning + bin_bytes(tiles, dcap)); }
 static inline int64_t win_table_bytes(int64_t views) { return align256(16 * views); }
 
diff --git a/d3ga_amd/csrc/raster_api.hip b/d3ga_amd/csrc/raster_api.hip
--- a/d3ga_amd/csrc/raster_api.hip
+++ b/d3ga_amd/csrc/raster_api.hip
@@ -5,8 +5,8 @@
 namespace d3ga {
 static const int kKnobDefault[D3GA_KNOB_COUNT] = {
      32 | 128,  512,  2,  -1,  -1,
-     1,  1,  0,  0};
-static std::atomic<int> g_knob[D3GA_KNOB_COUNT] = {{32 | 128}, {512}, {2}, {-1}, {-1}, {1}, {1}, {0}, {0}};
+     1,  1,  0,  0,  1,  -1};
+static std::atomic<int> g_knob[D3GA_KNOB_COUNT] = {{32 | 128}, {512}, {2}, {-1}, {-1}, {1}, {1}, {0}, {0}, {1}, {-1}};
 int debug_knob(int key) { return (key >= 0 && key < D3GA_KNOB_COUNT) ? g_knob[key].load(std::memory_order_relaxed) : 0; }
 }
 
@@ -143,9 +143,9 @@
                                    const float *projmatrix, const float *campos, const float *bg, void *geom,
                                    void *binning, void *img, int64_t d_capacity, float *out_color, int32_t *radii,
                                    float *out_invdepth, d3ga_stream_t stream) {
-    D3GA_TRY(d3ga_raster_preprocess(prm, means3D, shs, colors_precomp, opacities, scales, rotations, cov3D_precomp,
-                                    viewmatrix, projmatrix, campos, geom, binning, d_capacity, radii, stream));
-    D3GA_TRY(d3ga_raster_bin_sort(prm, geom, binning, d_capacity, stream));
+    D3GA_TRY(d3ga_raster_preprocess_split(prm, means3D, shs, colors_precomp, opacities, scales, rotations, cov3D_precomp,
+                                          viewmatrix, projmatrix, campos, geom, binning, d_capacity, radii, stream));
+    D3GA_TRY(d3ga_raster_bin_sort_colour(prm, means3D, shs, campos, geom, binning, d_capacity, stream));
     return d3ga_raster_composite_fwd(prm, bg, geom, binning, d_capacity, img, out_color, out_invdepth, stream);
 }
 
diff --git a/d3ga_amd/csrc/raster_bin.hip b/d3ga_amd/csrc/raster_bin.hip
--- a/d3ga_amd/csrc/raster_bin.hip
+++ b/d3ga_amd/csrc/raster_bin.hip
@@ -1,6 +1,7 @@
 #include <atomic>
 
 #include "composite_common.h"
+#include "raster_colour.h"
 
 namespace d3ga {
 
@@ -169,6 +170,7 @@
     }
 }
 
+template <int COLOUR>
 __global__ __launch_bounds__(kScanBlock) void tile_scan_order_kernel(int tiles, const uint32_t *__restrict__ count,
                                                                      uint32_t *__restrict__ start,
                                                                      uint32_t *__restrict__ cursor,
@@ -177,7 +179,15 @@
                                                                      uint32_t *__restrict__ huge_tiles,
                                                                      uint32_t *__restrict__ mid_tiles, uint32_t n_small,
                                                                      uint32_t n_mid, uint32_t n_large,
-                                                                     uint32_t *__restrict__ order) {
+                                                                     uint32_t *__restrict__ order, ColourJob job) {
+    static_assert(kScanBlock == kColourUnit, "a colour unit is one workgroup of this launch");
+    if constexpr (COLOUR != 0) {
+        if ((int)blockIdx.x >= job.block0) {
+            extern __shared__ __attribute__((aligned(16))) char smem[];
+            colour_unit<COLOUR == 2>(job, reinterpret_cast<float *>(smem));
+            return;
+        }
+    }
     if (blockIdx.x == 0) tile_scan_body(tiles, count, start, cursor, counters, dcap, big_tiles, huge_tiles, mid_tiles, n_small, n_mid, n_large);
     else tile_order_body(tiles, count, order, counters);
 }
@@ -445,7 +455,7 @@
     }
 }
 
-template <int BLOCK, int CAP>
+template <int BLOCK, int CAP, int COLOUR = 0>
 __global__ __launch_bounds__(BLOCK) void tile_sort_lds_list_kernel(const uint32_t *__restrict__ start,
                                                                    const uint64_t *__restrict__ keys,
                                                                    uint32_t *__restrict__ point_list, uint64_t dcap,
@@ -455,19 +465,26 @@
                                                                    const uint32_t *__restrict__ huge_list,
                                                                    const uint32_t *__restrict__ huge_count,
                                                                    const uint32_t *__restrict__ list2,
-                                                                   const uint32_t *__restrict__ list2_count) {
+                                                                   const uint32_t *__restrict__ list2_count, ColourJob job, uint32_t sort_grid) {
     extern __shared__ __attribute__((aligned(16))) uint64_t s_key_dyn[];
+    if constexpr (COLOUR != 0) {
+        static_assert(BLOCK == kColourUnit, "a colour unit is one workgroup of this launch");
+        if ((int)blockIdx.x >= job.block0) {
+            colour_unit<COLOUR == 2>(job, reinterpret_cast<float *>(s_key_dyn));
+            return;
+        }
+    }
     uint32_t *s_bin = reinterpret_cast<uint32_t *>(s_key_dyn + CAP);
     uint32_t *s_red = s_bin + CAP + 1;
     uint32_t *s_cur = s_red + 2 * (BLOCK / 64) + 2;
     const uint32_t count = *list_count;
-    for (uint32_t v = blockIdx.x; v < count; v += gridDim.x) {
+    for (uint32_t v = blockIdx.x; v < count; v += sort_grid) {
         __syncthreads();
         sort_one_tile_bucket<BLOCK, CAP>(s_key_dyn, s_bin, s_red, (int)list[v], start, keys, point_list, dcap);
     }
     if (list2) {
         const uint32_t count2 = *list2_count;
-        for (uint32_t v = gridDim.x - 1u - blockIdx.x; v < count2; v += gridDim.x) {
+        for (uint32_t v = sort_grid - 1u - blockIdx.x; v < count2; v += sort_grid) {
             __syncthreads();
             sort_one_tile_bucket<BLOCK, CAP>(s_key_dyn, s_bin, s_red, (int)list2[v], start, keys, point_list, dcap);
         }
@@ -475,7 +492,7 @@
     if (huge_list) {
         const uint32_t hcount = *huge_count;
         const int tid = threadIdx.x;
-        for (uint32_t k = blockIdx.x; k < hcount; k += gridDim.x) {
+        for (uint32_t k = blockIdx.x; k < hcount; k += sort_grid) {
             const int tile = (int)huge_list[k];
             const uint64_t b64 = min((uint64_t)start[tile], dcap), e64 = min((uint64_t)start[tile + 1], dcap);
             const int n = (int)(e64 - b64);
@@ -498,10 +515,45 @@
 static inline size_t sort_lds_bytes(int cap, int block, bool huge = false) {
     return (size_t)cap * 8 + ((size_t)cap + 1 + 2 * (block / 64) + 2 + (huge ? cap : 0)) * 4 + 16;
 }
-
-
-extern "C" int d3ga_raster_bin_sort(const d3ga_raster_params *prm, void *geom, void *binning, int64_t d_capacity,
-                                    d3ga_stream_t stream) {
+static_assert(kColourLdsBytes <= (size_t)kSortLarge * 8 + ((size_t)2 * kSortLarge) * 4, "a colour unit's slabs fit the LDS of the 8192-key launch");
+
+extern "C" int d3ga_raster_colour_plan(int32_t P, int32_t list_launch, int32_t cus, int32_t scan_pct, int32_t out[3]) {
+    if (!out) return D3GA_E_NULL;
+    if (P < 0 || cus < 1) return D3GA_E_SIZE;
+    const int64_t units = ((int64_t)P + kColourUnit - 1) / kColourUnit;
+    int64_t scan = units;
+    if (list_launch) {
+        if (scan_pct >= 0 && scan_pct <= 100) scan = (units * scan_pct + 99) / 100;
+        else {
+            const int64_t a = cus > 2 ? cus - 2 : 1, b = cus > 1 ? cus - 1 : 1;
+            scan = (units * a + a + b - 1) / (a + b);
+        }
+    }
+    out[0] = (int32_t)units; out[1] = (int32_t)scan; out[2] = (int32_t)(units - scan);
+    return D3GA_OK;
+}
+
+static int colour_device(int *cus_out) {
+    static std::atomic<int> cus_of[64] = {};
+    int dev = 0;
+    D3GA_HIP(hipGetDevice(&dev));
+    int cus = (dev >= 0 && dev < 64) ? cus_of[dev].load(std::memory_order_relaxed) : 0;
+    if (cus == 0) {
+        if (hipDeviceGetAttribute(&cus, hipDeviceAttributeMultiprocessorCount, dev) != hipSuccess || cus < 1) cus = 256;
+        D3GA_HIP(hipFuncSetAttribute((const void *)tile_scan_order_kernel<1>, hipFuncAttributeMaxDynamicSharedMemorySize, (int)kColourLdsBytes));
+        D3GA_HIP(hipFuncSetAttribute((const void *)tile_scan_order_kernel<2>, hipFuncAttributeMaxDynamicSharedMemorySize, (int)kColourLdsBytes));
+        D3GA_HIP(hipFuncSetAttribute((const void *)tile_sort_lds_list_kernel<1024, kSortLarge, 1>,
+                                     hipFuncAttributeMaxDynamicSharedMemorySize, (int)sort_lds_bytes(kSortLarge, 1024, true)));
+        D3GA_HIP(hipFuncSetAttribute((const void *)tile_sort_lds_list_kernel<1024, kSortLarge, 2>,
+                                     hipFuncAttributeMaxDynamicSharedMemorySize, (int)sort_lds_bytes(kSortLarge, 1024, true)));
+        if (dev >= 0 && dev < 64) cus_of[dev].store(cus, std::memory_order_relaxed);
+    }
+    *cus_out = cus;
+    return D3GA_OK;
+}
+
+static int bin_sort_launch(const d3ga_raster_params *prm, void *geom, void *binning, int64_t d_capacity, d3ga_stream_t stream,
+                           bool colour, const float *means3D, const float *shs, const float *campos) {
     if (!prm || !geom || !binning) return D3GA_E_NULL;
     if (prm->P < 0 || prm->W <= 0 || prm->H <= 0 || d_capacity < 0) return D3GA_E_SIZE;
     hipStream_t s = (hipStream_t)stream;
@@ -511,9 +563,24 @@
     const int64_t P = (int64_t)prm->P * views;
     BinBuf bin = carve_bin(binning, tiles, d_capacity);
     GeomBuf g = carve_geom(geom, P);
-    hipLaunchKernelGGL(tile_scan_order_kernel, dim3(2), dim3(kScanBlock), 0, s, tiles, bin.tile_count, bin.tile_start,
-                       bin.tile_cursor, bin.counters, (uint64_t)d_capacity, bin.big_tiles, bin.huge_tiles, bin.mid_tiles,
-                       (uint32_t)kSortSmall, (uint32_t)kSortMid, (uint32_t)kSortLarge, bin.tile_order);
+    ColourJob job = {};
+    int plan[3] = {0, 0, 0};
+    const int cj = colour ? (prm->forward_only || !sh_staged(prm->M) ? 1 : 2) : 0;
+    if (colour) {
+        int cus = 0;
+        D3GA_TRY(colour_device(&cus));
+        D3GA_TRY(d3ga_raster_colour_plan(prm->P, d_capacity > 0, cus, debug_knob(D3GA_KNOB_COLOUR_SCAN_PCT), plan));
+        job.prm = *prm; job.means3D = means3D; job.shs = shs; job.campos = campos; job.geom = g;
+        job.block0 = 2; job.unit0 = 0;
+    }
+#define D3GA_LAUNCH_SCAN(COLOURV, GRID, LDS)                                                                                     \
+    hipLaunchKernelGGL(tile_scan_order_kernel<COLOURV>, dim3(GRID), dim3(kScanBlock), LDS, s, tiles, bin.tile_count, bin.tile_start, \
+                       bin.tile_cursor, bin.counters, (uint64_t)d_capacity, bin.big_tiles, bin.huge_tiles, bin.mid_tiles,           \
+                       (uint32_t)kSortSmall, (uint32_t)kSortMid, (uint32_t)kSortLarge, bin.tile_order, job)
+    if (plan[1] == 0) D3GA_LAUNCH_SCAN(0, 2, 0);
+    else if (cj == 1) D3GA_LAUNCH_SCAN(1, 2 + plan[1], kColourLdsBytes);
+    else D3GA_LAUNCH_SCAN(2, 2 + plan[1], kColourLdsBytes);
+#undef D3GA_LAUNCH_SCAN
     D3GA_TRY(check_launch(s, prm->debug));
     if (P == 0 || d_capacity == 0) return D3GA_OK;
     hipLaunchKernelGGL(tile_scatter_kernel, dim3((unsigned)((P + kBlock - 1) / kBlock)), dim3(kBlock), 0, s, (int)P, gx, g.rect,
@@ -548,17 +615,37 @@
     const int lgrid = tiles < 256 ? tiles : 256, mgrid = tiles < 768 ? tiles : 768;
     const int merge_knob = debug_knob(D3GA_KNOB_SORT_MERGE);
     const bool merged = merge_knob >= 0 ? merge_knob != 0 : d_capacity / (tiles > 0 ? tiles : 1) < 320;
-#define D3GA_LAUNCH_LIST_SORT(BLOCKV, CAPV, GRID, HUGE, LIST, CNT, KEYS_RW, HLIST, HCNT, LIST2, CNT2)                              \
-    hipLaunchKernelGGL((tile_sort_lds_list_kernel<BLOCKV, CAPV>), dim3(GRID), dim3(BLOCKV), sort_lds_bytes(CAPV, BLOCKV, HUGE), s, \
-                       bin.tile_start, bin.keys, bin.point_list, (uint64_t)d_capacity, LIST, CNT, KEYS_RW, HLIST, HCNT, LIST2, CNT2)
+#define D3GA_LAUNCH_LIST_SORT(BLOCKV, CAPV, COLOURV, GRID, HUGE, LIST, CNT, KEYS_RW, HLIST, HCNT, LIST2, CNT2)                              \
+    hipLaunchKernelGGL((tile_sort_lds_list_kernel<BLOCKV, CAPV, COLOURV>), dim3((GRID) + ((COLOURV) ? plan[2] : 0)), dim3(BLOCKV),            \
+                       sort_lds_bytes(CAPV, BLOCKV, HUGE), s, bin.tile_start, bin.keys, bin.point_list, (uint64_t)d_capacity, LIST, CNT,      \
+                       KEYS_RW, HLIST, HCNT, LIST2, CNT2, job, (uint32_t)(GRID))
     const uint32_t *const nil = nullptr;
     if (!merged) {
-        D3GA_LAUNCH_LIST_SORT(512, kSortMid, mgrid, false, bin.mid_tiles, bin.counters + D3GA_CNT_MID, (uint64_t *)nullptr, nil, nil, nil, nil);
+        D3GA_LAUNCH_LIST_SORT(512, kSortMid, 0, mgrid, false, bin.mid_tiles, bin.counters + D3GA_CNT_MID, (uint64_t *)nullptr, nil, nil, nil, nil);
         D3GA_TRY(check_launch(s, prm->debug));
     }
     const uint32_t *l2 = merged ? (const uint32_t *)bin.mid_tiles : nil, *c2 = merged ? (const uint32_t *)(bin.counters + D3GA_CNT_MID) : nil;
-    D3GA_LAUNCH_LIST_SORT(1024, kSortLarge, lgrid, true, bin.big_tiles, bin.counters + D3GA_CNT_BIG, bin.keys,
-                          (const uint32_t *)bin.huge_tiles, (const uint32_t *)(bin.counters + D3GA_CNT_HUGE), l2, c2);
+    job.block0 = lgrid; job.unit0 = plan[1];
+#define D3GA_LAUNCH_LARGE(COLOURV)                                                                                    \
+    D3GA_LAUNCH_LIST_SORT(1024, kSortLarge, COLOURV, lgrid, true, bin.big_tiles, bin.counters + D3GA_CNT_BIG, bin.keys, \
+                          (const uint32_t *)bin.huge_tiles, (const uint32_t *)(bin.counters + D3GA_CNT_HUGE), l2, c2)
+    if (plan[2] == 0) D3GA_LAUNCH_LARGE(0);
+    else if (cj == 1) D3GA_LAUNCH_LARGE(1);
+    else D3GA_LAUNCH_LARGE(2);
+#undef D3GA_LAUNCH_LARGE
 #undef D3GA_LAUNCH_LIST_SORT
     return check_launch(s, prm->debug);
 }
+
+extern "C" int d3ga_raster_bin_sort(const d3ga_raster_params *prm, void *geom, void *binning, int64_t d_capacity,
+                                    d3ga_stream_t stream) {
+    return bin_sort_launch(prm, geom, binning, d_capacity, stream, false, nullptr, nullptr, nullptr);
+}
+
+extern "C" int d3ga_raster_bin_sort_colour(const d3ga_raster_params *prm, const float *means3D, const float *shs, const float *campos,
+                                           void *geom, void *binning, int64_t d_capacity, d3ga_stream_t stream) {
+    if (!prm) return D3GA_E_NULL;
+    const bool colour = colour_split(prm, shs);
+    if (colour && (!means3D || !campos)) return D3GA_E_NULL;
+    return bin_sort_launch(prm, geom, binning, d_capacity, stream, colour, means3D, shs, campos);
+}
diff --git a/d3ga_amd/csrc/raster_colour.h b/d3ga_amd/csrc/raster_colour.h
--- /dev/null
+++ b/d3ga_amd/csrc/raster_colour.h
@@ -0,0 +1,159 @@
+#pragma once
+#include "composite_common.h"
+#include "raster_pre_body.h"
+
+namespace d3ga {
+
+constexpr int kShRow = 52;
+constexpr int kShSlab = 64 * kShRow;
+constexpr size_t kShLdsBytes = (size_t)(kBlock / 64) * kShSlab * sizeof(float);
+
+__host__ __device__ __forceinline__ bool sh_staged(int M) { return M > 0 && (3 * M) % 4 == 0 && 3 * M <= 48; }
+
+__device__ __forceinline__ void sh_slab_load(float *slab, const float *__restrict__ src, int rows, int M3, int lane) {
+    const int nvec = rows * M3 / 4;
+    for (int v = lane; v < nvec; v += 64) {
+        const float4 x = reinterpret_cast<const float4 *>(src)[v];
+        const int e = 4 * v, r = e / M3, c = e - r * M3;
+        *reinterpret_cast<float4 *>(slab + r * kShRow + c) = x;
+    }
+}
+__device__ __forceinline__ void sh_slab_store(const float *slab, float *__restrict__ dst, int rows, int M3, int lane) {
+    const int nvec = rows * M3 / 4;
+    for (int v = lane; v < nvec; v += 64) {
+        const int e = 4 * v, r = e / M3, c = e - r * M3;
+        reinterpret_cast<float4 *>(dst)[v] = *reinterpret_cast<const float4 *>(slab + r * kShRow + c);
+    }
+}
+
+template <int ROWS>
+struct ShRegs { float4 v[ROWS * 12 / 64]; };
+template <int ROWS>
+__device__ __forceinline__ ShRegs<ROWS> sh_rows48_load(const float *__restrict__ src, int lane) {
+    ShRegs<ROWS> r;
+#pragma unroll
+    for (int k = 0; k < ROWS * 12 / 64; ++k) r.v[k] = reinterpret_cast<const float4 *>(src)[lane + 64 * k];
+    return r;
+}
+template <int ROWS>
+__device__ __forceinline__ void sh_rows48_to_slab(float *slab, const ShRegs<ROWS> &r, int lane) {
+#pragma unroll
+    for (int k = 0; k < ROWS * 12 / 64; ++k) {
+        const int e = 4 * (lane + 64 * k), row = e / 48, c = e - row * 48;
+        *reinterpret_cast<float4 *>(slab + row * kShRow + c) = r.v[k];
+    }
+}
+template <int ROWS>
+__device__ __forceinline__ void sh_rows48_store(const float *slab, float *__restrict__ dst, int lane) {
+#pragma unroll
+    for (int k = 0; k < ROWS * 12 / 64; ++k) {
+        const int e = 4 * (lane + 64 * k), row = e / 48, c = e - row * 48;
+        reinterpret_cast<float4 *>(dst)[lane + 64 * k] = *reinterpret_cast<const float4 *>(slab + row * kShRow + c);
+    }
+}
+
+constexpr int kShPassRows = 32;
+constexpr int kShHalfSlab = kShPassRows * kShRow;
+constexpr size_t kShHalfLdsBytes = (size_t)(kBlock / 64) * kShHalfSlab * sizeof(float);
+
+template <bool WANT_J>
+__device__ __forceinline__ void staged_sh_colour(const d3ga_raster_params &prm, const float *__restrict__ means3D,
+                                                 const float *__restrict__ shs, const float *__restrict__ campos,
+                                                 float *s_sh, float acc[3], ShColJ &cj, int first) {
+    const int tid = threadIdx.x, lane = tid & 63, wave = tid >> 6;
+    const int i = first + tid;
+    const int M3 = 3 * prm.M;
+    float *slab = s_sh + wave * kShHalfSlab;
+    const int row0 = first + wave * 64;
+    const int rows = min(64, prm.P - row0);
+    const int nb = (prm.sh_degree + 1) * (prm.sh_degree + 1);
+    float B[16];
+    float dx = 0.f, dy = 0.f, dz = 1.f;
+    if (WANT_J && i < prm.P) sh_view_dir(means3D, i, campos, dx, dy, dz);
+    auto eval = [&](const float *row) __attribute__((always_inline)) {
+        if (WANT_J) cj = sh_accumulate_jacobian(B, dx, dy, dz, row, nb, cj);
+        else sh_accumulate(B, row, 0, 16, nb, acc);
+    };
+    if (M3 == 48 && rows == 64) {
+        const float *src = shs + (size_t)48 * row0;
+        const ShRegs<kShPassRows> h0 = sh_rows48_load<kShPassRows>(src, lane);
+        const ShRegs<kShPassRows> h1 = sh_rows48_load<kShPassRows>(src + 48 * kShPassRows, lane);
+        sh_view_basis(prm, means3D, i, campos, B);
+        __builtin_amdgcn_wave_barrier();
+        sh_rows48_to_slab<kShPassRows>(slab, h0, lane);
+        __builtin_amdgcn_wave_barrier();
+        if (lane / kShPassRows == 0) eval(slab + (lane % kShPassRows) * kShRow);
+        __builtin_amdgcn_wave_barrier();
+        sh_rows48_to_slab<kShPassRows>(slab, h1, lane);
+        __builtin_amdgcn_wave_barrier();
+        if (lane / kShPassRows == 1) eval(slab + (lane % kShPassRows) * kShRow);
+        return;
+    }
+    if (i < prm.P) sh_view_basis(prm, means3D, i, campos, B);
+    for (int h = 0; h < 2; ++h) {
+        const int r = min(kShPassRows, rows - kShPassRows * h);
+        __builtin_amdgcn_wave_barrier();
+        if (r > 0) sh_slab_load(slab, shs + (size_t)M3 * (row0 + kShPassRows * h), r, M3, lane);
+        __builtin_amdgcn_wave_barrier();
+        if (i < prm.P && lane / kShPassRows == h) eval(slab + (lane % kShPassRows) * kShRow);
+    }
+}
+
+template <bool WANT_J>
+__device__ __forceinline__ void colour_records(const d3ga_raster_params &prm, const float *__restrict__ means3D,
+                                               const float *__restrict__ shs, const float *__restrict__ colors_precomp,
+                                               const float *__restrict__ campos, const GeomBuf &src, const GeomBuf &dst, float *s_sh,
+                                               int first) {
+    const int i = first + threadIdx.x;
+    const int M3 = 3 * prm.M;
+    const bool staged = shs != nullptr && sh_staged(prm.M);
+    ShColJ cj = {0.f, 0.f, 0.f, 0.f, 0.f, 0.f, 0.f, 0.f, 0.f, 0.f, 0.f, 0.f};
+    float acc[3] = {0.f, 0.f, 0.f};
+    if (staged) staged_sh_colour<WANT_J>(prm, means3D, shs, campos, s_sh, acc, cj, first);
+    if (i >= prm.P) return;
+    if (WANT_J) {
+        acc[0] = cj.a0; acc[1] = cj.a1; acc[2] = cj.a2;
+        dcol_store(dst.dcol, dst.dcol_stride, i, cj);
+    }
+    const uint2 rc = src.rect[i];
+    const bool visible = rect_visible(rc.x, rc.y);
+    const float depth = src.depth[i];
+    float rgb[3] = {0.f, 0.f, 0.f};
+    uint8_t mask = 0;
+    if (visible) {
+        if (colors_precomp) {
+            rgb[0] = colors_precomp[3 * (size_t)i]; rgb[1] = colors_precomp[3 * (size_t)i + 1];
+            rgb[2] = colors_precomp[3 * (size_t)i + 2];
+        } else {
+            if (!staged) {
+                float B[16];
+                sh_view_basis(prm, means3D, i, campos, B);
+                sh_accumulate(B, shs + (size_t)M3 * i, 0, 16, (prm.sh_degree + 1) * (prm.sh_degree + 1), acc);
+            }
+#pragma unroll
+            for (int c = 0; c < 3; ++c) {
+                const float v = acc[c] + 0.5f;
+                if (v < 0.f) mask |= (uint8_t)(1u << c);
+                rgb[c] = fmaxf(v, 0.f);
+            }
+        }
+    }
+    dst.rgb_invd[i] = make_float4(rgb[0], rgb[1], rgb[2], visible ? 1.0f / depth : 0.f);
+    dst.clamped[i] = mask;
+}
+
+constexpr int kColourUnit = 1024;
+constexpr size_t kColourLdsBytes = (size_t)(kColourUnit / 64) * kShHalfSlab * sizeof(float);
+struct ColourJob {
+    d3ga_raster_params prm;
+    const float *means3D, *shs, *campos;
+    GeomBuf geom;
+    int block0, unit0;
+};
+template <bool WANT_J>
+__device__ __forceinline__ void colour_unit(const ColourJob &job, float *s_sh) {
+    const int unit = job.unit0 + ((int)blockIdx.x - job.block0);
+    colour_records<WANT_J>(job.prm, job.means3D, job.shs, nullptr, job.campos, job.geom, job.geom, s_sh, unit * kColourUnit);
+}
+
+}
diff --git a/d3ga_amd/csrc/raster_pre.hip b/d3ga_amd/csrc/raster_pre.hip
--- a/d3ga_amd/csrc/raster_pre.hip
+++ b/d3ga_amd/csrc/raster_pre.hip
@@ -1,106 +1,13 @@
 #include "composite_common.h"
+#include "raster_colour.h"
 #include "raster_pre_body.h"
 
 namespace d3ga {
 
-constexpr int kShRow = 52;
-constexpr int kShSlab = 64 * kShRow;
-constexpr size_t kShLdsBytes = (size_t)(kBlock / 64) * kShSlab * sizeof(float);
-
-__host__ __device__ __forceinline__ bool sh_staged(int M) { return M > 0 && (3 * M) % 4 == 0 && 3 * M <= 48; }
-
-__device__ __forceinline__ void sh_slab_load(float *slab, const float *__restrict__ src, int rows, int M3, int lane) {
-    const int nvec = rows * M3 / 4;
-    for (int v = lane; v < nvec; v += 64) {
-        const float4 x = reinterpret_cast<const float4 *>(src)[v];
-        const int e = 4 * v, r = e / M3, c = e - r * M3;
-        *reinterpret_cast<float4 *>(slab + r * kShRow + c) = x;
-    }
-}
-__device__ __forceinline__ void sh_slab_store(const float *slab, float *__restrict__ dst, int rows, int M3, int lane) {
-    const int nvec = rows * M3 / 4;
-    for (int v = lane; v < nvec; v += 64) {
-        const int e = 4 * v, r = e / M3, c = e - r * M3;
-        reinterpret_cast<float4 *>(dst)[v] = *reinterpret_cast<const float4 *>(slab + r * kShRow + c);
-    }
-}
-
-template <int ROWS>
-struct ShRegs { float4 v[ROWS * 12 / 64]; };
-template <int ROWS>
-__device__ __forceinline__ ShRegs<ROWS> sh_rows48_load(const float *__restrict__ src, int lane) {
-    ShRegs<ROWS> r;
-#pragma unroll
-    for (int k = 0; k < ROWS * 12 / 64; ++k) r.v[k] = reinterpret_cast<const float4 *>(src)[lane + 64 * k];
-    return r;
-}
-template <int ROWS>
-__device__ __forceinline__ void sh_rows48_to_slab(float *slab, const ShRegs<ROWS> &r, int lane) {
-#pragma unroll
-    for (int k = 0; k < ROWS * 12 / 64; ++k) {
-        const int e = 4 * (lane + 64 * k), row = e / 48, c = e - row * 48;
-        *reinterpret_cast<float4 *>(slab + row * kShRow + c) = r.v[k];
-    }
-}
-template <int ROWS>
-__device__ __forceinline__ void sh_rows48_store(const float *slab, float *__restrict__ dst, int lane) {
-#pragma unroll
-    for (int k = 0; k < ROWS * 12 / 64; ++k) {
-        const int e = 4 * (lane + 64 * k), row = e / 48, c = e - row * 48;
-        reinterpret_cast<float4 *>(dst)[lane + 64 * k] = *reinterpret_cast<const float4 *>(slab + row * kShRow + c);
-    }
-}
-
-constexpr int kShPassRows = 32;
-constexpr int kShHalfSlab = kShPassRows * kShRow;
-constexpr size_t kShHalfLdsBytes = (size_t)(kBlock / 64) * kShHalfSlab * sizeof(float);
-
-template <bool WANT_J>
-__device__ __forceinline__ void staged_sh_colour(const d3ga_raster_params &prm, const float *__restrict__ means3D,
-                                                 const float *__restrict__ shs, const float *__restrict__ campos,
-                                                 float *s_sh, float acc[3], ShColJ &cj) {
-    const int tid = threadIdx.x, lane = tid & 63, wave = tid >> 6;
-    const int i = blockIdx.x * kBlock + tid;
-    const int M3 = 3 * prm.M;
-    float *slab = s_sh + wave * kShHalfSlab;
-    const int row0 = blockIdx.x * kBlock + wave * 64;
-    const int rows = min(64, prm.P - row0);
-    const int nb = (prm.sh_degree + 1) * (prm.sh_degree + 1);
-    float B[16];
-    float dx = 0.f, dy = 0.f, dz = 1.f;
-    if (WANT_J && i < prm.P) sh_view_dir(means3D, i, campos, dx, dy, dz);
-    auto eval = [&](const float *row) __attribute__((always_inline)) {
-        if (WANT_J) cj = sh_accumulate_jacobian(B, dx, dy, dz, row, nb, cj);
-        else sh_accumulate(B, row, 0, 16, nb, acc);
-    };
-    if (M3 == 48 && rows == 64) {
-        const float *src = shs + (size_t)48 * row0;
-        const ShRegs<kShPassRows> h0 = sh_rows48_load<kShPassRows>(src, lane);
-        const ShRegs<kShPassRows> h1 = sh_rows48_load<kShPassRows>(src + 48 * kShPassRows, lane);
-        sh_view_basis(prm, means3D, i, campos, B);
-        __builtin_amdgcn_wave_barrier();
-        sh_rows48_to_slab<kShPassRows>(slab, h0, lane);
-        __builtin_amdgcn_wave_barrier();
-        if (lane / kShPassRows == 0) eval(slab + (lane % kShPassRows) * kShRow);
-        __builtin_amdgcn_wave_barrier();
-        sh_rows48_to_slab<kShPassRows>(slab, h1, lane);
-        __builtin_amdgcn_wave_barrier();
-        if (lane / kShPassRows == 1) eval(slab + (lane % kShPassRows) * kShRow);
-        return;
-    }
-    if (i < prm.P) sh_view_basis(prm, means3D, i, campos, B);
-    for (int h = 0; h < 2; ++h) {
-        const int r = min(kShPassRows, rows - kShPassRows * h);
-        __builtin_amdgcn_wave_barrier();
-        if (r > 0) sh_slab_load(slab, shs + (size_t)M3 * (row0 + kShPassRows * h), r, M3, lane);
-        __builtin_amdgcn_wave_barrier();
-        if (i < prm.P && lane / kShPassRows == h) eval(slab + (lane % kShPassRows) * kShRow);
-    }
-}
 
 struct TileRect { bool visible; int r0, r1, r2, r3; };
 __device__ __forceinline__ TileRect write_geom_records(const GeomBuf &geom, int i, const PreOut &o, bool keep_cov, int tile_row0,
-                                                       int32_t *__restrict__ radii, bool want_j, const ShColJ &cj) {
+                                                       int32_t *__restrict__ radii, bool want_j, const ShColJ &cj, bool colour = true) {
     const Splat &sp = o.sp;
     if (keep_cov) {
 #pragma unroll
@@ -116,9 +23,11 @@
         const SplatCull sc = splat_cull(sp.conic[0], sp.conic[1], sp.conic[2], o.opacity);
         geom.xyh[i] = make_float4(sp.px, sp.py, sp.visible ? sc.hx : -1.0f, sc.hy);
     }
-    geom.rgb_invd[i] = make_float4(o.rgb[0], o.rgb[1], o.rgb[2], sp.visible ? 1.0f / sp.depth : 0.f);
-    geom.clamped[i] = o.clampmask;
-    if (want_j) dcol_store(geom.dcol, geom.dcol_stride, i, cj);
+    if (colour) {
+        geom.rgb_invd[i] = make_float4(o.rgb[0], o.rgb[1], o.rgb[2], sp.visible ? 1.0f / sp.depth : 0.f);
+        geom.clamped[i] = o.clampmask;
+        if (want_j) dcol_store(geom.dcol, geom.dcol_stride, i, cj);
+    }
     return TileRect{sp.visible, sp.rect[0], sp.rect[1] + tile_row0, sp.rect[2], sp.rect[3] + tile_row0};
 }
 
@@ -168,7 +77,7 @@
                                                     const float *sh_row, bool staged, const ShColJ &cj, bool pre, const float (&pc6)[6],
                                                     float pop, const float *colors_precomp, const float *opacities, const float *scales,
                                                     const float *rotations, const float *cov3D_precomp, const GeomBuf &geom,
-                                                    int tile_row0, int32_t *radii, bool want_j, int gx, int gy) {
+                                                    int tile_row0, int32_t *radii, bool want_j, int gx, int gy, bool colour = true) {
     PreLoaded pl;
     pl.has_sh = staged; pl.has_c6 = pre;
     pl.sh[0] = cj.a0; pl.sh[1] = cj.a1; pl.sh[2] = cj.a2;
@@ -177,10 +86,10 @@
     pl.op = pop;
     PreOut o = preprocess_one(prm, cam, i, means3D, sh_row, colors_precomp, opacities, scales, rotations, cov3D_precomp, pl);
     if constexpr (WIN) o = window_clip(o, cam.ox / kTile, cam.oy / kTile, gx, gy);
-    return write_geom_records(geom, i, o, !cov3D_precomp, tile_row0, radii, want_j, cj);
-}
-
-template <bool WANT_J, bool WIN>
+    return write_geom_records(geom, i, o, !cov3D_precomp, tile_row0, radii, want_j, cj, colour);
+}
+
+template <bool WANT_J, bool WIN, bool GEOM_ONLY = false>
 __global__ __launch_bounds__(kBlock) void preprocess_kernel(
     d3ga_raster_params prm, const float *__restrict__ means3D, const float *__restrict__ shs,
     const float *__restrict__ colors_precomp, const float *__restrict__ opacities, const float *__restrict__ scales,
@@ -197,9 +106,9 @@
     const int tid = threadIdx.x;
     const int i = blockIdx.x * kBlock + tid;
     const int M3 = 3 * prm.M;
-    const bool staged = shs != nullptr && sh_staged(prm.M);
+    const bool staged = !GEOM_ONLY && shs != nullptr && sh_staged(prm.M);
     float pc6[6] = {0.f, 0.f, 0.f, 0.f, 0.f, 0.f}, pop = 0.f;
-    const bool pre = staged && cov3D_precomp != nullptr;
+    const bool pre = (staged || GEOM_ONLY) && cov3D_precomp != nullptr;
     if (pre && i < prm.P) {
 #pragma unroll
         for (int k = 0; k < 6; ++k) pc6[k] = cov3D_precomp[6 * (size_t)i + k];
@@ -208,12 +117,16 @@
     ShColJ cj = {0.f, 0.f, 0.f, 0.f, 0.f, 0.f, 0.f, 0.f, 0.f, 0.f, 0.f, 0.f};
     float acc[3] = {0.f, 0.f, 0.f};
     if (staged) {
-        staged_sh_colour<WANT_J>(prm, means3D, shs, campos, s_sh, acc, cj);
+        staged_sh_colour<WANT_J>(prm, means3D, shs, campos, s_sh, acc, cj, blockIdx.x * kBlock);
         if (!WANT_J) { cj.a0 = acc[0]; cj.a1 = acc[1]; cj.a2 = acc[2]; }
         __syncthreads();
     }
     TileRect tr = {false, 0, 0, 0, 0};
     if (i < prm.P) {
+        if constexpr (GEOM_ONLY)
+            tr = preprocess_view<WIN>(prm, cam, i, means3D, nullptr, true, cj, pre, pc6, pop, nullptr, opacities, scales, rotations,
+                                      cov3D_precomp, geom, tile_row0, radii, false, gx, gy, false);
+        else
         tr = staged ? preprocess_view<WIN>(prm, cam, i, means3D, nullptr, true, cj, pre, pc6, pop, colors_precomp, opacities, scales,
                                            rotations, cov3D_precomp, geom, tile_row0, radii, WANT_J, gx, gy)
                     : preprocess_view<WIN>(prm, cam, i, means3D, shs ? shs + (size_t)M3 * i : nullptr, false, cj, false, pc6, pop,
@@ -321,49 +234,15 @@
                                                          const float *__restrict__ colors_precomp,
                                                          const float *__restrict__ campos, GeomBuf src, GeomBuf dst) {
     extern __shared__ __attribute__((aligned(16))) char smem[];
-    float *s_sh = reinterpret_cast<float *>(smem);
     const int i = blockIdx.x * kBlock + threadIdx.x;
-    const int M3 = 3 * prm.M;
-    const bool staged = shs != nullptr && sh_staged(prm.M);
-    ShColJ cj = {0.f, 0.f, 0.f, 0.f, 0.f, 0.f, 0.f, 0.f, 0.f, 0.f, 0.f, 0.f};
-    float acc[3] = {0.f, 0.f, 0.f};
-    if (staged) staged_sh_colour<WANT_J>(prm, means3D, shs, campos, s_sh, acc, cj);
+    colour_records<WANT_J>(prm, means3D, shs, colors_precomp, campos, src, dst, reinterpret_cast<float *>(smem), blockIdx.x * kBlock);
     if (i >= prm.P) return;
-    if (WANT_J) {
-        acc[0] = cj.a0; acc[1] = cj.a1; acc[2] = cj.a2;
-        dcol_store(dst.dcol, dst.dcol_stride, i, cj);
-    }
-    const uint2 rc = src.rect[i];
-    const bool visible = rect_visible(rc.x, rc.y);
-    const float depth = src.depth[i];
-    dst.depth[i] = depth;
+    dst.depth[i] = src.depth[i];
     dst.conic_o[i] = src.conic_o[i];
     dst.xyh[i] = src.xyh[i];
-    dst.rect[i] = rc;
+    dst.rect[i] = src.rect[i];
 #pragma unroll
     for (int k = 0; k < 6; ++k) dst.cov3D[6 * (size_t)i + k] = src.cov3D[6 * (size_t)i + k];
-    float rgb[3] = {0.f, 0.f, 0.f};
-    uint8_t mask = 0;
-    if (visible) {
-        if (colors_precomp) {
-            rgb[0] = colors_precomp[3 * (size_t)i]; rgb[1] = colors_precomp[3 * (size_t)i + 1];
-            rgb[2] = colors_precomp[3 * (size_t)i + 2];
-        } else {
-            if (!staged) {
-                float B[16];
-                sh_view_basis(prm, means3D, i, campos, B);
-                sh_accumulate(B, shs + (size_t)M3 * i, 0, 16, (prm.sh_degree + 1) * (prm.sh_degree + 1), acc);
-            }
-#pragma unroll
-            for (int c = 0; c < 3; ++c) {
-                const float v = acc[c] + 0.5f;
-                if (v < 0.f) mask |= (uint8_t)(1u << c);
-                rgb[c] = fmaxf(v, 0.f);
-            }
-        }
-    }
-    dst.rgb_invd[i] = make_float4(rgb[0], rgb[1], rgb[2], visible ? 1.0f / depth : 0.f);
-    dst.clamped[i] = mask;
 }
 
 __device__ __forceinline__ ViewRecs view_recs(const GeomBuf &g, const float *acc) {
@@ -564,11 +443,11 @@
 template <class T>
 static T *at(T *p, size_t n, size_t r) { return p ? p + n * r : nullptr; }
 
-extern "C" int d3ga_raster_preprocess(const d3ga_raster_params *prm, const float *means3D, const float *shs,
-                                      const float *colors_precomp, const float *opacities, const float *scales,
-                                      const float *rotations, const float *cov3D_precomp, const float *viewmatrix,
-                                      const float *projmatrix, const float *campos, void *geom, void *binning,
-                                      int64_t d_capacity, int32_t *radii, d3ga_stream_t stream) {
+static int preprocess_launch(const d3ga_raster_params *prm, const float *means3D, const float *shs,
+                             const float *colors_precomp, const float *opacities, const float *scales,
+                             const float *rotations, const float *cov3D_precomp, const float *viewmatrix,
+                             const float *projmatrix, const float *campos, void *geom, void *binning,
+                             int64_t d_capacity, int32_t *radii, d3ga_stream_t stream, bool split) {
     D3GA_TRY(validate(prm));
     if (!geom || !binning || !viewmatrix || !projmatrix || !campos) return D3GA_E_NULL;
     if (d_capacity < 0) return D3GA_E_SIZE;
@@ -588,7 +467,8 @@
     if (shs && (prm->sh_degree + 1) * (prm->sh_degree + 1) > prm->M) return D3GA_E_CONFIG;
     if (!means3D || !opacities || !radii) return D3GA_E_NULL;
     const GeomBuf g = carve_geom(geom, (int64_t)prm->P * views);
-    const size_t lds = lds_bytes(staged(prm, shs), kShHalfLdsBytes, (size_t)kWinTiles * 4);
+    const bool geom_only = split && colour_split(prm, shs);
+    const size_t lds = lds_bytes(staged(prm, shs) && !geom_only, kShHalfLdsBytes, (size_t)kWinTiles * 4);
     const bool want_j = leaves_dcol(prm, shs);
     const int cs = cam_stride(prm);
     const size_t pv = (views > 1 && prm->per_view_geometry) ? (size_t)prm->P : 0;
@@ -611,8 +491,9 @@
         else if (left == 3 || left == 5) launch_group(std::integral_constant<int, 3>());
         else launch_group(std::integral_constant<int, 2>());
     }
-    const auto kernel = want_j ? (wnd ? preprocess_kernel<true, true> : preprocess_kernel<true, false>)
-                               : (wnd ? preprocess_kernel<false, true> : preprocess_kernel<false, false>);
+    const auto kernel = geom_only ? preprocess_kernel<false, false, true>
+                        : want_j  ? (wnd ? preprocess_kernel<true, true> : preprocess_kernel<true, false>)
+                                  : (wnd ? preprocess_kernel<false, true> : preprocess_kernel<false, false>);
     for (int v = v0; v < views; ++v) {
         const ViewCams<1> c = view_cams<1>(viewmatrix, projmatrix, campos, cs, v, 1);
         const size_t og = pv * v, oa = pa * v;
@@ -621,6 +502,24 @@
                            geom_view(g, prm->P, v), bin.tile_count, bin.counters, radii + (size_t)prm->P * v, v * gyv);
     }
     return check_launch(s, prm->debug & 0xff);
+}
+
+extern "C" int d3ga_raster_preprocess(const d3ga_raster_params *prm, const float *means3D, const float *shs,
+                                      const float *colors_precomp, const float *opacities, const float *scales,
+                                      const float *rotations, const float *cov3D_precomp, const float *viewmatrix,
+                                      const float *projmatrix, const float *campos, void *geom, void *binning,
+                                      int64_t d_capacity, int32_t *radii, d3ga_stream_t stream) {
+    return preprocess_launch(prm, means3D, shs, colors_precomp, opacities, scales, rotations, cov3D_precomp, viewmatrix, projmatrix,
+                             campos, geom, binning, d_capacity, radii, stream, false);
+}
+
+extern "C" int d3ga_raster_preprocess_split(const d3ga_raster_params *prm, const float *means3D, const float *shs,
+                                            const float *colors_precomp, const float *opacities, const float *scales,
+                                            const float *rotations, const float *cov3D_precomp, const float *viewmatrix,
+                                            const float *projmatrix, const float *campos, void *geom, void *binning,
+                                            int64_t d_capacity, int32_t *radii, d3ga_stream_t stream) {
+    return preprocess_launch(prm, means3D, shs, colors_precomp, opacities, scales, rotations, cov3D_precomp, viewmatrix, projmatrix,
+                             campos, geom, binning, d_capacity, radii, stream, true);
 }
 
 extern "C" int d3ga_raster_recolor(const d3ga_raster_params *prm, const float *means3D, const float *shs,
diff --git a/d3ga_amd/rasterizer.py b/d3ga_amd/rasterizer.py
--- a/d3ga_amd/rasterizer.py
+++ b/d3ga_amd/rasterizer.py
@@ -231,12 +231,12 @@
     L = _lib.lib()
     if stage_timer.enabled or k > 1 or pair is not None or l1 is not None:
         st, pp = stream_handle(), ctypes.byref(prm)
-        stage_timer.stage("preprocess", lambda: check(L.d3ga_raster_preprocess(
+        stage_timer.stage("preprocess", lambda: check(L.d3ga_raster_preprocess_split(
             pp, dptr(means3D), dptr(sh), dptr(colors_precomp), dptr(opacities), dptr(scales), dptr(rotations),
             dptr(cov3Ds_precomp), dptr(view), dptr(proj), dptr(campos), dptr(geom), dptr(binning), cap,
-            dptr(radii), st), "d3ga_raster_preprocess"))
-        stage_timer.stage("bin_sort", lambda: check(L.d3ga_raster_bin_sort(
-            pp, dptr(geom), dptr(binning), cap, st), "d3ga_raster_bin_sort"))
+            dptr(radii), st), "d3ga_raster_preprocess_split"))
+        stage_timer.stage("bin_sort", lambda: check(L.d3ga_raster_bin_sort_colour(
+            pp, dptr(means3D), dptr(sh), dptr(campos), dptr(geom), dptr(binning), cap, st), "d3ga_raster_bin_sort_colour"))
         _composite_forward(prm, cap, windowed, bg, geom, binning, img, color, invdepth, pair, l1)
     else:
         check(L.d3ga_raster_forward(ctypes.byref(prm), dptr(means3D), dptr(sh), dptr(colors_precomp),
diff --git a/include/d3ga.h b/include/d3ga.h
--- a/include/d3ga.h
+++ b/include/d3ga.h
@@ -32,7 +32,9 @@
 #define D3GA_KNOB_WGRAD_WS 6
 #define D3GA_KNOB_CHAIN_ABL 7
 #define D3GA_KNOB_CHAIN_GRID 8
-#define D3GA_KNOB_COUNT 9
+#define D3GA_KNOB_SPLIT_COLOUR 9
+#define D3GA_KNOB_COLOUR_SCAN_PCT 10
+#define D3GA_KNOB_COUNT 11
 #define D3GA_KNOB_DEFAULT (-2147483647 - 1)
 int d3ga_debug_set(int32_t key, int32_t value);
 int d3ga_debug_defaults(int32_t *out, int32_t n);
@@ -197,6 +199,14 @@
                            int64_t d_capacity, int32_t *radii, d3ga_stream_t stream);
 int d3ga_raster_bin_sort(const d3ga_raster_params *prm, void *geom, void *binning, int64_t d_capacity,
                          d3ga_stream_t stream);
+int d3ga_raster_preprocess_split(const d3ga_raster_params *prm, const float *means3D, const float *shs,
+                                 const float *colors_precomp, const float *opacities, const float *scales,
+                                 const float *rotations, const float *cov3D_precomp, const float *viewmatrix,
+                                 const float *projmatrix, const float *campos, void *geom, void *binning,
+                                 int64_t d_capacity, int32_t *radii, d3ga_stream_t stream);
+int d3ga_raster_bin_sort_colour(const d3ga_raster_params *prm, const float *means3D, const float *shs, const float *campos,
+                                void *geom, void *binning, int64_t d_capacity, d3ga_stream_t stream);
+int d3ga_raster_colour_plan(int32_t P, int32_t list_launch, int32_t cus, int32_t scan_pct, int32_t out[3]);
 int d3ga_raster_composite_fwd(const d3ga_raster_params *prm, const float *bg, const void *geom, const void *binning,
                               int64_t d_capacity, void *img, float *out_color, float *out_invdepth,
                               d3ga_stream_t stream);
```

After: 2571. -1.9%, worse.
